# tkoolen/Parametron.jl

Hardware: AMD Instinct MI355X
Metric: QP re-evaluations/sec (Q,q,C,d rebuild) at n=4096 (higher is better)
Workload: dtype f64; 1 GPU; C2 dense least-squares QP: n=4096 vars, A 4096x4096, m=512 equality rows, fp64; canonical Q,q,const + C,d MOI triplets; n=4096, r=4096, m=512, objective_mode=canonical, instances_per_gpu=1, parallelism=single GPU, replay=tape

## Files before the change

include/parametron_hip.h:

```cpp
#ifndef PARAMETRON_HIP_H
#define PARAMETRON_HIP_H

#include <stddef.h>
#include <stdint.h>

#ifdef __cplusplus
extern "C" {
#endif

#define PMT_OK 0
#define PMT_DIMENSION_MISMATCH 1
#define PMT_INVALID_ARGUMENT 2
#define PMT_HIP_ERROR 3
#define PMT_STATE_ERROR 4
#define PMT_OUT_OF_MEMORY 5

typedef struct { double coeff; int64_t var; } pmt_linear_term;
typedef struct { double coeff; int64_t row; int64_t col; } pmt_quadratic_term;
typedef struct { int64_t output_index; double coeff; int64_t var; } pmt_vector_affine_term;

const char *pmt_last_error(void);
int pmt_version(void);
int pmt_device_count(void);

// ... 127 lines not shown
int pmt_pack_scalar_affine_f64(const pmt_linear_term *terms, int64_t n, const int64_t *varmap,
                               pmt_linear_term *out_terms, void *stream);
int pmt_pack_scalar_quadratic_f64(const pmt_quadratic_term *quad, int64_t nq, const int64_t *varmap,
                                  pmt_quadratic_term *out_quad, void *stream);
int pmt_pack_vector_affine_f64(const pmt_linear_term *terms, const int64_t *row_ptr, int64_t rows, int64_t row_len,
                               const int64_t *varmap, int64_t row_offset,
                               pmt_vector_affine_term *out_terms, void *stream);

int pmt_canonical_order_affine(int64_t n, const int64_t *host_vars, int64_t *host_perm, int64_t *host_seg_ptr, int64_t *host_out_vars,
                               int64_t *nseg);
int pmt_canonical_order_quadratic(int64_t n, const int64_t *host_rows, const int64_t *host_cols, int64_t *host_perm, int64_t *host_seg_ptr,
                                  int64_t *host_out_rows, int64_t *host_out_cols, int64_t *nseg);
int pmt_segment_sum_f64(const void *in_terms, int64_t in_stride_bytes, const int64_t *perm, const int64_t *seg_ptr, int64_t nseg,
                        void *out_terms, int64_t out_stride_bytes, void *stream);
int pmt_canonical_order_device(const void *terms, int64_t n, int term_bytes, int64_t *perm, int64_t *seg_ptr, int64_t *nseg_host, void *stream);
int pmt_canonical_init_terms(const void *terms, int term_bytes, const int64_t *perm, const int64_t *seg_ptr, int64_t nseg, void *out_terms, void *stream);

size_t pmt_prune_zero_workspace_bytes(int64_t n, int term_bytes);
int pmt_prune_zero_f64(const void *terms, int64_t n, int term_bytes, double atol, void *out_terms, int64_t *out_count,
                       void *workspace, size_t workspace_bytes, void *stream);

enum { PMT_SET_EQUAL = 0, PMT_SET_GREATER = 1, PMT_SET_LESS = 2 };
int pmt_csc_order(int64_t nnz_in, const int64_t *host_rows, const int64_t *host_cols, int64_t nrows, int64_t ncols, int upper,
                  int64_t *host_perm, int64_t *host_seg_ptr, int64_t *host_col_ptr, int64_t *host_row_idx, int64_t *nnz_out);
int pmt_csc_values_f64(const void *src_coeff, int64_t src_stride_bytes, int64_t nnz_in, const int64_t *perm, const int64_t *seg_ptr,
                       int64_t nnz_out, double alpha, const int64_t *dst_index, double *dst_values, void *stream);
int pmt_qp_bounds_f64(const double *consts, int64_t rows, int set_kind, double set_value, double infty, double *l, double *u,
                      void *stream);
int pmt_csc_values_gather_f64(const double *const *term_ptr, int64_t nnz_in, const int64_t *seg_ptr, int64_t nnz_out, double alpha,
                              const int64_t *dst_index, double *dst_values, void *stream);
int pmt_copy_2d_f64(const double *src, int64_t src_pitch, double *dst, int64_t dst_pitch, const int64_t *dst_offset, int64_t rows,
                    int64_t cols, void *stream);
int pmt_qp_bounds_rows_f64(const double *const *const_ptr, const int *set_kind, const double *set_value, int64_t rows, double infty,
                           double *l, double *u, void *stream);

int pmt_sparse_rowmajor_order(int64_t m, int64_t n, const int64_t *host_colptr, const int64_t *host_rowval,
                              int64_t *host_perm, int64_t *host_rows, int64_t *host_cols, int64_t *host_row_ptr);
int pmt_sparse_pack_vector_f64(const double *nzval, const int64_t *perm, const int64_t *term_row, const int64_t *term_var,
                               int64_t nnz, const int64_t *varmap, int64_t row_offset,
                               pmt_vector_affine_term *out_terms, void *stream);
int pmt_sparse_assemble_f64(const double *nzval, const int64_t *perm, const int64_t *term_var, int64_t nnz,
                            pmt_linear_term *out_terms, void *stream);
int pmt_sparse_slab_ptr(int64_t rows, int64_t cols, int nslab, const int64_t *host_row_ptr, const int64_t *host_term_col,
                        int64_t *host_slab_ptr);
int pmt_sparse_pack_vector_slabs_f64(const double *nzval, const int64_t *perm, const int64_t *term_var, const int64_t *slab_ptr,
                                     int64_t rows, int nslab, const int64_t *varmap, int64_t row_offset,
                                     pmt_vector_affine_term *out_terms, void *stream);
int pmt_sparse_assemble_slabs_f64(const double *nzval, const int64_t *perm, const int64_t *term_var, const int64_t *slab_ptr,
                                  int64_t rows, int nslab, pmt_linear_term *out_terms, void *stream);
int pmt_sparse_pack_vector_slabs_u32_f64(const double *nzval, const uint32_t *perm, const uint32_t *term_var, const int64_t *slab_ptr,
                                         int64_t rows, int nslab, const int64_t *varmap, int64_t row_offset,
                                         pmt_vector_affine_term *out_terms, void *stream);
int pmt_sparse_assemble_slabs_u32_f64(const double *nzval, const uint32_t *perm, const uint32_t *term_var, const int64_t *slab_ptr,
                                      int64_t rows, int nslab, pmt_linear_term *out_terms, void *stream);

int pmt_sparse_blocks_width(int64_t m, int64_t n, const int64_t *host_colptr, const int64_t *host_rowval, int *out_cw);
int pmt_sparse_blocks_build(int64_t m, int64_t n, const int64_t *host_colptr, const int64_t *host_rowval, const int64_t *host_perm,
                            const int64_t *host_term_col, const int64_t *host_row_ptr, int cw, uint64_t *host_desc, uint32_t *host_idx,
                            int64_t *host_band_ptr);
int pmt_sparse_pack_vector_blocks_f64(const double *nzval, const uint64_t *desc, const uint32_t *idx, const int64_t *band_ptr,
                                      const int64_t *col_var, int64_t rows, int64_t cols, int64_t nnz, int cw, const int64_t *varmap,
                                      int64_t row_offset, const double *d, int sign, pmt_vector_affine_term *out_terms,
                                      double *out_consts, void *stream);
int pmt_sparse_assemble_blocks_f64(const double *nzval, const uint64_t *desc, const uint32_t *idx, const int64_t *band_ptr,
                                   const int64_t *col_var, int64_t rows, int64_t cols, int64_t nnz, int cw, const double *d, int sign,
                                   pmt_linear_term *out_terms, double *out_consts, void *stream);
int pmt_consts_f64(const double *d, int64_t n, int sign, double *out, void *stream);

int pmt_sparse_gram_count(int64_t m, int64_t n, const int64_t *host_colptr, const int64_t *host_rowval, int64_t *nq, int64_t *nprod);
int pmt_sparse_gram_order(int64_t m, int64_t n, const int64_t *host_colptr, const int64_t *host_rowval, int64_t nq, int64_t nprod,
                          uint32_t *host_pair_j, uint32_t *host_pair_k, int64_t *host_seg_ptr, void *host_prod, uint32_t *host_lin_col,
                          int64_t *nlin);
int pmt_sparse_gram_runs(const int64_t *host_seg_ptr, int64_t nq, int64_t cap, int64_t *host_runs, int64_t *nruns, int64_t *host_long_seg,
                         int64_t *nlong);
int pmt_sparse_gram_f64(const double *nzval, const void *prod, const int64_t *seg_ptr, const uint32_t *pair_j, const uint32_t *pair_k,
                        int64_t nq, const int64_t *runs, int64_t nruns, const int64_t *long_seg, int64_t nlong,
                        const int64_t *lin_seg, const uint32_t *rowidx0, const uint32_t *lin_col, int64_t nlin, const int64_t *lin_runs,
                        int64_t nlin_runs, const int64_t *lin_long, int64_t nlin_long, int64_t rows, const int64_t *xvar, const double *d,
                        int sign, int moi, const int64_t *varmap, pmt_quadratic_term *out_quad, pmt_linear_term *out_lin, double *out_const,
                        void *stream);

int64_t pmt_batch_lsq_slab_doubles(int64_t n, int64_t m);
int pmt_batch_lsq_coeffs_f64(const double *A, const double *b, const double *C, const double *d, int64_t B, int64_t n, int64_t r,
                             int64_t m, int sign_b, int sign_d, double *out, int64_t out_stride, void *stream);
int pmt_batch_expand_f64(const double *slab, int64_t n, int64_t m, const int64_t *xvar, const int64_t *varmap,
                         pmt_quadratic_term *out_quad, pmt_linear_term *out_lin, double *out_const,
                         pmt_vector_affine_term *out_vat, double *out_vconsts, void *stream);

int pmt_fill_uniform_f64(double *dst, int64_t n, uint64_t seed, double scale, void *stream);
int pmt_fill_uniform_matrix_f64(double *dst, int64_t rows, int64_t cols, int64_t lda, uint64_t seed, double scale, void *stream);
int pmt_fill_uniform_dyn_f64(double *dst, int64_t rows, int64_t cols, int64_t lda, const uint64_t *seed_word, double scale, void *stream);
int pmt_fill_uniform_offset_f64(double *dst, int64_t n, uint64_t seed, uint64_t index_offset, double scale, void *stream);

int pmt_profile_enable(int on);
int pmt_profile_filter(const char *substring);
int64_t pmt_profile_report(char *host_buf, size_t cap);
int pmt_profile_kernel_stamps(void *device_words, int64_t workgroups);
int pmt_device_clock_khz(int device, int *khz);

int pmt_comm_unique_id(void *out_id_128_bytes);
int pmt_comm_init_rank(int nranks, int rank, const void *unique_id_128_bytes, int device, void **out_comm);
int64_t pmt_comm_rccl_calls(void *comm);
int pmt_comm_destroy(void *comm);
int pmt_batch_shard(int64_t total, int nranks, int rank, int64_t *per_rank, int64_t *first);
int64_t pmt_batch_num_chunks(int64_t per_rank, int64_t chunk);
int pmt_batch_chunk_range(int64_t per_rank, int64_t chunk, int64_t c, int64_t *lo, int64_t *hi);
int64_t pmt_batch_gathered_offset(int rank, int64_t per_rank, int64_t local_instance, int64_t stride);
int pmt_batch_allgather_f64(void *comm, const double *local, double *gathered, int64_t per_rank, int64_t stride, int64_t chunk, void *stream);
int pmt_batch_step_f64(void *comm, const double *A, const double *b, const double *C, const double *d, int64_t per_rank, int64_t n, int64_t r,
                       int64_t m, int sign_b, int sign_d, double *local, double *gathered, int64_t stride, int64_t chunk, void *stream);

typedef struct pmt_plan pmt_plan;

int pmt_plan_create(int device, void *stream , pmt_plan **out);
int pmt_plan_destroy(pmt_plan *plan);
void *pmt_plan_stream(pmt_plan *plan);
int pmt_plan_alloc(pmt_plan *plan, size_t bytes, void **out_device_ptr);
size_t pmt_plan_bytes_allocated(const pmt_plan *plan);
int pmt_host_alloc(size_t bytes, void **out_host_ptr);
int pmt_host_free(void *host_ptr);
int pmt_plan_upload(pmt_plan *plan, void *device_dst, const void *host_src, size_t bytes);
int pmt_plan_fetch(pmt_plan *plan, void *host_dst, const void *device_src, size_t bytes);
int pmt_plan_zero(pmt_plan *plan, void *device_dst, size_t bytes);
int pmt_plan_upload_2d(pmt_plan *plan, void *device_dst, size_t dst_pitch, const void *host_src, size_t src_pitch, size_t width_bytes,
                       size_t height);
int pmt_plan_fetch_2d(pmt_plan *plan, void *host_dst, size_t dst_pitch, const void *device_src, size_t src_pitch, size_t width_bytes,
                      size_t height);
int pmt_plan_synchronize(pmt_plan *plan);
int pmt_plan_check(pmt_plan *plan);
int pmt_plan_record_fetch(pmt_plan *plan, void *host_dst, const void *device_src, size_t bytes);
int pmt_plan_record_fetch_2d(pmt_plan *plan, void *host_dst, size_t dst_pitch, const void *device_src, size_t src_pitch, size_t width_bytes,
                             size_t height);
int pmt_host_copy_2d(void *host_dst, size_t dst_pitch, const void *host_src, size_t src_pitch, size_t width_bytes, size_t height, int threads);
int pmt_plan_fetch_synchronize(pmt_plan *plan);

int pmt_plan_stage_upload(pmt_plan *plan, void *device_staging, const void *host_src, size_t bytes);
int pmt_plan_stage_upload_2d(pmt_plan *plan, void *device_staging, size_t dst_pitch, const void *host_src, size_t src_pitch, size_t width_bytes,
                             size_t height);
int pmt_plan_wait_staged(pmt_plan *plan);
int pmt_plan_commit_staged(pmt_plan *plan, void *device_dst, const void *device_staging, size_t bytes);
int pmt_plan_staging_consumed(pmt_plan *plan);
int pmt_plan_commit_lane(pmt_plan *plan, int lane);
int pmt_plan_staged_synchronize(pmt_plan *plan);
int pmt_plan_stage_slot(pmt_plan *plan, int slot);

int pmt_plan_begin_record(pmt_plan *plan);
int pmt_plan_end_record(pmt_plan *plan);
int pmt_plan_set_lane(pmt_plan *plan, int lane);
int pmt_plan_lane_stream(pmt_plan *plan, int lane, void **out_stream);
void *pmt_plan_recording_stream(pmt_plan *plan);
int64_t pmt_plan_tape_length(const pmt_plan *plan);
int pmt_plan_set_fusion(pmt_plan *plan, int on);
int pmt_plan_fused(const pmt_plan *plan, int *groups, int *nodes, int64_t *exec_length);
int pmt_plan_fused_phases(const pmt_plan *plan);
int pmt_plan_fused_workgroups(const pmt_plan *plan);
typedef struct pmt_model pmt_model;
int pmt_model_create(pmt_plan *plan, pmt_model **out);
int pmt_model_destroy(pmt_model *model);
int pmt_model_add_mailbox(pmt_model *model, const double *host, int64_t rows, int64_t cols, int64_t row_stride, int64_t col_stride,
                          double *mailbox, int64_t ld, int *out_slot);
int pmt_model_add_seed(pmt_model *model, uint64_t *seed_word, uint64_t base, uint64_t stride, int *out_slot);
int pmt_model_set_host(pmt_model *model, int slot, const double *host);
int pmt_model_add_constant(pmt_model *model, const double *src, double *dst);
int pmt_model_add_fetch(pmt_model *model, void *host_dst, const void *device_src, size_t bytes);
int pmt_model_num_slots(const pmt_model *model);
int pmt_model_update(pmt_model *model, const unsigned char *dirty, int nslots, int synchronize);
int pmt_model_wait(pmt_model *model);
int pmt_plan_update(pmt_plan *plan);
int pmt_plan_instantiate_graph(pmt_plan *plan);

#ifdef __cplusplus
}
#endif
#endif
```

parametron.jl_amd/_lib.py:

```python
import ctypes as C
import os

import numpy as np

HERE = os.path.dirname(os.path.abspath(__file__))
LIB_PATH = os.environ.get("PMT_LIB_PATH") or os.path.join(HERE, "lib", "libparametron_hip.so")

LT = np.dtype([("coeff", "<f8"), ("var", "<i8")])
QT = np.dtype([("coeff", "<f8"), ("row", "<i8"), ("col", "<i8")])
VAT = np.dtype([("out", "<i8"), ("coeff", "<f8"), ("var", "<i8")])

PMT_OK, PMT_DIMENSION_MISMATCH, PMT_INVALID_ARGUMENT, PMT_HIP_ERROR, PMT_STATE_ERROR, PMT_OUT_OF_MEMORY = range(6)
PMT_LSQ_BLOCK, PMT_LSQ_DIAG, PMT_LSQ_LINEAR, PMT_LSQ_CONSTANT = 1, 2, 3, 4
PMT_LSQ_MAX_TERMS, PMT_LSQ_MAX_BLOCKS, PMT_LSQ_MAX_RUNS = 32, 8, 64
PMT_QUAD_MAX_GROUPS = 8
STACK_COLUMN = np.dtype([("src", "<u8"), ("sign", "<i8")])


class LsqTerm(C.Structure):
    _fields_ = [("kind", C.c_int32), ("sign", C.c_int32), ("scale", C.c_double), ("weight", C.c_void_p), ("values", C.c_void_p),
                ("lin", C.c_void_p), ("constant", C.c_void_p), ("vec", C.c_void_p)]


def lsq_terms(terms):
# ... 57 lines not shown

class ArgumentError(ValueError):
    """Julia's ArgumentError (src/lazyexpression.jl:175,185; src/model.jl:226,243,246)."""


class ErrorException(RuntimeError):
    """Julia's ErrorException — error(...) (src/model.jl:50,61,69,139)."""


class HipError(RuntimeError):
    pass


_vp, _i64, _f64, _ci, _u64, _sz = C.c_void_p, C.c_int64, C.c_double, C.c_int, C.c_uint64, C.c_size_t

SIGNATURES = {
    "pmt_last_error": (C.c_char_p, []),
    "pmt_version": (_ci, []),
    "pmt_device_count": (_ci, []),
    "pmt_affine_assemble_f64": (_ci, [_vp, _i64, _i64, _i64, _vp, _vp, _ci, _vp, _vp, _vp]),
    "pmt_affine_pack_vector_f64": (_ci, [_vp, _i64, _i64, _i64, _vp, _vp, _ci, _vp, _i64, _vp, _vp, _vp]),
    "pmt_affine_pack_vector_background_f64": (_ci, [_vp, _i64, _i64, _i64, _vp, _vp, _ci, _vp, _i64, _vp, _vp, _vp]),
    "pmt_vars_addsub_f64": (_ci, [_vp, _i64, _vp, _ci, _vp, _i64, _vp, _vp, _vp, _vp]),
    "pmt_affvec_combine_f64": (_ci, [_i64, _vp, _vp, _i64, _vp, _vp, _vp, _i64, _vp, _ci, _vp, _vp, _i64, _vp, _vp]),
    "pmt_affvec_scale_f64": (_ci, [_i64, _i64, _vp, _vp, _vp, _f64, _vp, _vp, _vp]),
    "pmt_scale_vars_f64": (_ci, [_vp, _i64, _vp, _f64, _vp, _vp]),
    "pmt_scale_numbers_f64": (_ci, [_vp, _i64, _vp, _f64, _vp, _vp]),
    "pmt_transpose_f64": (_ci, [_vp, _i64, _i64, _i64, _vp, _i64, _vp]),
    "pmt_quad_combine_f64": (_ci, [_vp, _i64, _vp, _i64, _ci, _vp, _vp]),
    "pmt_quad_scale_f64": (_ci, [_vp, _i64, _vp, _f64, _vp, _vp]),
    "pmt_copy_bytes": (_ci, [_vp, _vp, _sz, _vp]),
    "pmt_matvecmul_affs_f64": (_ci, [_vp, _i64, _i64, _i64, _vp, _i64, _vp, _vp, _vp, _vp]),
    "pmt_vecdot_numbers_vars_f64": (_ci, [_vp, _vp, _i64, _vp, _vp, _vp]),
    "pmt_vecdot_numbers_affs_f64": (_ci, [_vp, _i64, _vp, _i64, _vp, _vp, _vp, _vp]),
    "pmt_quad_expand_f64": (_ci, [_i64, _vp, _i64, _vp, _vp, _i64, _vp, _ci, _vp, _vp, _vp, _vp, _vp]),
    "pmt_quad_gram_workspace_bytes": (_sz, [_i64, _i64]),
    "pmt_quad_gram_constant_order": (_ci, [_i64, _i64, C.POINTER(_ci), C.POINTER(_ci), C.POINTER(_ci)]),
    "pmt_quad_gram_f64": (_ci, [_vp, _i64, _i64, _i64, _vp, _vp, _ci, _ci, _vp, _vp, _vp, _vp, _vp, _vp]),
    "pmt_quad_gram_csc_f64": (_ci, [_vp, _i64, _i64, _i64, _vp, _vp, _ci, _vp, _f64, _vp, _vp, _vp, _vp, _vp, _vp]),
    "pmt_quad_gram_csc_deliver_f64": (_ci, [_vp, _i64, _i64, _i64, _vp, _vp, _ci, _vp, _f64, _vp, _vp, _ci, _vp, _vp, _vp, _vp]),
    "pmt_quad_gram_deliver_f64": (_ci, [_vp, _i64, _i64, _i64, _vp, _vp, _ci, _ci, _vp, _vp, _vp, _ci, _vp, _vp, _vp, _vp]),
    "pmt_quad_gram_sum_f64": (_ci, [_i64, _vp, _ci, _vp, _vp, _vp, _vp]),
    "pmt_quad_gram_sum_sub_f64": (_ci, [_i64, _vp, _ci, _vp, _vp, _vp, _vp, _vp, _vp]),
    "pmt_affine_stack_columns_f64": (_ci, [_vp, _i64, _i64, _vp, _i64, _vp]),
    "pmt_quad_form_f64": (_ci, [_vp, _i64, _i64, _vp, _ci, _vp, _f64, _vp, _vp, _vp, _vp, _vp]),
    "pmt_quad_groups_gather_f64": (_ci, [_vp, _vp, _vp, _i64, _i64, _vp, _vp, _i64, _vp, _vp, _vp]),
    "pmt_quad_groups_constant_f64": (_ci, [_vp, _ci, _vp, _vp]),
    "pmt_fetch_synchronize": (_ci, [_vp]),
    "pmt_set_host_delivery": (_ci, [_ci]),
    "pmt_get_host_delivery": (_ci, [_ci, C.POINTER(_ci), C.POINTER(_ci)]),
    "pmt_set_fault_injection": (_ci, [_ci]),
    "pmt_bilinear_f64": (_ci, [_vp, _i64, _i64, _i64, _vp, _vp, _ci, _vp, _vp, _vp]),
    "pmt_fill_uniform_matrix_f64": (_ci, [_vp, _i64, _i64, _i64, _u64, _f64, _vp]),
    "pmt_plan_upload_2d": (_ci, [_vp, _vp, _sz, _vp, _sz, _sz, _sz]),
    "pmt_plan_fetch_2d": (_ci, [_vp, _vp, _sz, _vp, _sz, _sz, _sz]),
    "pmt_vecdot_terms_f64": (_ci, [_i64, _vp, _vp, _vp, _vp, _ci, _vp, _vp, _vp]),
    "pmt_vecdot_affs_vars_f64": (_ci, [_i64, _vp, _i64, _vp, _vp, _ci, _vp, _vp, _vp, _vp]),
    "pmt_pack_scalar_affine_f64": (_ci, [_vp, _i64, _vp, _vp, _vp]),
    "pmt_pack_scalar_quadratic_f64": (_ci, [_vp, _i64, _vp, _vp, _vp]),
    "pmt_pack_vector_affine_f64": (_ci, [_vp, _vp, _i64, _i64, _vp, _i64, _vp, _vp]),
    "pmt_canonical_order_affine": (_ci, [_i64, _vp, _vp, _vp, _vp, C.POINTER(_i64)]),
    "pmt_canonical_order_quadratic": (_ci, [_i64, _vp, _vp, _vp, _vp, _vp, _vp, C.POINTER(_i64)]),
    "pmt_canonical_order_device": (_ci, [_vp, _i64, _ci, _vp, _vp, C.POINTER(_i64), _vp]),
    "pmt_canonical_init_terms": (_ci, [_vp, _ci, _vp, _vp, _i64, _vp, _vp]),
    "pmt_segment_sum_f64": (_ci, [_vp, _i64, _vp, _vp, _i64, _vp, _i64, _vp]),
    "pmt_prune_zero_workspace_bytes": (_sz, [_i64, _ci]),
    "pmt_prune_zero_f64": (_ci, [_vp, _i64, _ci, _f64, _vp, _vp, _vp, _sz, _vp]),
    "pmt_csc_order": (_ci, [_i64, _vp, _vp, _i64, _i64, _ci, _vp, _vp, _vp, _vp, C.POINTER(_i64)]),
    "pmt_csc_values_f64": (_ci, [_vp, _i64, _i64, _vp, _vp, _i64, _f64, _vp, _vp, _vp]),
    "pmt_qp_bounds_f64": (_ci, [_vp, _i64, _ci, _f64, _f64, _vp, _vp, _vp]),
    "pmt_csc_values_gather_f64": (_ci, [_vp, _i64, _vp, _i64, _f64, _vp, _vp, _vp]),
    "pmt_copy_2d_f64": (_ci, [_vp, _i64, _vp, _i64, _vp, _i64, _i64, _vp]),
    "pmt_qp_bounds_rows_f64": (_ci, [_vp, _vp, _vp, _i64, _f64, _vp, _vp, _vp]),
    "pmt_sparse_rowmajor_order": (_ci, [_i64, _i64, _vp, _vp, _vp, _vp, _vp, _vp]),
    "pmt_sparse_assemble_f64": (_ci, [_vp, _vp, _vp, _i64, _vp, _vp]),
    "pmt_sparse_pack_vector_f64": (_ci, [_vp, _vp, _vp, _vp, _i64, _vp, _i64, _vp, _vp]),
    "pmt_sparse_slab_ptr": (_ci, [_i64, _i64, _ci, _vp, _vp, _vp]),
    "pmt_sparse_pack_vector_slabs_f64": (_ci, [_vp, _vp, _vp, _vp, _i64, _ci, _vp, _i64, _vp, _vp]),
    "pmt_sparse_assemble_slabs_f64": (_ci, [_vp, _vp, _vp, _vp, _i64, _ci, _vp, _vp]),
    "pmt_sparse_pack_vector_slabs_u32_f64": (_ci, [_vp, _vp, _vp, _vp, _i64, _ci, _vp, _i64, _vp, _vp]),
    "pmt_sparse_assemble_slabs_u32_f64": (_ci, [_vp, _vp, _vp, _vp, _i64, _ci, _vp, _vp]),
    "pmt_sparse_blocks_width": (_ci, [_i64, _i64, _vp, _vp, _vp]),
    "pmt_sparse_blocks_build": (_ci, [_i64, _i64, _vp, _vp, _vp, _vp, _vp, _ci, _vp, _vp, _vp]),
    "pmt_sparse_pack_vector_blocks_f64": (_ci, [_vp, _vp, _vp, _vp, _vp, _i64, _i64, _i64, _ci, _vp, _i64, _vp, _ci, _vp, _vp, _vp]),
    "pmt_sparse_assemble_blocks_f64": (_ci, [_vp, _vp, _vp, _vp, _vp, _i64, _i64, _i64, _ci, _vp, _ci, _vp, _vp, _vp]),
    "pmt_sparse_gram_count": (_ci, [_i64, _i64, _vp, _vp, C.POINTER(_i64), C.POINTER(_i64)]),
    "pmt_sparse_gram_order": (_ci, [_i64, _i64, _vp, _vp, _i64, _i64, _vp, _vp, _vp, _vp, _vp, C.POINTER(_i64)]),
    "pmt_sparse_gram_runs": (_ci, [_vp, _i64, _i64, _vp, C.POINTER(_i64), _vp, C.POINTER(_i64)]),
    "pmt_sparse_gram_f64": (_ci, [_vp, _vp, _vp, _vp, _vp, _i64, _vp, _i64, _vp, _i64, _vp, _vp, _vp, _i64, _vp, _i64, _vp, _i64, _i64, _vp, _vp, _ci,
                                  _ci, _vp, _vp, _vp, _vp, _vp]),
    "pmt_batch_lsq_slab_doubles": (_i64, [_i64, _i64]),
    "pmt_batch_lsq_coeffs_f64": (_ci, [_vp, _vp, _vp, _vp, _i64, _i64, _i64, _i64, _ci, _ci, _vp, _i64, _vp]),
    "pmt_batch_expand_f64": (_ci, [_vp, _i64, _i64, _vp, _vp, _vp, _vp, _vp, _vp, _vp, _vp]),
    "pmt_comm_unique_id": (_ci, [_vp]),
    "pmt_comm_init_rank": (_ci, [_ci, _ci, _vp, _ci, C.POINTER(_vp)]),
    "pmt_comm_destroy": (_ci, [_vp]),
    "pmt_comm_rccl_calls": (_i64, [_vp]),
    "pmt_batch_num_chunks": (_i64, [_i64, _i64]),
    "pmt_batch_chunk_range": (_ci, [_i64, _i64, _i64, C.POINTER(_i64), C.POINTER(_i64)]),
    "pmt_batch_gathered_offset": (_i64, [_ci, _i64, _i64, _i64]),
    "pmt_batch_shard": (_ci, [_i64, _ci, _ci, C.POINTER(_i64), C.POINTER(_i64)]),
    "pmt_batch_allgather_f64": (_ci, [_vp, _vp, _vp, _i64, _i64, _i64, _vp]),
    "pmt_batch_step_f64": (_ci, [_vp, _vp, _vp, _vp, _vp, _i64, _i64, _i64, _i64, _ci, _ci, _vp, _vp, _i64, _i64, _vp]),
    "pmt_consts_f64": (_ci, [_vp, _i64, _ci, _vp, _vp]),
    "pmt_fill_uniform_f64": (_ci, [_vp, _i64, _u64, _f64, _vp]),
    "pmt_fill_uniform_offset_f64": (_ci, [_vp, _i64, _u64, _u64, _f64, _vp]),
    "pmt_profile_enable": (_ci, [_ci]),
    "pmt_profile_filter": (_ci, [C.c_char_p]),
    "pmt_profile_kernel_stamps": (_ci, [_vp, _i64]),
    "pmt_device_clock_khz": (_ci, [_ci, C.POINTER(_ci)]),
    "pmt_profile_report": (_i64, [C.c_char_p, _sz]),
    "pmt_plan_create": (_ci, [_ci, _vp, C.POINTER(_vp)]),
    "pmt_plan_destroy": (_ci, [_vp]),
    "pmt_plan_stream": (_vp, [_vp]),
    "pmt_plan_alloc": (_ci, [_vp, _sz, C.POINTER(_vp)]),
    "pmt_plan_bytes_allocated": (_sz, [_vp]),
    "pmt_host_alloc": (_ci, [_sz, C.POINTER(_vp)]),
    "pmt_host_free": (_ci, [_vp]),
    "pmt_plan_upload": (_ci, [_vp, _vp, _vp, _sz]),
    "pmt_plan_fetch": (_ci, [_vp, _vp, _vp, _sz]),
    "pmt_plan_zero": (_ci, [_vp, _vp, _sz]),
    "pmt_plan_synchronize": (_ci, [_vp]),
    "pmt_plan_check": (_ci, [_vp]),
    "pmt_model_create": (_ci, [_vp, C.POINTER(_vp)]),
    "pmt_model_destroy": (_ci, [_vp]),
    "pmt_model_add_mailbox": (_ci, [_vp, _vp, _i64, _i64, _i64, _i64, _vp, _i64, C.POINTER(_ci)]),
    "pmt_model_add_seed": (_ci, [_vp, C.POINTER(C.c_uint64), C.c_uint64, C.c_uint64, C.POINTER(_ci)]),
    "pmt_model_set_host": (_ci, [_vp, _ci, _vp]),
    "pmt_model_add_constant": (_ci, [_vp, _vp, _vp]),
    "pmt_model_add_fetch": (_ci, [_vp, _vp, _vp, C.c_size_t]),
    "pmt_model_num_slots": (_ci, [_vp]),
    "pmt_model_update": (_ci, [_vp, _vp, _ci, _ci]),
    "pmt_model_wait": (_ci, [_vp]),
    "pmt_plan_record_fetch": (_ci, [_vp, _vp, _vp, _sz]),
    "pmt_plan_record_fetch_2d": (_ci, [_vp, _vp, _sz, _vp, _sz, _sz, _sz]),
    "pmt_host_copy_2d": (_ci, [_vp, _sz, _vp, _sz, _sz, _sz, _ci]),
    "pmt_plan_fetch_synchronize": (_ci, [_vp]),
    "pmt_plan_stage_upload": (_ci, [_vp, _vp, _vp, _sz]),
    "pmt_plan_stage_upload_2d": (_ci, [_vp, _vp, _sz, _vp, _sz, _sz, _sz]),
    "pmt_plan_wait_staged": (_ci, [_vp]),
    "pmt_plan_commit_staged": (_ci, [_vp, _vp, _vp, _sz]),
    "pmt_plan_staging_consumed": (_ci, [_vp]),
    "pmt_plan_staged_synchronize": (_ci, [_vp]),
    "pmt_plan_stage_slot": (_ci, [_vp, _ci]),
    "pmt_plan_begin_record": (_ci, [_vp]),
    "pmt_plan_end_record": (_ci, [_vp]),
    "pmt_plan_commit_lane": (_ci, [_vp, _ci]),
    "pmt_plan_set_lane": (_ci, [_vp, _ci]),
    "pmt_plan_lane_stream": (_ci, [_vp, _ci, C.POINTER(_vp)]),
    "pmt_plan_recording_stream": (_vp, [_vp]),
    "pmt_plan_tape_length": (_i64, [_vp]),
    "pmt_plan_set_fusion": (_ci, [_vp, _ci]),
    "pmt_plan_fused": (_ci, [_vp, C.POINTER(_ci), C.POINTER(_ci), C.POINTER(_i64)]),
    "pmt_plan_fused_phases": (_ci, [_vp]),
    "pmt_plan_fused_workgroups": (_ci, [_vp]),
    "pmt_fill_uniform_dyn_f64": (_ci, [_vp, _i64, _i64, _i64, C.POINTER(_u64), _f64, _vp]),
    "pmt_plan_update": (_ci, [_vp]),
    "pmt_plan_instantiate_graph": (_ci, [_vp]),
}

_lib = None


def load():
    global _lib
    if _lib is None:
        if not os.path.exists(LIB_PATH):
            raise ErrorException(
                "libparametron_hip.so is not built (%s); run `python -c 'import __graft_entry__ as g; g.build()'`" % LIB_PATH)
        if os.environ.get("PMT_NO_TORCH_PRELOAD") != "1":
            try:
                import torch
            except Exception:
                pass
        L = C.CDLL(LIB_PATH)
        for name, (res, args) in SIGNATURES.items():
            fn = getattr(L, name)
            fn.restype = res
            fn.argtypes = args
        _lib = L
    return _lib


def require_gpu():
    n = load().pmt_device_count()
    if n <= 0:
        raise ErrorException("no MI355X / HIP device visible: the Parametron hot path has no CPU fallback")
    return n


def check(rc):
    if rc == PMT_OK:
        return
    msg = load().pmt_last_error().decode("utf-8", "replace")
    if rc == PMT_DIMENSION_MISMATCH:
        raise DimensionMismatch(msg)
    if rc == PMT_INVALID_ARGUMENT:
        raise ArgumentError(msg)
    if rc == PMT_STATE_ERROR:
        raise ErrorException(msg)
    if rc == PMT_OUT_OF_MEMORY:
        raise MemoryError(msg)
    raise HipError(msg)


def call(name, *args):
    check(getattr(load(), name)(*args))
```

parametron.jl_amd/csrc/affine.hip:

```cpp
#include "common.h"

namespace pmt {

constexpr int64_t NTL_MIN_BYTES = 8 << 20;

constexpr int TILE = 64;
constexpr int PITCH = TILE + 1;

typedef unsigned long long u64;
typedef u64 u64x2 __attribute__((ext_vector_type(2)));
typedef double f64x2 __attribute__((ext_vector_type(2)));

__device__ __forceinline__ u64 f2u(double x) { return (u64)__double_as_longlong(x); }

template <bool NT>
__device__ __forceinline__ void store16(u64x2 *p, u64x2 v) {
    if (NT) __builtin_nontemporal_store(v, p); else *p = v;
}
template <bool NT>
__device__ __forceinline__ void store8(u64 *p, u64 v) {
    if (NT) __builtin_nontemporal_store(v, p); else *p = v;
}

template <int MODE, bool NT, int TR, bool NTL = false>
__global__ __launch_bounds__(256) void affine_tile_kernel(
    const double *__restrict__ A, int64_t lda, int64_t rows, int64_t cols,
    const int64_t *__restrict__ xvar, const double *__restrict__ b, int sign,
    const int64_t *__restrict__ varmap, int64_t row_offset,
    u64 *__restrict__ out, double *__restrict__ out_consts, int vec_in, int vec_out, u64 *stamps, unsigned stamp_cap) {
    __shared__ double tile[TR * PITCH];
    __shared__ u64 vmx[TILE];

    const int t = threadIdx.x;
    const unsigned wg = blockIdx.y * gridDim.x + blockIdx.x;
    if (stamps && t == 0 && wg < stamp_cap) stamps[2 * wg] = (u64)wall_clock64();
    const int lane = t & 63;
    const int wave = t >> 6;
    const int64_t c0 = (int64_t)blockIdx.x * TILE;
    const int64_t r0 = (int64_t)blockIdx.y * TR;
    const int nr = (int)min((int64_t)TR, rows - r0);
    const int nc = (int)min((int64_t)TILE, cols - c0);
    const bool full = (nr == TR) && (nc == TILE);

    if (full && vec_in) {
        constexpr int TPC = TR / 2;
        constexpr int CPI = 256 / TPC;
        const int cg = t / TPC;
        const int lr = (t % TPC) * 2;
        const double *base = A + (c0 + cg) * lda + r0 + lr;
#pragma unroll
        for (int it = 0; it < TILE / CPI; ++it) {
            const f64x2 *src = reinterpret_cast<const f64x2 *>(base + (int64_t)it * CPI * lda);
            f64x2 v = NTL ? __builtin_nontemporal_load(src) : *src;
            const int c = it * CPI + cg;
            tile[lr * PITCH + c] = v.x;
            tile[(lr + 1) * PITCH + c] = v.y;
        }
    } else {
        const int r = t & 63;
        for (int c = t >> 6; c < nc; c += 4)
            if (r < nr) tile[r * PITCH + c] = A[(c0 + c) * lda + r0 + r];
    }
    if (t < nc) {
        const int64_t v = xvar[c0 + t];
        vmx[t] = (u64)(MODE == 1 ? map_var(varmap, v) : v);
    }
    if (blockIdx.x == 0 && t < nr && out_consts)
        out_consts[r0 + t] = signed_const(b ? b[r0 + t] : 0.0, b ? sign : 0);
    __syncthreads();

    if (MODE == 0) {
        if (lane < nc) {
            const u64 var = vmx[lane];
            for (int r = wave; r < nr; r += 4) {
                u64x2 v;
                v.x = f2u(tile[r * PITCH + lane]);
                v.y = var;
                store16<NT>(reinterpret_cast<u64x2 *>(out + ((r0 + r) * cols + c0 + lane) * 2), v);
            }
        }
    } else {
        if (full && vec_out) {
            for (int rp = wave * 2; rp < TR; rp += 8) {
#pragma unroll
                for (int s = 0; s < 3; ++s) {
                    int r, chunk;
                    if (s == 0) { r = rp; chunk = lane; }
                    else if (s == 1) { r = rp + (lane >> 5); chunk = 64 + (lane & 31); }
                    else { r = rp + 1; chunk = lane; }
                    const int q0 = chunk * 2;
                    const u64 rowidx = (u64)(row_offset + r0 + r + 1);
                    u64 w[2];
#pragma unroll
                    for (int h = 0; h < 2; ++h) {
                        const int q = q0 + h;
                        const int term = q / 3;
                        const int f = q - term * 3;
                        w[h] = (f == 0) ? rowidx : (f == 1 ? f2u(tile[r * PITCH + term]) : vmx[term]);
                    }
                    u64x2 v; v.x = w[0]; v.y = w[1];
                    store16<NT>(reinterpret_cast<u64x2 *>(out + ((r0 + r) * cols + c0) * 3 + q0), v);
                }
            }
        } else {
            if (lane < nc) {
                const u64 var = vmx[lane];
                for (int r = wave; r < nr; r += 4) {
                    u64 *p = out + ((r0 + r) * cols + c0 + lane) * 3;
                    store8<NT>(p, (u64)(row_offset + r0 + r + 1));
                    store8<NT>(p + 1, f2u(tile[r * PITCH + lane]));
                    store8<NT>(p + 2, var);
                }
            }
        }
    }
    if (stamps) {
        __syncthreads();
        if (t == 0 && wg < stamp_cap) {
            __builtin_amdgcn_s_waitcnt(0);
            stamps[2 * wg + 1] = (u64)wall_clock64();
        }
    }
}

__global__ void vars_addsub_kernel(const int64_t *__restrict__ xvar, int64_t n, const double *__restrict__ v, int sign,
                                   const int64_t *__restrict__ varmap, int64_t row_offset,
                                   LT *__restrict__ out_lt, VAT *__restrict__ out_vat, double *__restrict__ out_consts) {
    const int64_t i = (int64_t)blockIdx.x * blockDim.x + threadIdx.x;
    if (i >= n) return;
    const int64_t var = xvar[i];
    if (out_lt) { LT t; t.coeff = 1.0; t.var = var; out_lt[i] = t; }
    if (out_vat) { VAT t; t.output_index = row_offset + i + 1; t.coeff = 1.0; t.var = map_var(varmap, var); out_vat[i] = t; }
    if (out_consts) out_consts[i] = signed_const(v ? v[i] : 0.0, v ? sign : 0);
}

__global__ void consts_kernel(const double *__restrict__ d, int64_t n, int sign, double *__restrict__ out) {
    const int64_t i = (int64_t)blockIdx.x * blockDim.x + threadIdx.x;
    if (i < n) out[i] = signed_const(d[i], sign);
}

__global__ __launch_bounds__(256) void affine_pack_background_kernel(const double *__restrict__ A, int64_t lda, int rows, int cols,
                                                                     const int64_t *__restrict__ xvar, const int64_t *__restrict__ varmap,
                                                                     int64_t row_offset, unsigned long long *__restrict__ out) {
    const int wave = blockIdx.x * 4 + (threadIdx.x >> 6), lane = threadIdx.x & 63;
    const int chunk = wave / rows, row = wave - chunk * rows;
    const int c0 = chunk * 256 + lane;
    const double *a = A + row;
    unsigned long long *o = out + (int64_t)row * cols * 3;
    const unsigned long long rowword = (unsigned long long)(row_offset + row + 1);
#pragma unroll 1
    for (int c = c0; c < min(cols, chunk * 256 + 256); c += 64) {
        const double v = a[(int64_t)c * lda];
        const int64_t var = map_var(varmap, xvar[c]);
        unsigned long long *p = o + (int64_t)c * 3;
        p[0] = rowword;
        p[1] = (unsigned long long)__double_as_longlong(v);
        p[2] = (unsigned long long)var;
    }
}

__global__ void pack_scalar_affine_kernel(const LT *__restrict__ in, int64_t n, const int64_t *__restrict__ varmap, LT *__restrict__ out) {
    const int64_t i = (int64_t)blockIdx.x * blockDim.x + threadIdx.x;
    if (i >= n) return;
    LT t = in[i];
    t.var = map_var(varmap, t.var);
    out[i] = t;
}
__global__ __launch_bounds__(256) void pack_scalar_quadratic_kernel(const QT *__restrict__ in, int64_t n, const int64_t *__restrict__ varmap,
                                                                    QT *__restrict__ out, int aligned) {
    typedef unsigned long long u64;
    typedef u64 u64x2 __attribute__((ext_vector_type(2)));
    __shared__ u64 words[256 * 3];
    const int64_t base = (int64_t)blockIdx.x * 256;
    const int cnt = (int)min((int64_t)256, n - base);
    const int tid = threadIdx.x;
    if (aligned && cnt == 256) {
        const u64x2 *src = reinterpret_cast<const u64x2 *>(in + base);
        u64x2 *sw = reinterpret_cast<u64x2 *>(words);
        sw[tid] = src[tid];
        if (tid < 128) sw[256 + tid] = src[256 + tid];
        __syncthreads();
        const double c = __longlong_as_double((long long)words[3 * tid]);
        const int64_t r = (int64_t)words[3 * tid + 1], cl = (int64_t)words[3 * tid + 2];
        const double cm = (r == cl) ? 2 * c : c;
        words[3 * tid] = (u64)__double_as_longlong(cm);
        words[3 * tid + 1] = (u64)map_var(varmap, r);
        words[3 * tid + 2] = (u64)map_var(varmap, cl);
        __syncthreads();
        u64x2 *dst = reinterpret_cast<u64x2 *>(out + base);
        dst[tid] = sw[tid];
        if (tid < 128) dst[256 + tid] = sw[256 + tid];
        return;
    }
    if (tid < cnt) {
        QT t = in[base + tid];
        QT o;
        o.coeff = (t.row == t.col) ? 2 * t.coeff : t.coeff;
        o.row = map_var(varmap, t.row);
        o.col = map_var(varmap, t.col);
        out[base + tid] = o;
    }
}
__global__ __launch_bounds__(256) void pack_vector_affine_kernel(const LT *__restrict__ in, const int64_t *__restrict__ row_ptr, int64_t rows,
                                                                 int64_t row_len, const int64_t *__restrict__ varmap, int64_t row_offset,
                                                                 VAT *__restrict__ out) {
    typedef unsigned long long u64;
    __shared__ u64 s_c[4][64], s_v[4][64];
    const int wave = threadIdx.x >> 6, lane = threadIdx.x & 63;
    const int64_t row = (int64_t)blockIdx.x * 4 + wave;
    if (row >= rows) return;
    const int64_t beg = row_ptr ? row_ptr[row] : row * row_len;
    const int64_t end = row_ptr ? row_ptr[row + 1] : beg + row_len;
    const u64 rowword = (u64)(row_offset + row + 1);
    for (int64_t ts = beg; ts < end; ts += 64) {
        const int cnt = (int)min((int64_t)64, end - ts);
        if (lane < cnt) {
            const LT t = in[ts + lane];
            s_c[wave][lane] = (u64)__double_as_longlong(t.coeff);
            s_v[wave][lane] = (u64)map_var(varmap, t.var);
        }
        __builtin_amdgcn_wave_barrier();
        wave_write_words<3>(reinterpret_cast<u64 *>(out) + ts * 3, cnt, lane, [&](int q) -> u64 {
            const int t = q / 3, f = q - 3 * t;
            return f == 0 ? rowword : (f == 1 ? s_c[wave][t] : s_v[wave][t]);
        });
        __builtin_amdgcn_wave_barrier();
    }
}

static int validate_affine(const double *A, int64_t lda, int64_t rows, int64_t cols, const int64_t *xvar, const double *b,
                           int sign, const void *out_terms) {
    PMT_REQUIRE(rows >= 0 && cols >= 0, PMT_DIMENSION_MISMATCH, "affine: negative dimension");
    PMT_REQUIRE(lda >= rows, PMT_DIMENSION_MISMATCH, "affine: lda < rows");
    PMT_REQUIRE(sign >= -1 && sign <= 1, PMT_INVALID_ARGUMENT, "affine: sign must be -1, 0 or +1");
    if (rows > 0 && cols > 0) {
        PMT_REQUIRE(A && xvar && out_terms, PMT_INVALID_ARGUMENT, "affine: null pointer");
    }
    PMT_REQUIRE(sign == 0 || b || rows == 0, PMT_INVALID_ARGUMENT, "affine: sign != 0 needs b");
    return PMT_OK;
}

static bool env_nt() {
#ifdef PMT_TUNING
    static int v = -1;
    if (v < 0) { const char *e = getenv("PMT_NONTEMPORAL"); v = (e && e[0] == '0') ? 0 : 1; }
    return v != 0;
#else
    return true;
#endif
}

static u64 *g_stamps = nullptr;
static unsigned g_stamp_cap = 0;

template <int MODE>
static int launch_affine(const double *A, int64_t lda, int64_t rows, int64_t cols, const int64_t *xvar, const double *b, int sign,
                         const int64_t *varmap, int64_t row_offset, void *out_terms, double *out_consts, hipStream_t s) {
    if (rows == 0 || cols == 0) return PMT_OK;
    const int vec_in = ((reinterpret_cast<uintptr_t>(A) & 15) == 0 && (lda & 1) == 0) ? 1 : 0;
    const int vec_out = ((reinterpret_cast<uintptr_t>(out_terms) & 15) == 0 && (cols & 1) == 0) ? 1 : 0;
    const char *name = MODE == 0 ? "affine_tile_kernel<LT>" : "affine_tile_kernel<VAT>";
    u64 *out = reinterpret_cast<u64 *>(out_terms);
    const bool small = cdiv(cols, TILE) * cdiv(rows, TILE) < 1024 && rows > 32;
    const bool ntl = MODE == 1 && rows * cols * (int64_t)sizeof(double) >= NTL_MIN_BYTES;
    u64 *stamps = MODE == 1 ? g_stamps : nullptr;
#define AFFINE_LAUNCH(NTV, TRV, NTLV)                                                                                                    \
    PMT_LAUNCH_NAMED(name, (affine_tile_kernel<MODE, NTV, TRV, NTLV>), dim3((unsigned)cdiv(cols, TILE), (unsigned)cdiv(rows, TRV)), dim3(256), 0, s, A, \
                     lda, rows, cols, xvar, b, sign, varmap, row_offset, out, out_consts, vec_in, vec_out, stamps, g_stamp_cap)
    if constexpr (MODE == 1) {
        if (ntl) {
            if (small) AFFINE_LAUNCH(true, 32, true); else AFFINE_LAUNCH(true, 64, true);
            return check_launch("affine_tile_kernel");
        }
    }
    if (env_nt()) { if (small) AFFINE_LAUNCH(true, 32, false); else AFFINE_LAUNCH(true, 64, false); }
    else { if (small) AFFINE_LAUNCH(false, 32, false); else AFFINE_LAUNCH(false, 64, false); }
#undef AFFINE_LAUNCH
    return check_launch("affine_tile_kernel");
}

}

using namespace pmt;

extern "C" int pmt_profile_kernel_stamps(void *device_words, int64_t workgroups) {
    PMT_REQUIRE(workgroups >= 0 && workgroups < ((int64_t)1 << 31), PMT_INVALID_ARGUMENT, "profile_kernel_stamps: bad capacity");
    g_stamps = workgroups > 0 ? reinterpret_cast<u64 *>(device_words) : nullptr;
    g_stamp_cap = g_stamps ? (unsigned)workgroups : 0;
    return PMT_OK;
}

extern "C" int pmt_device_clock_khz(int device, int *khz) {
    PMT_REQUIRE(khz, PMT_INVALID_ARGUMENT, "device_clock_khz: null pointer");
    PMT_HIP_CHECK(hipDeviceGetAttribute(khz, hipDeviceAttributeWallClockRate, device));
    return PMT_OK;
}

extern "C" int pmt_affine_assemble_f64(const double *A, int64_t lda, int64_t rows, int64_t cols, const int64_t *xvar, const double *b,
                                       int sign, pmt_linear_term *out_terms, double *out_consts, void *stream) {
    int rc = validate_affine(A, lda, rows, cols, xvar, b, sign, out_terms);
    if (rc) return rc;
    if (cols == 0 && rows > 0 && out_consts)
        return b && sign ? pmt_consts_f64(b, rows, sign, out_consts, stream)
                         : dispatch(stream, [=](hipStream_t s) { PMT_HIP_CHECK(hipMemsetAsync(out_consts, 0, rows * sizeof(double), s)); return PMT_OK; });
    SmallNode nd;
    nd.op = SOP_AFFINE_LT; nd.sign = sign; nd.d[0] = lda; nd.d[1] = rows; nd.d[2] = cols; nd.d[3] = 0;
    nd.in[0] = A; nd.in[1] = xvar; nd.in[2] = b; nd.out[0] = out_terms; nd.out[1] = out_consts; nd.work = rows * cols + rows;
    return dispatch(stream, [=](hipStream_t s) {
        return launch_affine<0>(A, lda, rows, cols, xvar, b, sign, nullptr, 0, out_terms, out_consts, s);
    }, nd);
}

extern "C" int pmt_affine_pack_vector_f64(const double *A, int64_t lda, int64_t rows, int64_t cols, const int64_t *xvar, const double *b,
                                          int sign, const int64_t *varmap, int64_t row_offset, pmt_vector_affine_term *out_terms,
                                          double *out_consts, void *stream) {
    int rc = validate_affine(A, lda, rows, cols, xvar, b, sign, out_terms);
    if (rc) return rc;
    if (cols == 0 && rows > 0 && out_consts)
        return b && sign ? pmt_consts_f64(b, rows, sign, out_consts, stream)
                         : dispatch(stream, [=](hipStream_t s) { PMT_HIP_CHECK(hipMemsetAsync(out_consts, 0, rows * sizeof(double), s)); return PMT_OK; });
    SmallNode nd;
    nd.op = SOP_AFFINE_VAT; nd.sign = sign; nd.d[0] = lda; nd.d[1] = rows; nd.d[2] = cols; nd.d[3] = row_offset;
    nd.in[0] = A; nd.in[1] = xvar; nd.in[2] = b; nd.in[3] = varmap; nd.out[0] = out_terms; nd.out[1] = out_consts; nd.work = rows * cols + rows;
    return dispatch(stream, [=](hipStream_t s) {
        return launch_affine<1>(A, lda, rows, cols, xvar, b, sign, varmap, row_offset, out_terms, out_consts, s);
    }, nd);
}

extern "C" int pmt_affine_pack_vector_background_f64(const double *A, int64_t lda, int64_t rows, int64_t cols, const int64_t *xvar, const double *b,
                                                     int sign, const int64_t *varmap, int64_t row_offset, pmt_vector_affine_term *out_terms,
                                                     double *out_consts, void *stream) {
    int rc = validate_affine(A, lda, rows, cols, xvar, b, sign, out_terms);
    if (rc) return rc;
    PMT_REQUIRE(rows < (1 << 30) && cols < (1 << 30) && cdiv(cols, 256) * rows < ((int64_t)1 << 31), PMT_DIMENSION_MISMATCH,
                "affine_pack_vector_background: block too large");
    if (rows > 0 && out_consts) {
        rc = b && sign ? pmt_consts_f64(b, rows, sign, out_consts, stream)
                       : dispatch(stream, [=](hipStream_t s) { PMT_HIP_CHECK(hipMemsetAsync(out_consts, 0, rows * sizeof(double), s)); return PMT_OK; });
        if (rc) return rc;
    }
    if (rows == 0 || cols == 0) return PMT_OK;
    return dispatch(stream, [=](hipStream_t s) {
        const int64_t waves = cdiv(cols, 256) * rows;
        PMT_LAUNCH(affine_pack_background_kernel, dim3((unsigned)cdiv(waves, 4)), dim3(256), 0, s, A, lda, (int)rows, (int)cols, xvar, varmap, row_offset,
                   reinterpret_cast<unsigned long long *>(out_terms));
        return check_launch("affine_pack_background_kernel");
    });
}

extern "C" int pmt_vars_addsub_f64(const int64_t *xvar, int64_t n, const double *v, int sign, const int64_t *varmap, int64_t row_offset,
                                   pmt_linear_term *out_terms_lt, pmt_vector_affine_term *out_terms_vat, double *out_consts, void *stream) {
    PMT_REQUIRE(n >= 0, PMT_DIMENSION_MISMATCH, "vars_addsub: negative length");
    PMT_REQUIRE(sign >= -1 && sign <= 1, PMT_INVALID_ARGUMENT, "vars_addsub: sign must be -1, 0 or +1");
    if (n == 0) return PMT_OK;
    PMT_REQUIRE(xvar, PMT_INVALID_ARGUMENT, "vars_addsub: null xvar");
    PMT_REQUIRE(sign == 0 || v, PMT_INVALID_ARGUMENT, "vars_addsub: sign != 0 needs v");
    SmallNode nd;
    nd.op = SOP_VARS_ADDSUB; nd.sign = sign; nd.d[0] = n; nd.d[1] = row_offset; nd.in[0] = xvar; nd.in[1] = v; nd.in[2] = varmap;
    nd.out[0] = out_terms_lt; nd.out[1] = out_terms_vat; nd.out[2] = out_consts; nd.work = n;
    return dispatch(stream, [=](hipStream_t s) {
        PMT_LAUNCH(vars_addsub_kernel, dim3((unsigned)cdiv(n, 256)), dim3(256), 0, s, xvar, n, v, sign, varmap, row_offset,
                           out_terms_lt, out_terms_vat, out_consts);
        return check_launch("vars_addsub_kernel");
    }, nd);
}

extern "C" int pmt_consts_f64(const double *d, int64_t n, int sign, double *out, void *stream) {
    PMT_REQUIRE(n >= 0, PMT_DIMENSION_MISMATCH, "consts: negative length");
    if (n == 0) return PMT_OK;
    PMT_REQUIRE(d && out, PMT_INVALID_ARGUMENT, "consts: null pointer");
    SmallNode nd;
    nd.op = SOP_CONSTS; nd.sign = sign; nd.d[0] = n; nd.in[0] = d; nd.out[0] = out; nd.work = n;
    return dispatch(stream, [=](hipStream_t s) {
        PMT_LAUNCH(consts_kernel, dim3((unsigned)cdiv(n, 256)), dim3(256), 0, s, d, n, sign, out);
        return check_launch("consts_kernel");
    }, nd);
}

extern "C" int pmt_pack_scalar_affine_f64(const pmt_linear_term *terms, int64_t n, const int64_t *varmap, pmt_linear_term *out_terms,
                                          void *stream) {
    PMT_REQUIRE(n >= 0, PMT_DIMENSION_MISMATCH, "pack_scalar_affine: negative length");
    if (n == 0) return PMT_OK;
    PMT_REQUIRE(terms && out_terms, PMT_INVALID_ARGUMENT, "pack_scalar_affine: null pointer");
    SmallNode nd;
    nd.op = SOP_PACK_SA; nd.d[0] = n; nd.in[0] = terms; nd.in[1] = varmap; nd.out[0] = out_terms; nd.work = n;
    return dispatch(stream, [=](hipStream_t s) {
        PMT_LAUNCH(pack_scalar_affine_kernel, dim3((unsigned)cdiv(n, 256)), dim3(256), 0, s, terms, n, varmap, out_terms);
        return check_launch("pack_scalar_affine_kernel");
    }, nd);
}

extern "C" int pmt_pack_scalar_quadratic_f64(const pmt_quadratic_term *quad, int64_t nq, const int64_t *varmap,
                                             pmt_quadratic_term *out_quad, void *stream) {
    PMT_REQUIRE(nq >= 0, PMT_DIMENSION_MISMATCH, "pack_scalar_quadratic: negative length");
    if (nq == 0) return PMT_OK;
    PMT_REQUIRE(quad && out_quad, PMT_INVALID_ARGUMENT, "pack_scalar_quadratic: null pointer");
    SmallNode nd;
    nd.op = SOP_PACK_SQ; nd.d[0] = nq; nd.in[0] = quad; nd.in[1] = varmap; nd.out[0] = out_quad; nd.work = nq;
    return dispatch(stream, [=](hipStream_t s) {
        const int aligned = (((reinterpret_cast<uintptr_t>(quad) | reinterpret_cast<uintptr_t>(out_quad)) & 15) == 0) ? 1 : 0;
        PMT_LAUNCH(pack_scalar_quadratic_kernel, dim3((unsigned)cdiv(nq, 256)), dim3(256), 0, s, quad, nq, varmap, out_quad, aligned);
        return check_launch("pack_scalar_quadratic_kernel");
    }, nd);
}

extern "C" int pmt_pack_vector_affine_f64(const pmt_linear_term *terms, const int64_t *row_ptr, int64_t rows, int64_t row_len,
                                          const int64_t *varmap, int64_t row_offset, pmt_vector_affine_term *out_terms, void *stream) {
    PMT_REQUIRE(rows >= 0 && row_len >= 0, PMT_DIMENSION_MISMATCH, "pack_vector_affine: negative dimension");
    if (rows == 0) return PMT_OK;
    PMT_REQUIRE((terms && out_terms) || (!row_ptr && row_len == 0), PMT_INVALID_ARGUMENT, "pack_vector_affine: null pointer");
    SmallNode nd;
    nd.op = SOP_PACK_VA; nd.d[0] = rows; nd.d[1] = row_len; nd.d[2] = row_offset; nd.in[0] = terms; nd.in[1] = row_ptr; nd.in[2] = varmap;
    nd.out[0] = out_terms;
    nd.work = row_ptr ? SMALL_NODE_WORK_MAX + 1 : rows * row_len;
    return dispatch(stream, [=](hipStream_t s) {
        PMT_LAUNCH(pack_vector_affine_kernel, dim3((unsigned)cdiv(rows, 4)), dim3(256), 0, s, terms, row_ptr, rows, row_len, varmap,
                           row_offset, out_terms);
        return check_launch("pack_vector_affine_kernel");
    }, nd);
}
```

parametron.jl_amd/csrc/gram.hip:

```cpp
#include <algorithm>
#include <memory>
#include <vector>

#include "streams.h"

#ifndef PMT_GRAM_ABL_NO_LINEAR
#define PMT_GRAM_ABL_NO_LINEAR 0
#endif

namespace pmt {

constexpr size_t PAIR_FLAG_BYTES = 4096;
constexpr int DELIVER_ORDER_W = 1;

__global__ __launch_bounds__(256) void gram_linear_kernel(const double *__restrict__ A, int64_t lda, int64_t rows, int64_t cols,
                                                          const int64_t *__restrict__ xvar, const double *__restrict__ b, int sign,
                                                          int moi, const int64_t *__restrict__ varmap, LT *__restrict__ out_lin) {
    const int64_t col = (int64_t)blockIdx.x * 4 + (threadIdx.x >> 6);
    if (col >= cols) return;
    const int lane = threadIdx.x & 63;
    const double *a = A + col * lda;
    double acc = 0.0;
    if (b && sign)
        for (int64_t i = lane; i < rows; i += 64) acc += signed_const(b[i], sign) * a[i];
// ... 115 lines not shown
    double *host = nullptr;
    double *host_dev = nullptr;
    const double *src = nullptr;
    std::shared_ptr<DeliverSignals> sig;
    int order_w = 0, nstages = 0;
    int64_t seq_begin[MAXGROUPS], seq_count[MAXGROUPS];
    int group_of[MAXGROUPS];
    int ngroups = 0;
    int64_t gbeg[MAXGROUPS], gend[MAXGROUPS];
};

static DeliverPlan deliver_plan(int64_t rows, int64_t cols, bool staged, int nstages_hint, bool quad) {
    DeliverPlan d;
#ifdef PMT_TUNING
    static const int order_w = [] { const char *e = getenv("PMT_DELIVER_ORDER_W"); return e ? atoi(e) : DELIVER_ORDER_W; }();
#else
    constexpr int order_w = DELIVER_ORDER_W;
#endif
    d.order_w = quad ? 0 : -order_w;
    const int nt = (int)cdiv(cols, ST);
    const int64_t T = (int64_t)nt * (nt + 1) / 2;
    const int64_t nchunk = std::max<int64_t>(1, cdiv(rows, 256));
    const int64_t G = std::min<int64_t>(T * nchunk, 256);
    int64_t per = nchunk >= 2 ? std::max<int64_t>(1, G / 2) : G;
    if (nstages_hint > 0) per = std::max<int64_t>(1, cdiv(T, std::min(nstages_hint, MAXGROUPS)));
    if (cdiv(T, per) > MAXGROUPS) per = cdiv(T, MAXGROUPS);
    if (!staged) per = T;
    std::vector<int64_t> seq_end_of_band((size_t)nt), bandbeg((size_t)nt), bandend((size_t)nt);
    int64_t seq_end = 0;
    if (quad) {
        for (int j0 = 0; j0 < nt; j0 += 4) {
            const int h = std::min(4, nt - j0), W = nt - j0;
            seq_end += (int64_t)h * (h + 1) / 2 + (int64_t)(W - h) * h;
            for (int jb = j0; jb < j0 + h; ++jb) seq_end_of_band[(size_t)jb] = seq_end;
        }
        for (int jb = 0; jb < nt; ++jb) {
            const int64_t J0 = (int64_t)jb * ST, J = std::min<int64_t>(cols, (int64_t)(jb + 1) * ST);
            bandbeg[(size_t)jb] = 3 * (J0 * cols - J0 * (J0 - 1) / 2);
            bandend[(size_t)jb] = 3 * (J * cols - J * (J - 1) / 2);
        }
    } else {
        std::vector<int64_t> start_of_super((size_t)nt);
        int64_t pos = 0;
        for (int c0 = 0; c0 < nt; c0 += order_w) {
            const int h = std::min(order_w, nt - c0);
            for (int kb = c0; kb < c0 + h; ++kb) start_of_super[(size_t)kb] = pos;
            pos += (int64_t)c0 * h + (int64_t)h * (h + 1) / 2;
        }
        for (int kb = 0; kb < nt; ++kb) {
            seq_end_of_band[(size_t)kb] = T - start_of_super[(size_t)kb];
            const int64_t c0 = (int64_t)kb * ST, cend = std::min<int64_t>(cols, (int64_t)(kb + 1) * ST);
            bandbeg[(size_t)kb] = c0 * (c0 + 1) / 2;
            bandend[(size_t)kb] = cend * (cend + 1) / 2;
        }
    }
    auto band_at = [&](int i) { return quad ? i : nt - 1 - i; };
    int done_bands = 0;
    for (int64_t t0 = 0; t0 < T; t0 += per) {
        const int st = d.nstages++;
        d.seq_begin[st] = t0;
        d.seq_count[st] = std::min<int64_t>(per, T - t0);
        int nb = done_bands;
        while (nb < nt && seq_end_of_band[(size_t)band_at(nb)] <= t0 + d.seq_count[st]) ++nb;
        d.group_of[st] = -1;
        if (nb > done_bands) {
            d.group_of[st] = d.ngroups;
            const int first = band_at(done_bands), last = band_at(nb - 1);
            d.gbeg[d.ngroups] = bandbeg[(size_t)std::min(first, last)];
            d.gend[d.ngroups] = bandend[(size_t)std::max(first, last)];
            ++d.ngroups;
            done_bands = nb;
        }
    }
    return d;
}

struct GramArgs {
    const double *A; int64_t lda, rows, cols; const int64_t *xvar; const double *b; int sign, moi; const int64_t *varmap;
    pmt_quadratic_term *out_quad; double *out_csc; double alpha; pmt_linear_term *out_lin; double *out_const; void *workspace;
};

static int deliver_arm(const DeliverPlan &d, SideStream *side, hipStream_t s) {
    PMT_REQUIRE(side && side->counters, PMT_STATE_ERROR, "quad_gram_csc_deliver: no auxiliary streams for this stream");
    DeliverSignals *sig = d.sig.get();
    const int mode = dma::delivery_mode();
    if (sig->pending) { if (int rc = dma::wait(sig->eng, sig->done, 10.0)) return rc; sig->pending = false; }
    if (!side->in_replay) { if (int rc = wait_dma_pending(side)) return rc; }
    if (mode != 2 && !sig->tried) {
        sig->tried = true;
        dma::Engine *eng = dma::get(side->device);
        bool ok = eng && dma::signal_create(eng, 0, &sig->done) == PMT_OK;
        for (int i = 0; ok && i < d.ngroups; ++i) { ok = dma::signal_create(eng, 1, &sig->dep[i]) == PMT_OK; if (ok) sig->n = i + 1; }
        if (ok) sig->eng = eng;
    }
    sig->engine = mode != 2 && sig->eng != nullptr;
    PMT_REQUIRE(mode != 1 || sig->engine, PMT_STATE_ERROR, "host delivery: the copy engine was demanded (pmt_set_host_delivery(1)) but is not available");
    if (side->fetch_pending) { PMT_HIP_CHECK(hipStreamWaitEvent(s, side->fetch_done, 0)); side->fetch_pending = false; }
    if (!sig->engine) return ensure_fetch_stream(side);
    for (int i = 0; i < d.ngroups; ++i) dma::signal_set(sig->eng, sig->dep[i], 1);
    dma::signal_set(sig->eng, sig->done, d.ngroups);
    return PMT_OK;
}

static int release_group(const DeliverPlan &d, SideStream *side, int grp, hipStream_t s) {
    const dma::Signal flag{0, reinterpret_cast<int64_t *>(static_cast<char *>(side->counters) + FLAGS_OFFSET) + grp};
    return dma::launch_signal_store(d.sig->engine ? d.sig->dep[grp] : flag, s);
}

static int deliver_submit(const DeliverPlan &d, SideStream *side) {
    if (!d.sig->engine) {
        char *cb = static_cast<char *>(side->counters);
        if (int rc = launch_courier(d.src, d.host_dev, reinterpret_cast<long long *>(cb + FLAGS_OFFSET), reinterpret_cast<unsigned *>(cb + DONE_OFFSET),
                                    side->err_dev, d.ngroups, d.gbeg, d.gend, side->fetch)) return rc;
        PMT_HIP_CHECK(hipEventRecord(side->fetch_done, side->fetch));
        side->fetch_pending = true;
        return PMT_OK;
    }
    auto submit = [p = d]() -> int {
        for (int i = 0; i < p.ngroups; ++i)
            if (int rc = dma::copy_to_host(p.sig->eng, p.host + p.gbeg[i], p.src + p.gbeg[i], sizeof(double) * (size_t)(p.gend[i] - p.gbeg[i]),
                                           &p.sig->dep[i], p.sig->done, 1)) return rc;
        return PMT_OK;
    };
    d.sig->pending = true;
    side->dma_pending.emplace_back(d.sig->eng, d.sig->done);
    side->keepalive.push_back(d.sig);
    if (!side->in_replay) return submit();
    side->deferred.push_back(submit);
    return PMT_OK;
}

static int fork_side(SideStream *side, hipStream_t s) {
    PMT_HIP_CHECK(hipEventRecord(side->fork, s));
    PMT_HIP_CHECK(hipStreamWaitEvent(side->stream, side->fork, 0));
    return PMT_OK;
}
static bool forks_in_replay(const SideStream *side) { return side && side->in_replay && side->side_work; }

static int fused_node(const GramArgs &g, SideStream *side, hipStream_t s) {
    int rc = launch_gram_tall(g.A, g.lda, g.rows, g.cols, g.xvar, g.b, g.sign, g.moi, g.varmap, g.out_quad, g.out_csc, g.alpha, g.out_lin,
                              g.out_const, g.workspace, s);
    if (!rc && forks_in_replay(side)) rc = fork_side(side, s);
    const int64_t nt = cdiv(g.cols, ST);
    if (!rc && nt > 1)
        rc = launch_gram_sk(g.A, g.lda, g.rows, g.cols, g.xvar, g.varmap, g.moi, g.out_quad, g.out_csc, g.alpha, g.workspace, 0, 0, nt * (nt - 1) / 2,
                            nullptr, 0, nullptr, s, 1);
    return rc;
}

static int mid_node(const GramArgs &g, SideStream *side, hipStream_t s) {
    PMT_REQUIRE(side && side->counters && (size_t)gram_mid_counters(g.cols) * sizeof(unsigned) <= MID_COUNTER_BYTES, PMT_STATE_ERROR,
                "quad_gram: no auxiliary state for this stream");
    int rc = launch_gram_mid(g.A, g.lda, g.rows, g.cols, g.xvar, g.b, g.sign, g.moi, g.varmap, g.out_quad, g.out_csc, g.alpha, g.out_lin,
                             g.out_const, g.workspace, reinterpret_cast<unsigned *>(static_cast<char *>(side->counters) + MID_OFFSET), s);
    return !rc && forks_in_replay(side) ? fork_side(side, s) : rc;
}

static int stream_k_node(const GramArgs &g, bool staged, const DeliverPlan &d, SideStream *side, hipStream_t s) {
    hipStream_t s2 = side ? side->stream : s;
    if (side) { if (int rc = fork_side(side, s)) return rc; }
    if (side && side->in_replay) side->side_work = true;
    const int64_t rows = g.rows, cols = g.cols;
    int rc = PMT_OK;
    double *scratch = g.workspace ? reinterpret_cast<double *>(static_cast<char *>(g.workspace) + gram_sk_workspace_bytes(rows, cols)) : nullptr;
    const int nsplit = (scratch && g.b && g.sign) ? linear_splits(rows, cols) : 1;
    if (PMT_GRAM_ABL_NO_LINEAR) {
    } else if (cols > 0 && nsplit > 1) {
        const int64_t chunk = 64 * cdiv(cdiv(rows, nsplit), 64);
        PMT_LAUNCH(gram_linear_split_kernel, dim3((unsigned)cdiv(cols, 4), (unsigned)nsplit), dim3(256), 0, s2, g.A, g.lda, rows, cols, g.b, g.sign, chunk, scratch);
        PMT_LAUNCH(gram_linear_finish_kernel, dim3((unsigned)cdiv(cols, 256)), dim3(256), 0, s2, scratch, nsplit, cols, g.xvar, g.moi, g.varmap, g.out_lin);
        rc = check_launch("gram_linear_split_kernel");
    } else if (cols > 0) {
        PMT_LAUNCH(gram_linear_kernel, dim3((unsigned)cdiv(cols, 4)), dim3(256), 0, s2, g.A, g.lda, rows, cols, g.xvar, g.b, g.sign, g.moi, g.varmap, g.out_lin);
        rc = check_launch("gram_linear_kernel");
    }
    double *chains = scratch ? scratch + (size_t)linear_splits(rows, cols) * (size_t)cols : nullptr;
    const int order = constant_order(staged ? GramForm::StreamKStaged : GramForm::StreamK, rows, cols).order;
    auto const_part = [=]() -> int {
        int rc2 = PMT_OK;
        if (order == 5) rc2 = launch_gram_mid_constant(g.b, g.sign, rows, g.out_const, s2);
        else if (g.b && g.sign && rows > 0) rc2 = launch_blocked_dot(g.b, g.sign, g.b, g.sign, rows, chains, g.out_const, s2, order);
        else if (hipMemsetAsync(g.out_const, 0, sizeof(double), s2) != hipSuccess) rc2 = fail(PMT_HIP_ERROR, "hipMemsetAsync(out_const)");
        if (side) { PMT_HIP_CHECK(hipEventRecord(side->join2, side->stream)); PMT_HIP_CHECK(hipStreamWaitEvent(s, side->join2, 0)); }
        return rc2;
    };
    const bool defer_const = side && side->in_replay;
    if (!rc && defer_const) side->deferred.push_back(const_part);
    if (side) PMT_HIP_CHECK(hipEventRecord(side->join, side->stream));
    if (!rc && cols > 0 && !staged) rc = launch_gram_sk(g.A, g.lda, rows, cols, g.xvar, g.varmap, g.moi, g.out_quad, g.out_csc, g.alpha, g.workspace, 0, 0, -1,
                                                        nullptr, 0, nullptr, s);
    else if (!rc && cols > 0) {
        unsigned *pair_flags = g.workspace ? reinterpret_cast<unsigned *>(static_cast<char *>(g.workspace) + gram_sk_workspace_bytes(rows, cols) - PAIR_FLAG_BYTES) : nullptr;
        if (pair_flags) PMT_HIP_CHECK(hipMemsetAsync(pair_flags, 0, PAIR_FLAG_BYTES, s));
        for (int st = 0; !rc && st < d.nstages; ++st) {
            rc = launch_gram_sk(g.A, g.lda, rows, cols, g.xvar, g.varmap, g.moi, g.out_quad, g.out_csc, g.alpha, g.workspace, d.order_w, d.seq_begin[st],
                                d.seq_count[st], pair_flags, (unsigned)(st + 1), side->err_dev, s);
            if (!rc && d.group_of[st] >= 0) rc = release_group(d, side, d.group_of[st], s);
        }
        if (!rc) rc = deliver_submit(d, side);
    }
    if (side) PMT_HIP_CHECK(hipStreamWaitEvent(s, side->join, 0));
    if (!rc && !defer_const) rc = const_part();
    return rc;
}

static int gram_node(const GramArgs &g, void *stream, double *host = nullptr, int ngroups = 0) {
    const int64_t rows = g.rows, cols = g.cols;
    PMT_REQUIRE(rows >= 0 && cols >= 0, PMT_DIMENSION_MISMATCH, "quad_gram: negative dimension");
    PMT_REQUIRE(g.lda >= rows, PMT_DIMENSION_MISMATCH, "quad_gram: lda < rows");
    PMT_REQUIRE(g.sign >= -1 && g.sign <= 1, PMT_INVALID_ARGUMENT, "quad_gram: sign must be -1, 0 or +1");
    PMT_REQUIRE(g.out_const, PMT_INVALID_ARGUMENT, "quad_gram: null out_const");
    PMT_REQUIRE(g.sign == 0 || g.b || rows == 0, PMT_INVALID_ARGUMENT, "quad_gram: sign != 0 needs b");
    if (cols > 0) PMT_REQUIRE(g.xvar && (g.out_quad || g.out_csc) && g.out_lin && (g.A || rows == 0), PMT_INVALID_ARGUMENT, "quad_gram: null pointer");
    PMT_REQUIRE(cols < (int64_t)ST * 32000, PMT_DIMENSION_MISMATCH, "quad_gram: too many columns");
    const GramForm form = gram_form(rows, cols, g.out_csc != nullptr, host != nullptr);
    PMT_REQUIRE(g.workspace || (form != GramForm::Fused && form != GramForm::Mid), PMT_INVALID_ARGUMENT, "quad_gram: workspace required");
    if (int rc = check_strictly_increasing(g.xvar, cols, stream)) return rc;
    if (form == GramForm::Tiny) {
        SmallNode nd;
        nd.op = SOP_GRAM; nd.sign = (g.b && g.sign) ? g.sign : 0; nd.moi = g.moi; nd.d[0] = g.lda; nd.d[1] = rows; nd.d[2] = cols;
        nd.in[0] = g.A; nd.in[1] = g.xvar; nd.in[2] = g.b; nd.in[3] = g.varmap; nd.out[0] = g.out_quad; nd.out[1] = g.out_lin; nd.out[2] = g.out_const;
        nd.work = rows * cols * (cols + 1) / 2 + 64 * rows;
        return dispatch(stream, [=](hipStream_t s) { return launch_small_one(nd, s); }, nd);
    }
    DeliverPlan dplan;
    if (host && cols > 0) {
        dplan = deliver_plan(rows, cols, form == GramForm::StreamKStaged, ngroups, !g.out_csc);
        dplan.host = host;
        dplan.src = g.out_csc ? g.out_csc : reinterpret_cast<const double *>(g.out_quad);
        dplan.host_dev = static_cast<double *>(host_device_pointer(host));
        PMT_REQUIRE(dplan.host_dev, PMT_INVALID_ARGUMENT, "quad_gram_csc_deliver: host_P_values must be page-locked host memory (pmt_host_alloc)");
        dplan.sig = std::make_shared<DeliverSignals>();
        mark_no_graph(stream);
    }
    return dispatch(stream, [=](hipStream_t s) -> int {
        SideStream *side = side_stream(s);
        const bool deliver = dplan.host != nullptr;
        if (deliver) { if (int rc = deliver_arm(dplan, side, s)) return rc; }
        if (form == GramForm::StreamK || form == GramForm::StreamKStaged) return stream_k_node(g, form == GramForm::StreamKStaged, dplan, side, s);
        int rc = form == GramForm::Fused ? fused_node(g, side, s) : mid_node(g, side, s);
        if (!rc && deliver) rc = release_group(dplan, side, 0, s);
        if (!rc && deliver) rc = deliver_submit(dplan, side);
        return rc;
    });
}

}

using namespace pmt;

extern "C" int pmt_quad_gram_constant_order(int64_t rows, int64_t cols, int *order, int *groups, int *stage_rows) {
    PMT_REQUIRE(rows >= 0 && cols >= 0 && order, PMT_INVALID_ARGUMENT, "quad_gram_constant_order: bad argument");
    const ConstantOrder o = constant_order(gram_form(rows, cols, true, false), rows, cols);
    *order = o.order; if (groups) *groups = o.groups; if (stage_rows) *stage_rows = o.stage_rows;
    return PMT_OK;
}

extern "C" size_t pmt_quad_gram_workspace_bytes(int64_t rows, int64_t cols) {
    size_t bytes = gram_sk_workspace_bytes(rows, cols) +
                   sizeof(double) * ((size_t)linear_splits(rows, cols) * (size_t)std::max<int64_t>(cols, 0) + blocked_dot_scratch_doubles());
    for (const bool deliver : {false, true}) {
        const GramForm form = gram_form(rows, cols, true, deliver);
        bytes = std::max(bytes, form == GramForm::Fused ? gram_tall_workspace_bytes(rows, cols) : form == GramForm::Mid ? gram_mid_workspace_bytes(rows, cols) : 0);
    }
    return bytes;
}

extern "C" int pmt_quad_gram_f64(const double *A, int64_t lda, int64_t rows, int64_t cols, const int64_t *xvar, const double *b, int sign,
                                 int moi, const int64_t *varmap, pmt_quadratic_term *out_quad, pmt_linear_term *out_lin, double *out_const,
                                 void *workspace, void *stream) {
    if (cols > 0) PMT_REQUIRE(out_quad, PMT_INVALID_ARGUMENT, "quad_gram: null out_quad");
    return gram_node({A, lda, rows, cols, xvar, b, sign, moi, varmap, out_quad, nullptr, 1.0, out_lin, out_const, workspace}, stream);
}

extern "C" int pmt_quad_gram_csc_f64(const double *A, int64_t lda, int64_t rows, int64_t cols, const int64_t *xvar, const double *b, int sign,
                                     const int64_t *varmap, double alpha, double *out_P_values, pmt_quadratic_term *out_quad,
                                     pmt_linear_term *out_lin, double *out_const, void *workspace, void *stream) {
    if (cols > 0) PMT_REQUIRE(out_P_values, PMT_INVALID_ARGUMENT, "quad_gram_csc: null out_P_values");
    return gram_node({A, lda, rows, cols, xvar, b, sign, 1, varmap, out_quad, out_P_values, alpha, out_lin, out_const, workspace}, stream);
}

extern "C" int pmt_quad_gram_deliver_f64(const double *A, int64_t lda, int64_t rows, int64_t cols, const int64_t *xvar, const double *b, int sign,
                                         int moi, const int64_t *varmap, pmt_quadratic_term *out_quad, pmt_quadratic_term *host_quad, int nstages,
                                         pmt_linear_term *out_lin, double *out_const, void *workspace, void *stream) {
    if (cols > 0) PMT_REQUIRE(out_quad && host_quad, PMT_INVALID_ARGUMENT, "quad_gram_deliver: null out_quad / host_quad");
    PMT_REQUIRE(nstages >= 0 && nstages <= MAXGROUPS, PMT_INVALID_ARGUMENT, "quad_gram_deliver: nstages must be 0 (default) .. 16");
    return gram_node({A, lda, rows, cols, xvar, b, sign, moi, varmap, out_quad, nullptr, 1.0, out_lin, out_const, workspace}, stream, reinterpret_cast<double *>(host_quad), nstages);
}

extern "C" int pmt_quad_gram_csc_deliver_f64(const double *A, int64_t lda, int64_t rows, int64_t cols, const int64_t *xvar, const double *b, int sign,
                                             const int64_t *varmap, double alpha, double *out_P_values, double *host_P_values, int ngroups,
                                             pmt_linear_term *out_lin, double *out_const, void *workspace, void *stream) {
    if (cols > 0) PMT_REQUIRE(out_P_values && host_P_values, PMT_INVALID_ARGUMENT, "quad_gram_csc_deliver: null P values pointer");
    PMT_REQUIRE(ngroups >= 0 && ngroups <= MAXGROUPS, PMT_INVALID_ARGUMENT, "quad_gram_csc_deliver: ngroups must be 0 (default) .. 16");
    return gram_node({A, lda, rows, cols, xvar, b, sign, 1, varmap, nullptr, out_P_values, alpha, out_lin, out_const, workspace}, stream, host_P_values, ngroups);
}
```

parametron.jl_amd/csrc/gram_common.h:

```cpp
#pragma once
#include "common.h"

namespace pmt {

typedef double f64x2 __attribute__((ext_vector_type(2)));
typedef unsigned long long u64;

constexpr int ST = 128;
constexpr int SKC = 256;
constexpr int MAXG = 512;
constexpr int SLOT = ST * ST;
constexpr int MAXGROUPS = 16;

struct SKArgs {
    const double *A; int64_t lda, rows, cols;
    const int64_t *xvar; const int64_t *varmap; int moi;
    QT *out_quad;
    double *out_csc;
    double alpha;
    int ntiles, nchunk, G;
    int skc;
    int tfull;
    int64_t U;
    int vec_in;
// ... 4 lines not shown
    unsigned *pair_flags; unsigned epoch;
    unsigned flag_value;
    int *error;
    long long pair_timeout;
    int strict;
};

template <int TN>
struct Cfg {
    static_assert(TN == 2, "the geometry below is the shipped one only");
    static constexpr int NW = 8;
    static constexpr int NT = NW * 64;
    static constexpr int WCOLS = 16 * TN;
    static constexpr int NWC = ST / WCOLS;
    static constexpr int NACC = 4 * TN * 4;
    static constexpr int NLD = (ST * 8) / NT;
};

__device__ __forceinline__ void sk_tri_unrank(int t, int nt, int &jb, int &kb) {
    int j = (int)((2.0 * nt + 1.0 - sqrt((2.0 * nt + 1.0) * (2.0 * nt + 1.0) - 8.0 * (double)t)) * 0.5);
    if (j < 0) j = 0;
    if (j > nt - 1) j = nt - 1;
    while (j > 0 && (j * nt - j * (j - 1) / 2) > t) --j;
    while (j + 1 < nt && ((j + 1) * nt - (j + 1) * j / 2) <= t) ++j;
    jb = j;
    kb = j + (t - (j * nt - j * (j - 1) / 2));
}

__device__ __forceinline__ void sk_seq_unrank(int idx, int nt, int &jb, int &kb) {
    int base = 0;
    for (int R = 0; R * 4 < nt; ++R) {
        const int j0 = R * 4;
        const int h = min(4, nt - j0);
        const int W = nt - j0;
        const int tri = h * (h + 1) / 2;
        const int count = tri + (W - h) * h;
        if (idx < base + count) {
            int p = idx - base;
            if (p < tri) {
                int c = 0;
                while (p >= c + 1) { p -= c + 1; ++c; }
                kb = j0 + c; jb = j0 + p;
            } else {
                p -= tri;
                kb = j0 + h + p / h; jb = j0 + p % h;
            }
            return;
        }
        base += count;
    }
    jb = kb = nt - 1;
}

__device__ __forceinline__ void sk_colseq_unrank(int idx, int nt, int w, int &jb, int &kb) {
    int base = 0;
    for (int c0 = 0; c0 < nt; c0 += w) {
        const int h = min(w, nt - c0);
        const int rect = c0 * h;
        const int count = rect + h * (h + 1) / 2;
        if (idx < base + count) {
            int p = idx - base;
            if (p < rect) {
                jb = p / h; kb = c0 + p % h;
            } else {
                p -= rect;
                int r = 0;
                while (p >= h - r) { p -= h - r; ++r; }
                jb = c0 + r; kb = c0 + r + p;
            }
            return;
        }
        base += count;
    }
    jb = kb = nt - 1;
}

__device__ __forceinline__ void sk_tile_unrank(const SKArgs &g, int idx, int &jb, int &kb) {
    if (g.order_w > 0) sk_colseq_unrank(idx, g.ntiles, g.order_w, jb, kb);
    else sk_seq_unrank(idx, g.ntiles, jb, kb);
}

__device__ __forceinline__ void sk_tile_unrank_strict(const SKArgs &g, int idx, int &jb, int &kb) {
    sk_seq_unrank(idx, g.ntiles - 1, jb, kb);
    kb += 1;
}

__device__ __forceinline__ int sk_phase_a_index(const SKArgs &g, int bid, int t) {
    if ((g.G & 7) == 0) return (t * 8 + (bid & 7)) * (g.G >> 3) + (bid >> 3);
    return bid * g.tfull + t;
}

__device__ __forceinline__ int64_t sk_unit_begin(const SKArgs &g, int b) { return (int64_t)b * g.U / g.G; }

__device__ __forceinline__ int sk_unit_owner(const SKArgs &g, int64_t u) {
    int b = (int)((u * g.G) / g.U);
    if (b >= g.G) b = g.G - 1;
    while (b + 1 < g.G && sk_unit_begin(g, b + 1) <= u) ++b;
    while (b > 0 && sk_unit_begin(g, b) > u) --b;
    return b;
}

__device__ __forceinline__ double *sk_partial_slot(const SKArgs &g, int b, int rtile) {
    const int64_t bu0 = sk_unit_begin(g, b);
    const int first_rtile = (int)(bu0 / g.nchunk);
    const int slot = 2 * b + (first_rtile == rtile ? 0 : 1);
    return g.ws + (int64_t)slot * SLOT;
}

template <int TN>
__device__ __forceinline__ void sk_acc_pos(int tid, int r, int &row, int &col) {
    const int lane = tid & 63, wave = tid >> 6;
    const int wr = wave / Cfg<TN>::NWC, wc = wave % Cfg<TN>::NWC;
    const int tm = r / (4 * TN), tn = (r / 4) % TN, s = r & 3;
    const int i = lane >> 4, b = (lane >> 2) & 3, j = lane & 3;
    row = wr * 64 + tm * 16 + 4 * b + i;
    col = wc * Cfg<TN>::WCOLS + tn * 16 + 4 * ((b + s) & 3) + j;
}

__device__ __forceinline__ void sk_store_term(const SKArgs &g, int jb, int kb, int row, int col, double v) {
    const int64_t n = g.cols;
    const int64_t j = (int64_t)jb * ST + row, k = (int64_t)kb * ST + col;
    if (k >= n || j >= n || j > k) return;
    double c = v;
    if (g.moi || j != k) c = 2 * c;
    if (g.out_csc) g.out_csc[k * (k + 1) / 2 + j] = g.alpha * c;
    if (!g.out_quad) return;
    const int64_t jv = g.xvar[j], kv = g.xvar[k];
    const int64_t pos = j * n - (j * (j - 1)) / 2 + (k - j);
    u64 *p = reinterpret_cast<u64 *>(g.out_quad) + pos * 3;
    p[0] = (u64)__double_as_longlong(c);
    p[1] = (u64)(g.moi ? map_var(g.varmap, jv) : jv);
    p[2] = (u64)(g.moi ? map_var(g.varmap, kv) : kv);
}


int launch_gram_sk(const double *A, int64_t lda, int64_t rows, int64_t cols, const int64_t *xvar, const int64_t *varmap, int moi,
                   pmt_quadratic_term *out_quad, double *out_csc, double alpha, void *workspace, int order_w, int64_t seq_begin, int64_t seq_count,
                   unsigned *pair_flags, unsigned epoch, int *error_word, hipStream_t s, int strict = 0);
size_t gram_sk_workspace_bytes(int64_t rows, int64_t cols);
bool gram_tiny(int64_t rows, int64_t cols);
bool gram_tall_applies(int64_t rows, int64_t cols);
bool gram_tall_diag_applies(int64_t rows, int64_t cols);
int gram_tall_groups(int64_t rows, int64_t cols);
int gram_tall_stage_rows(int64_t rows, int64_t cols);
int gram_tall_run_lanes(int64_t rows, int64_t cols);
size_t gram_tall_workspace_bytes(int64_t rows, int64_t cols);
int launch_gram_tall(const double *A, int64_t lda, int64_t rows, int64_t cols, const int64_t *xvar, const double *b, int sign, int moi,
                     const int64_t *varmap, pmt_quadratic_term *out_quad, double *out_csc, double alpha, pmt_linear_term *out_lin,
                     double *out_const, void *workspace, hipStream_t s);
size_t gram_mid_workspace_bytes(int64_t rows, int64_t cols);
int gram_mid_counters(int64_t cols);
int launch_gram_mid(const double *A, int64_t lda, int64_t rows, int64_t cols, const int64_t *xvar, const double *b, int sign, int moi,
                    const int64_t *varmap, pmt_quadratic_term *out_quad, double *out_csc, double alpha, pmt_linear_term *out_lin,
                    double *out_const, void *workspace, unsigned *counters, hipStream_t s);
int launch_gram_mid_constant(const double *b, int sign, int64_t rows, double *out_const, hipStream_t s);
int check_strictly_increasing(const int64_t *xvar_dev, int64_t n, void *stream);
void mark_no_graph(void *stream);
int launch_blocked_dot(const double *a, int sign_a, const double *b, int sign_b, int64_t n, double *scratch, double *out, hipStream_t s, int chained);
size_t blocked_dot_scratch_doubles();
int launch_small_one(const SmallNode &nd, hipStream_t s);

}
```

parametron.jl_amd/csrc/gram_mid.hip:

```cpp
#include "gram_common.h"

#ifndef PMT_MID_WPS
#define PMT_MID_WPS 1
#endif
#ifndef PMT_MID_G
#define PMT_MID_G 256
#endif
#ifndef PMT_MID_MAXWG
#define PMT_MID_MAXWG 2304
#endif
#ifndef PMT_MID_D
#define PMT_MID_D 2
#endif
#ifndef PMT_MID_GROUP_US
#define PMT_MID_GROUP_US 1.15
#endif
#ifndef PMT_MID_TAIL_US
#define PMT_MID_TAIL_US 0.95
#endif
#ifndef PMT_MID_SB
#define PMT_MID_SB 8
#endif
#ifndef PMT_MID_FB
#define PMT_MID_FB 4
#endif
#ifndef PMT_MID_FORMAL
#if defined(__HIP_DEVICE_COMPILE__) && !defined(__gfx950__) && !defined(__gfx942__)
#define PMT_MID_FORMAL 1
#else
#define PMT_MID_FORMAL 0
#endif
#endif

#ifdef PMT_MID_TRACE
__device__ unsigned long long g_mid_trace[1024 * 8];
__device__ unsigned long long g_mid_walk[1024 * 8];
#define MID_TRACE_WORDS 8
__device__ __forceinline__ void mid_walk_note(unsigned long long *w, int k, unsigned long long t) {
    if (k == 0) { if (w[0]) w[4] += t - w[7]; else w[5] = t; w[0] += 1; }
    else if (k == 1) w[1] += t - w[7];
    else if (k == 3 || k == 5) { w[2] += t - w[7]; w[6] = t; }
    else if (k == 6) { w[3] += t - w[7]; w[6] = t; }
    else return;
    w[7] = t;
}
#define MID_STAMP(k) do { if (threadIdx.x == 0 && blockIdx.x < 1024) { const unsigned long long t_ = wall_clock64(); g_mid_trace[blockIdx.x * 8 + (k)] = t_; \
                          mid_walk_note(reinterpret_cast<unsigned long long *>(sh + MSH), (k), t_); } } while (0)
extern "C" int pmt_mid_trace_read(unsigned long long *host) {
    return hipMemcpyFromSymbol(host, HIP_SYMBOL(g_mid_trace), sizeof(unsigned long long) * 1024 * 8) == hipSuccess ? 0 : 1;
}
extern "C" int pmt_mid_walk_read(unsigned long long *host) {
    return hipMemcpyFromSymbol(host, HIP_SYMBOL(g_mid_walk), sizeof(unsigned long long) * 1024 * 8) == hipSuccess ? 0 : 1;
}
#else
#define MID_STAMP(k) do { } while (0)
#define MID_TRACE_WORDS 0
#endif

namespace pmt {

constexpr int MT = 64;
constexpr int MACC = 64;
constexpr int MPART = MACC * 64;
constexpr int MSTRIDE = MPART + MT + 8;
constexpr int MPITCH = MT + 1;
constexpr int MFG = 8;
constexpr int MCNT = 16;
constexpr int MQBUF = 4 * 2048;
constexpr int MFLAG = MQBUF + 4 * MT;
constexpr int MMAPS = MFLAG + 8;
constexpr int MSH = MMAPS + 2 * MT;

struct MidArgs {
    const double *A; int64_t lda, rows, cols;
    const double *b; int sign;
    const int64_t *xvar; const int64_t *varmap; int moi;
    QT *out_quad; double *out_csc; double alpha; LT *out_lin; double *out_const;
    int nb;
    int n_off, s_off, s_diag;
    int gpc_off, gpc_diag;
    int n_tail, s_tail, gpc_tail;
    double *ws;
    unsigned *counters;
    int xcd;
    int persist, total;
    unsigned *tickets;
};

struct MidPlan { int nb, n_off, s_off, s_diag, gpc_off, gpc_diag, n_tail, s_tail, gpc_tail, wgs; };

static double mid_fold_us(int count) { return 0.5 + 2.6 * (double)cdiv(count, PMT_MID_FB); }

static MidPlan mid_plan(int64_t rows, int64_t cols) {
    MidPlan p;
    p.nb = (int)cdiv(cols, MT);
    p.n_off = p.nb * (p.nb - 1) / 2;
    const int ngroups = (int)std::max<int64_t>(1, cdiv(rows, 8));
    const int maxs = std::max(1, ngroups / 4);
    auto sd = [&](int s) { return std::min(maxs, std::max(1, (5 * s + 7) / 8)); };
    int best = 1;
    double best_t = 1e300;
    for (int s = 1; s <= std::min(maxs, 64); ++s) {
        const int64_t wgs = (int64_t)p.n_off * s + (int64_t)p.nb * sd(s);
        if (s > 1 && wgs > PMT_MID_MAXWG) break;
        const double it_off = (double)cdiv(cdiv(ngroups, s), 4), it_diag = 0.69 * (double)cdiv(cdiv(ngroups, sd(s)), 4);
        const double fold = s <= 1 ? 0.0 : s <= MFG ? mid_fold_us(s) : mid_fold_us(MFG) + 1.5 + mid_fold_us((int)cdiv(s, MFG));
        const double t = (double)cdiv(wgs, PMT_MID_G) * (PMT_MID_GROUP_US * (p.n_off ? std::max(it_off, it_diag) : it_diag) + 5.0 + (s > 1 ? 1.0 : 0.0)) +
                         fold * (1.0 + (double)(p.n_off + p.nb) / PMT_MID_G);
        if (t < best_t) { best_t = t; best = s; }
    }
    int s = best;
#ifdef PMT_TUNING
    if (const char *e = getenv("PMT_MID_S")) { const int v = atoi(e); if (v > 0) s = std::min(v, maxs); }
#endif
    int sdiag = sd(s), ntail = 0, stail = 1;
    if (p.n_off + p.nb > PMT_MID_G) {
        auto wg_us = [&](int c, double w) { return PMT_MID_TAIL_US * w * (double)cdiv(cdiv(ngroups, c), 4) + 5.0 + (c > 1 ? 1.0 : 0.0); };
        const int rem = p.n_off % PMT_MID_G;
        int ct = 1;
        double tail_off = 0.0;
        if (rem) {
            tail_off = 1e300;
            for (int c = 1; c <= std::min(maxs, MFG); ++c) {
                const double t = (double)cdiv((int64_t)rem * c, PMT_MID_G) * wg_us(c, 1.0) + (c > 1 ? mid_fold_us(c) : 0.0);
                if (t < tail_off) { tail_off = t; ct = c; }
            }
        }
        const int last = rem ? (int)(((int64_t)rem * ct) % PMT_MID_G) : 0, free_cus = last ? PMT_MID_G - last : 0;
        const double t_last = rem ? wg_us(ct, 1.0) : wg_us(1, 1.0);
        int cd = 1;
        double tail_diag = 1e300;
        for (int c = 1; c <= std::min(maxs, MFG); ++c) {
            const double t_d = wg_us(c, 0.69);
            const int64_t inside = (int64_t)free_cus * (int64_t)(t_last / t_d);
            const int64_t left = std::max<int64_t>(0, (int64_t)p.nb * c - inside);
            const double t = (double)cdiv(left, PMT_MID_G) * t_d + (c > 1 ? mid_fold_us(c) : 0.0);
            if (t < tail_diag) { tail_diag = t; cd = c; }
        }
        const double t1 = (double)(p.n_off / PMT_MID_G) * wg_us(1, 1.0) + tail_off + tail_diag;
        if (s == 1 || t1 * (PMT_MID_GROUP_US / PMT_MID_TAIL_US) < best_t) { s = 1; sdiag = cd; ntail = ct > 1 ? rem : 0; stail = ct > 1 ? ct : 1; }
    }
#ifdef PMT_TUNING
    if (const char *e = getenv("PMT_MID_TAIL")) { if (atoi(e) == 0) { ntail = 0; stail = 1; } }
#endif
    p.gpc_off = (int)cdiv(ngroups, s);
    p.s_off = (int)cdiv(ngroups, p.gpc_off);
    p.gpc_diag = (int)cdiv(ngroups, sdiag);
    p.s_diag = (int)cdiv(ngroups, p.gpc_diag);
    p.n_tail = ntail;
    p.gpc_tail = (int)cdiv(ngroups, stail);
    p.s_tail = ntail ? (int)cdiv(ngroups, p.gpc_tail) : 1;
    if (p.s_tail <= 1) { p.n_tail = 0; p.s_tail = 1; p.gpc_tail = ngroups; }
    p.wgs = (p.n_off - p.n_tail) * p.s_off + p.n_tail * p.s_tail + p.nb * p.s_diag + 1;
    return p;
}

template <bool DIAG, bool FAST>
__device__ __forceinline__ void mid_load(const MidArgs &g, int64_t row0, int lane, int64_t cj0, int64_t ck0, const unsigned (&voff)[DIAG ? 4 : 8],
                                         f64x2 (&buf)[DIAG ? 4 : 8], f64x2 &cb) {
    constexpr int NG = DIAG ? 4 : 8;
    const int lm = lane & 15, lk = lane >> 4;
    if (FAST) {
        const char *base = reinterpret_cast<const char *>(g.A + row0);
#pragma unroll
        for (int t = 0; t < NG; ++t) buf[t] = *reinterpret_cast<const f64x2 *>(base + voff[t]);
        cb.x = 0.0; cb.y = 0.0;
        if (DIAG && g.b) cb = *reinterpret_cast<const f64x2 *>(g.b + row0 + 2 * lk);
        return;
    }
    const int64_t row = row0 + 2 * lk;
    const bool r0 = row < g.rows, r1 = row + 1 < g.rows;
#pragma unroll
    for (int t = 0; t < NG; ++t) {
        const int64_t col = (t < 4 ? cj0 : ck0) + 16 * (t & 3) + lm;
        const bool cv = col < g.cols;
        const bool v0 = cv && r0, v1 = cv && r1;
        const double *p0 = g.A + (v0 ? col * g.lda + row : 0), *p1 = g.A + (v1 ? col * g.lda + row + 1 : 0);
        const double x = *p0, y = *p1;
        buf[t].x = v0 ? x : 0.0;
        buf[t].y = v1 ? y : 0.0;
    }
    cb.x = 0.0; cb.y = 0.0;
    if (DIAG && g.b) {
        const double x = g.b[r0 ? row : 0], y = g.b[r1 ? row + 1 : 0];
        cb.x = r0 ? x : 0.0;
        cb.y = r1 ? y : 0.0;
    }
}

template <bool DIAG>
__device__ __forceinline__ void mid_compute(double *__restrict__ rot, const f64x2 (&buf)[DIAG ? 4 : 8], const f64x2 &cb, int sign, int lane,
                                            double (&acc)[MACC], double (&qacc)[4]) {
    constexpr int BO = DIAG ? 0 : 4;
    const int lm = lane & 15, lrow = lane & 48;
#pragma unroll
    for (int t = 0; t < 4; ++t) *reinterpret_cast<f64x2 *>(rot + (t * 64 + lane) * 2) = buf[BO + t];
    f64x2 bv[4][4];
#pragma unroll
    for (int c = 0; c < 4; ++c) {
        bv[c][0] = buf[BO + c];
#pragma unroll
        for (int r = 1; r < 4; ++r) {
            bv[c][r] = *reinterpret_cast<const f64x2 *>(rot + (c * 64 + lrow + ((lm + 4 * r) & 15)) * 2);
        }
    }
    __builtin_amdgcn_sched_barrier(0);
    constexpr int NC = 4;
#pragma unroll
    for (int c = 0; c < NC; ++c)
#pragma unroll
        for (int tm = 0; tm < (DIAG ? c + 1 : 4); ++tm) {
            const int a = (tm * 4 + c) * 4;
            acc[a] = __builtin_amdgcn_mfma_f64_4x4x4f64(buf[tm].x, bv[c][0].x, acc[a], 0, 0, 0);
        }
#pragma unroll
    for (int c = 0; c < NC; ++c)
#pragma unroll
        for (int tm = 0; tm < (DIAG ? c + 1 : 4); ++tm) {
            const int a = (tm * 4 + c) * 4;
            acc[a] = __builtin_amdgcn_mfma_f64_4x4x4f64(buf[tm].y, bv[c][0].y, acc[a], 0, 0, 0);
        }
    __builtin_amdgcn_sched_barrier(0);
#pragma unroll
    for (int c = 0; c < NC; ++c) {
#pragma unroll
        for (int r = 1; r < 4; ++r)
#pragma unroll
            for (int tm = 0; tm < (DIAG ? c + 1 : 4); ++tm) {
                const int a = (tm * 4 + c) * 4 + r;
                acc[a] = __builtin_amdgcn_mfma_f64_4x4x4f64(buf[tm].x, bv[c][r].x, acc[a], 0, 0, 0);
            }
#pragma unroll
        for (int r = 1; r < 4; ++r)
#pragma unroll
            for (int tm = 0; tm < (DIAG ? c + 1 : 4); ++tm) {
                const int a = (tm * 4 + c) * 4 + r;
                acc[a] = __builtin_amdgcn_mfma_f64_4x4x4f64(buf[tm].y, bv[c][r].y, acc[a], 0, 0, 0);
            }
    }
// ... 350 lines not shown
                    mid_load<DIAG, FAST>(g, row_of(s0 + d + D), lane, cj0, ck0, voff, buf[d], cb[d]);
                }
            }
        }
    }
    if (ragged) {
        mid_load<DIAG, false>(g, (int64_t)(ngroups - 1) * 8, lane, cj0, ck0, voff, buf[0], cb[0]);
        mid_compute<DIAG>(rot, buf[0], cb[0], g.sign, lane, acc, qacc);
    }

    MID_STAMP(1);
    wk.pre = pf;
    unsigned drawn = 0;
    if (!DIAG && wk.early && tid == 0) drawn = __hip_atomic_fetch_add(wk.ticket, 1u, __ATOMIC_RELAXED, __HIP_MEMORY_SCOPE_AGENT);
    unsigned *flag = reinterpret_cast<unsigned *>(sh + MFLAG);
    double *w = g.ws + (int64_t)(first_wg + chunk) * MSTRIDE;
    __syncthreads();
    if (wave == 0) mid_tail<DIAG, 0>(g, sh, lane, acc, qacc, nchunk, w);
    else if (wave == 1) mid_tail<DIAG, 1>(g, sh, lane, acc, qacc, nchunk, w);
    else if (wave == 2) mid_tail<DIAG, 2>(g, sh, lane, acc, qacc, nchunk, w);
    else mid_tail<DIAG, 3>(g, sh, lane, acc, qacc, nchunk, w);
    MID_STAMP(2);
    if (nchunk > 1) {
        const bool two = nchunk > MFG;
        const int gfirst = two ? (chunk / MFG) * MFG : 0;
        const int n1 = two ? min(MFG, nchunk - gfirst) : nchunk;
        unsigned *c1 = two ? counter + 1 + chunk / MFG : counter;
        __syncthreads();
        if (tid == 0) *flag = __hip_atomic_fetch_add(c1, 1u, __ATOMIC_RELAXED, __HIP_MEMORY_SCOPE_AGENT);
        __syncthreads();
        MID_STAMP(3);
        if (*flag != (unsigned)(n1 - 1)) { mid_forget(buf); return; }
#if PMT_MID_FORMAL
        __builtin_amdgcn_fence(__ATOMIC_ACQUIRE, "agent");
#endif
        if (tid == 0) __hip_atomic_store(c1, 0u, __ATOMIC_RELAXED, __HIP_MEMORY_SCOPE_AGENT);
        double sum[16], qs;
        double *p = g.ws + (int64_t)(first_wg + gfirst) * MSTRIDE;
        mid_fold<DIAG>(p, n1, MSTRIDE, tid, sum, qs);
        if (two) {
#pragma unroll
            for (int u = 0; u < 16; ++u) if (mid_used(DIAG, (tid >> 6) + 4 * u)) mid_put(p + tid + 256 * u, sum[u]);
            if (DIAG && tid < MT) mid_put(p + MPART + tid, qs);
#if PMT_MID_FORMAL
            __builtin_amdgcn_fence(__ATOMIC_RELEASE, "agent");
#else
            __builtin_amdgcn_s_waitcnt(0);
#endif
            __syncthreads();
            if (tid == 0) *flag = __hip_atomic_fetch_add(counter, 1u, __ATOMIC_RELAXED, __HIP_MEMORY_SCOPE_AGENT);
            __syncthreads();
            const int ng = (nchunk + MFG - 1) / MFG;
            if (*flag != (unsigned)(ng - 1)) { mid_forget(buf); return; }
#if PMT_MID_FORMAL
            __builtin_amdgcn_fence(__ATOMIC_ACQUIRE, "agent");
#endif
            if (tid == 0) __hip_atomic_store(counter, 0u, __ATOMIC_RELAXED, __HIP_MEMORY_SCOPE_AGENT);
            mid_fold<DIAG>(g.ws + (int64_t)first_wg * MSTRIDE, ng, (int64_t)MFG * MSTRIDE, tid, sum, qs);
        }
        __syncthreads();
        MID_STAMP(4);
#pragma unroll
        for (int u = 0; u < 16; ++u) {
            const int a = (tid >> 6) + 4 * u;
            if (!mid_used(DIAG, a)) continue;
            int row, col;
            mid_pos(lane, a, row, col);
            sh[row * MPITCH + col] = sum[u];
        }
        if (DIAG && tid < MT) sh[MT * MPITCH + tid] = qs;
        mid_forget(buf);
    }
    if (!DIAG && wk.early && tid == 0) *wk.slot = wk.id0 + 8 * (int)drawn;
    __syncthreads();
    if (!DIAG && wk.early) wk.drawn = *wk.slot;
    MID_STAMP(5);
    mid_epilogue(g, sh, tid, jb, kb);
#ifdef PMT_MID_TRACE
    __builtin_amdgcn_s_waitcnt(0);
    MID_STAMP(6);
#endif
}

__device__ __forceinline__ int mid_xcd_rank(int id, int base, int n) {
    const int x = id & 7, end = base + n;
    int start = 0;
    for (int y = 0; y < x; ++y) {
        const int fy = base + ((y - base) & 7);
        start += fy < end ? ((end - 1 - fy) >> 3) + 1 : 0;
    }
    return start + ((id - (base + ((x - base) & 7))) >> 3);
}

__device__ __forceinline__ void mid_tile_of(int t, int nb, int &jb, int &kb) {
    constexpr int SB = PMT_MID_SB;
    const int nsb = (nb + SB - 1) / SB;
    for (int K = 0; K < nsb; ++K) {
        const int wK = min(SB, nb - SB * K);
        for (int J = 0; J <= K; ++J) {
            const int cnt = J < K ? SB * wK : wK * (wK - 1) / 2;
            if (t >= cnt) { t -= cnt; continue; }
            if (J < K) { jb = SB * J + t / wK; kb = SB * K + t % wK; return; }
            int kk = 1;
            while (t >= kk) { t -= kk; ++kk; }
            jb = SB * K + t; kb = SB * K + kk;
            return;
        }
    }
    jb = 0; kb = 1;
}

struct MidItem { int kind, jb, kb, chunk, nch, gpc, first, rank; };
__device__ __forceinline__ MidItem mid_decode(const MidArgs &g, int id) {
    MidItem it = {2, 0, 0, 0, 1, 0, 0, 0};
    const int nbody = g.n_off - g.n_tail, wbody = nbody * g.s_off, noff = wbody + g.n_tail * g.s_tail;
    if (id < noff) {
        const bool tail = id >= wbody;
        const int base = tail ? wbody : 0, ntile = tail ? g.n_tail : nbody, nch = tail ? g.s_tail : g.s_off;
        const int k = g.xcd ? mid_xcd_rank(id, base, ntile * nch) : ((id - base) % nch) * ntile + (id - base) / nch;
        const int chunk = k / ntile;
        const int rank = (tail ? nbody : 0) + (k - chunk * ntile);
        int t = rank, jb, kb;
        if (g.xcd) mid_tile_of(t, g.nb, jb, kb);
        else {
            kb = 1;
            while (t >= kb) { t -= kb; ++kb; }
            jb = t;
        }
        it.kind = 0; it.jb = jb; it.kb = kb; it.chunk = chunk; it.nch = nch; it.gpc = tail ? g.gpc_tail : g.gpc_off;
        it.first = tail ? wbody + (rank - nbody) * g.s_tail : rank * g.s_off;
        it.rank = rank;
        return it;
    }
    if (id < noff + g.nb * g.s_diag) {
        const int k = g.xcd ? mid_xcd_rank(id, noff, g.nb * g.s_diag) : ((id - noff) % g.s_diag) * g.nb + (id - noff) / g.s_diag;
        const int chunk = k / g.nb, jb = k - chunk * g.nb;
        it.kind = 1; it.jb = jb; it.kb = jb; it.chunk = chunk; it.nch = g.s_diag; it.gpc = g.gpc_diag; it.first = noff + jb * g.s_diag; it.rank = g.n_off + jb;
    }
    return it;
}

template <bool FAST>
__device__ __forceinline__ void mid_item(const MidArgs &g, double *sh, int tid, const MidItem &it, MidWalk &wk, f64x2 (&pbuf)[PMT_MID_D][8]) {
    if (it.kind == 0) {
        mid_body<false, FAST>(g, sh, tid, it.jb, it.kb, it.chunk, it.nch, it.gpc, it.first, g.counters + it.rank * MCNT, wk, pbuf);
        return;
    }
    wk.pre = false;
    if (it.kind == 1) mid_body<true, FAST>(g, sh, tid, it.jb, it.kb, it.chunk, it.nch, it.gpc, it.first, g.counters + it.rank * MCNT, wk, pbuf);
    else mid_constant(g, sh, tid);
    mid_forget(pbuf);
}

template <bool FAST>
__global__ __launch_bounds__(256, PMT_MID_WPS) void gram_mid_kernel(MidArgs g) {
    __shared__ double sh[MSH + MID_TRACE_WORDS];
    __shared__ int next_id, ahead_id;
    const int tid = threadIdx.x;
    const int x = blockIdx.x & 7, per = gridDim.x >> 3;
#ifdef PMT_MID_TRACE
    if (tid == 0) for (int i = 0; i < MID_TRACE_WORDS; ++i) reinterpret_cast<unsigned long long *>(sh + MSH)[i] = 0;
#endif
    f64x2 pbuf[PMT_MID_D][8];
    MidWalk wk = {};
    wk.ticket = g.tickets + x; wk.id0 = x + 8 * per; wk.slot = &ahead_id;
    const int wbody = (g.n_off - g.n_tail) * g.s_off;
    const bool look = FAST && g.persist && g.s_off == 1;
    int id = blockIdx.x, hand = -1;
    if (look) {
        if (tid == 0) next_id = wk.id0 + 8 * (int)__hip_atomic_fetch_add(wk.ticket, 1u, __ATOMIC_RELAXED, __HIP_MEMORY_SCOPE_AGENT);
        __syncthreads();
        hand = next_id;
    }
    MidItem cur = mid_decode(g, id);
    for (;;) {
        wk.early = hand >= 0 && hand < wbody;
        wk.next_full = false;
        if (wk.early) {
            const MidItem nx = mid_decode(g, hand);
            wk.next_full = (int64_t)(nx.kb + 1) * MT <= g.cols;
            wk.njb = nx.jb; wk.nkb = nx.kb; wk.nrank = nx.rank;
        }
        mid_item<FAST>(g, sh, tid, cur, wk, pbuf);
        if (!g.persist) return;
        __syncthreads();
        if (wk.early) {
            id = hand; hand = wk.drawn;
            cur.jb = wk.njb; cur.kb = wk.nkb; cur.first = cur.rank = wk.nrank;
            continue;
        }
        if (hand >= 0) { id = hand; hand = -1; }
        else {
            if (tid == 0) next_id = wk.id0 + 8 * (int)__hip_atomic_fetch_add(wk.ticket, 1u, __ATOMIC_RELAXED, __HIP_MEMORY_SCOPE_AGENT);
            __syncthreads();
            id = next_id;
        }
        if (id >= g.total) break;
        cur = mid_decode(g, id);
    }
#ifdef PMT_MID_TRACE
    if (tid == 0 && blockIdx.x < 1024) {
        for (int i = 0; i < 7; ++i) g_mid_walk[blockIdx.x * 8 + i] = reinterpret_cast<unsigned long long *>(sh + MSH)[i];
        g_mid_walk[blockIdx.x * 8 + 7] = wall_clock64();
    }
#endif
    if (tid == 0) {
        const unsigned gone = __hip_atomic_fetch_add(g.tickets + 8, 1u, __ATOMIC_RELAXED, __HIP_MEMORY_SCOPE_AGENT);
        if (gone == gridDim.x - 1) {
#pragma unroll
            for (int i = 0; i < 9; ++i) __hip_atomic_store(g.tickets + i, 0u, __ATOMIC_RELAXED, __HIP_MEMORY_SCOPE_AGENT);
        }
    }
}

__global__ __launch_bounds__(256) void gram_mid_constant_kernel(MidArgs g) {
    __shared__ double sh[8];
    mid_constant(g, sh, threadIdx.x);
}
int launch_gram_mid_constant(const double *b, int sign, int64_t rows, double *out_const, hipStream_t s) {
    MidArgs g = {};
    g.rows = rows; g.b = (b && sign) ? b : nullptr; g.sign = g.b ? sign : 0; g.out_const = out_const;
    PMT_LAUNCH_NAMED("gram_mid_constant_kernel", gram_mid_constant_kernel, dim3(1), dim3(256), 0, s, g);
    return check_launch("gram_mid_constant_kernel");
}

size_t gram_mid_workspace_bytes(int64_t rows, int64_t cols) {
    if (cols <= 0) return 0;
    const MidPlan p = mid_plan(rows, cols);
    return sizeof(double) * (size_t)p.wgs * MSTRIDE;
}
int gram_mid_counters(int64_t cols) { const int nb = (int)cdiv(cols, MT); return MCNT * (nb * (nb + 1) / 2) + 16; }

int launch_gram_mid(const double *A, int64_t lda, int64_t rows, int64_t cols, const int64_t *xvar, const double *b, int sign, int moi,
                    const int64_t *varmap, pmt_quadratic_term *out_quad, double *out_csc, double alpha, pmt_linear_term *out_lin,
                    double *out_const, void *workspace, unsigned *counters, hipStream_t s) {
    if (!workspace || !counters) return fail(PMT_INVALID_ARGUMENT, "quad_gram: workspace required");
    const MidPlan p = mid_plan(rows, cols);
    MidArgs g;
    g.A = A; g.lda = lda; g.rows = rows; g.cols = cols; g.b = (b && sign) ? b : nullptr; g.sign = g.b ? sign : 0;
    g.xvar = xvar; g.varmap = varmap; g.moi = moi; g.out_quad = reinterpret_cast<QT *>(out_quad); g.out_csc = out_csc; g.alpha = alpha;
    g.out_lin = reinterpret_cast<LT *>(out_lin); g.out_const = out_const;
    g.nb = p.nb; g.n_off = p.n_off; g.s_off = p.s_off; g.s_diag = p.s_diag; g.gpc_off = p.gpc_off; g.gpc_diag = p.gpc_diag;
    g.n_tail = p.n_tail; g.s_tail = p.s_tail; g.gpc_tail = p.gpc_tail;
    g.ws = reinterpret_cast<double *>(workspace); g.counters = counters;
    g.xcd = rows * cols * 8 > ((int64_t)4 << 20);
    const bool fast = (reinterpret_cast<uintptr_t>(A) & 15) == 0 && (lda & 1) == 0 && (reinterpret_cast<uintptr_t>(g.b) & 15) == 0 &&
                      (uint64_t)lda * (uint64_t)cols * 8 < (1ull << 32);
    g.total = p.wgs;
    g.persist = p.wgs >= 2 * PMT_MID_G;
    g.tickets = counters + gram_mid_counters(cols) - 16;
    const unsigned grid = g.persist ? (unsigned)PMT_MID_G : (unsigned)p.wgs;
    if (fast) PMT_LAUNCH_NAMED("gram_mid_kernel", (gram_mid_kernel<true>), dim3(grid), dim3(256), 0, s, g);
    else PMT_LAUNCH_NAMED("gram_mid_kernel", (gram_mid_kernel<false>), dim3(grid), dim3(256), 0, s, g);
    return check_launch("gram_mid_kernel");
}

}
```

parametron.jl_amd/csrc/plan.hip:

```cpp
#include <algorithm>
#include <atomic>
#include <cstring>
#include <mutex>
#include <unordered_map>
#include <vector>

#include <memory>

#include "streams.h"

namespace pmt {

static thread_local std::string g_last_error;
void set_error(const std::string &msg) { g_last_error = msg; }
int fail(int code, const std::string &msg) { g_last_error = msg; return code; }

}

struct pmt_plan {
    int device = 0;
    hipStream_t stream = nullptr;
    bool owns_stream = false;
    bool recording = false;
    std::vector<void *> allocations;
    size_t bytes = 0;
    std::vector<pmt::Launch> tape;
    std::vector<pmt::Launch> exec;
    std::vector<char> exec_lanes;
    std::vector<int> node_of;
    std::vector<pmt::SmallNode> nodes;
    bool fusion = true;
    int fused_groups = 0, fused_nodes = 0, fused_phases = 0, fused_workgroups = 0;
    int *barrier_error = nullptr;
    std::vector<std::pair<void *, size_t>> fused_tables;
    hipEvent_t multi_done = nullptr;
    bool multi_pending = false;
    bool single_workgroup_runs = false;
    std::vector<char> lanes;
    char record_lane = 0;
    hipEvent_t lane_fork = nullptr, lane_join = nullptr;
    hipGraph_t graph = nullptr;
    hipGraphExec_t graph_exec = nullptr;
    char recording_tag = 0;
    hipStream_t copy_stream = nullptr;
    hipEvent_t staged[2] = {nullptr, nullptr};
    hipEvent_t consumed[2] = {nullptr, nullptr};
    bool consumed_recorded[2] = {false, false};
    hipEvent_t consumed_side[2] = {nullptr, nullptr};
    bool consumed_side_recorded[2] = {false, false};
    bool side_commits = false;
    int commit_lane = 0;
    int slot = 0;
    hipEvent_t alloc_done = nullptr;
    bool alloc_pending = false;
    std::vector<hipEvent_t> fetch_events;
    bool no_graph = false;
};

namespace pmt { int small_plan_occupancy(); }

namespace {
struct MultiRegistry { std::mutex mu; std::vector<pmt_plan *> plans; };
MultiRegistry &multi_registry(int device) {
    static std::mutex mu;
    static std::unordered_map<int, std::unique_ptr<MultiRegistry>> regs;
    std::lock_guard<std::mutex> lock(mu);
    auto &r = regs[device];
    if (!r) r.reset(new MultiRegistry);
    return *r;
}
void multi_unregister(pmt_plan *plan) {
    MultiRegistry &r = multi_registry(plan->device);
    std::lock_guard<std::mutex> lock(r.mu);
    r.plans.erase(std::remove(r.plans.begin(), r.plans.end(), plan), r.plans.end());
}
int multi_workgroup_limit(pmt_plan *plan) {
    int cus = 0, per_cu = 0;
    hipDeviceProp_t prop;
    if (hipGetDeviceProperties(&prop, plan->device) == hipSuccess) cus = prop.multiProcessorCount; else (void)hipGetLastError();
    uint32_t mask[16] = {0};
    if (hipExtStreamGetCUMask(plan->stream, 16, mask) == hipSuccess) {
        int bits = 0;
        for (uint32_t m : mask) bits += __builtin_popcount(m);
        if (bits > 0 && (cus == 0 || bits < cus)) cus = bits;
    } else (void)hipGetLastError();
    per_cu = pmt::small_plan_occupancy();
    return std::max(1, cus * std::max(1, per_cu) / 2);
}
bool multi_may_launch(MultiRegistry &r, pmt_plan *plan) {
    for (pmt_plan *other : r.plans) {
        if (other == plan || !other->multi_pending) continue;
        const hipError_t e = hipEventQuery(other->multi_done);
        if (e == hipSuccess) { other->multi_pending = false; continue; }
        (void)hipGetLastError();
        return false;
    }
    return true;
}
int check_barrier_error(pmt_plan *plan) {
    if (plan->barrier_error && __atomic_exchange_n(plan->barrier_error, 0, __ATOMIC_ACQ_REL))
        return pmt::fail(PMT_HIP_ERROR, "small plan: a workgroup waited 2 s at the grid barrier of a fused run (its workgroups were not all running); "
                                        "the outputs of this re-evaluation are invalid");
    return PMT_OK;
}
}


namespace pmt {

static std::mutex g_mu;
static std::unordered_map<void *, pmt_plan *> g_recording;

static pmt_plan *recording_plan(void *stream) {
    if (!stream) return nullptr;
    std::lock_guard<std::mutex> lock(g_mu);
    auto it = g_recording.find(stream);
    return it != g_recording.end() ? it->second : nullptr;
}

int check_strictly_increasing(const int64_t *xvar_dev, int64_t n, void *stream) {
    if (n < 2 || !xvar_dev) return PMT_OK;
    pmt_plan *plan = recording_plan(stream);
    hipStream_t s;
    if (plan) {
        s = plan->stream;
    } else {
#ifdef PMT_DEBUG_CHECKS
        s = reinterpret_cast<hipStream_t>(stream);
#else
        return PMT_OK;
#endif
    }
    std::vector<int64_t> h((size_t)n);
    PMT_HIP_CHECK(hipStreamSynchronize(s));
    PMT_HIP_CHECK(hipMemcpy(h.data(), xvar_dev, (size_t)n * sizeof(int64_t), hipMemcpyDeviceToHost));
    for (int64_t i = 0; i + 1 < n; ++i)
        if (h[(size_t)i] >= h[(size_t)i + 1])
            return fail(PMT_INVALID_ARGUMENT, "quad_gram: xvar must be strictly increasing (xvar[" + std::to_string(i) + "] = " +
                        std::to_string(h[(size_t)i]) + " >= xvar[" + std::to_string(i + 1) + "] = " + std::to_string(h[(size_t)i + 1]) +
                        "); use the literal objective or canonicalize on the device for other variable orders");
    return PMT_OK;
}

bool is_recording_handle(void *stream) { return recording_plan(stream) != nullptr; }

void mark_no_graph(void *stream) {
    if (pmt_plan *plan = recording_plan(stream)) plan->no_graph = true;
}

int dispatch(void *stream, Launch launch) {
    if (stream) {
        pmt_plan *plan = nullptr;
        {
            std::lock_guard<std::mutex> lock(g_mu);
            auto it = g_recording.find(stream);
            if (it != g_recording.end()) plan = it->second;
        }
        if (plan) {
            if (!plan->recording) return fail(PMT_STATE_ERROR, "plan is not recording (call pmt_plan_begin_record first)");
            plan->tape.push_back(std::move(launch));
            plan->lanes.push_back(plan->record_lane);
            plan->node_of.push_back(-1);
            return PMT_OK;
        }
    }
    return launch(reinterpret_cast<hipStream_t>(stream));
}

int dispatch(void *stream, Launch launch, const SmallNode &node) {
    pmt_plan *plan = recording_plan(stream);
    if (plan && plan->recording) {
        plan->nodes.push_back(node);
        const int idx = (int)plan->nodes.size() - 1;
        if (int rc = dispatch(stream, std::move(launch))) { plan->nodes.pop_back(); return rc; }
        plan->node_of.back() = idx;
        if (node.seed_host) plan->no_graph = true;
        return PMT_OK;
    }
    return dispatch(stream, std::move(launch));
}

}

namespace pmt {

struct ProfRecord { const char *name; hipEvent_t e0, e1; };
static std::atomic<bool> g_prof_on{false};
static std::string g_prof_filter;
static std::vector<ProfRecord> g_prof_records;
static std::vector<hipEvent_t> g_prof_pool;

static hipEvent_t prof_event() {
    if (!g_prof_pool.empty()) { hipEvent_t e = g_prof_pool.back(); g_prof_pool.pop_back(); return e; }
    hipEvent_t e = nullptr;
    if (hipEventCreate(&e) != hipSuccess) { (void)hipGetLastError(); return nullptr; }
    return e;
}

ProfScope::ProfScope(const char *name, hipStream_t s) : name_(name), s_(s) {
    if (!g_prof_on.load(std::memory_order_relaxed)) return;
    hipStreamCaptureStatus st = hipStreamCaptureStatusNone;
    if (hipStreamIsCapturing(s, &st) != hipSuccess) { (void)hipGetLastError(); return; }
    if (st != hipStreamCaptureStatusNone) return;
    {
        std::lock_guard<std::mutex> lock(g_mu);
        if (!g_prof_filter.empty() && !strstr(name, g_prof_filter.c_str())) return;
        e0_ = prof_event(); e1_ = prof_event();
    }
    if (e0_ && e1_) (void)hipEventRecord(e0_, s);
}
ProfScope::~ProfScope() {
    if (!e0_ || !e1_) return;
    (void)hipEventRecord(e1_, s_);
    std::lock_guard<std::mutex> lock(g_mu);
    g_prof_records.push_back({name_, e0_, e1_});
}

}

using namespace pmt;

extern "C" int pmt_profile_filter(const char *substring) {
    std::lock_guard<std::mutex> lock(g_mu);
    g_prof_filter = substring ? substring : "";
    return PMT_OK;
}

extern "C" int pmt_profile_enable(int on) {
    std::lock_guard<std::mutex> lock(g_mu);
    for (auto &r : g_prof_records) { g_prof_pool.push_back(r.e0); g_prof_pool.push_back(r.e1); }
    g_prof_records.clear();
    g_prof_on.store(on != 0);
    return PMT_OK;
}

extern "C" int64_t pmt_profile_report(char *buf, size_t cap) {
    std::vector<ProfRecord> recs;
    {
        std::lock_guard<std::mutex> lock(g_mu);
        recs = g_prof_records;
    }
    struct Agg { int64_t n = 0; double tot = 0, mn = 1e300, mx = 0; };
    std::vector<std::pair<std::string, Agg>> aggs;
    for (auto &r : recs) {
        if (hipEventSynchronize(r.e1) != hipSuccess) { (void)hipGetLastError(); continue; }
        float ms = 0;
        if (hipEventElapsedTime(&ms, r.e0, r.e1) != hipSuccess) { (void)hipGetLastError(); continue; }
        Agg *a = nullptr;
        for (auto &p : aggs) if (p.first == r.name) { a = &p.second; break; }
        if (!a) { aggs.emplace_back(r.name, Agg()); a = &aggs.back().second; }
        a->n++; a->tot += ms; a->mn = std::min(a->mn, (double)ms); a->mx = std::max(a->mx, (double)ms);
    }
    std::string out;
    char line[512];
    for (auto &p : aggs) {
        snprintf(line, sizeof line, "%s\t%lld\t%.6f\t%.6f\t%.6f\n", p.first.c_str(), (long long)p.second.n, p.second.tot, p.second.mn, p.second.mx);
        out += line;
    }
    if (buf && cap) {
        size_t k = std::min(cap - 1, out.size());
        memcpy(buf, out.data(), k);
        buf[k] = 0;
    }
    return (int64_t)out.size();
}

extern "C" const char *pmt_last_error(void) { return g_last_error.c_str(); }
extern "C" int pmt_version(void) { return 100; }
extern "C" int pmt_device_count(void) {
    int n = 0;
    if (hipGetDeviceCount(&n) != hipSuccess) { (void)hipGetLastError(); return 0; }
    return n;
}

extern "C" int pmt_plan_create(int device, void *stream, pmt_plan **out) {
    PMT_REQUIRE(out, PMT_INVALID_ARGUMENT, "plan_create: null out");
    PMT_HIP_CHECK(hipSetDevice(device));
    pmt_plan *p = new pmt_plan();
    p->device = device;
    if (stream) {
        p->stream = reinterpret_cast<hipStream_t>(stream);
    } else {
        hipError_t e = hipStreamCreateWithFlags(&p->stream, hipStreamNonBlocking);
        if (e != hipSuccess) { delete p; return fail(PMT_HIP_ERROR, std::string("hipStreamCreate: ") + hipGetErrorString(e)); }
        p->owns_stream = true;
    }
    {
        std::lock_guard<std::mutex> lock(g_mu);
        g_recording[&p->recording_tag] = p;
    }
    pmt::retain_side_stream(p->stream);
    *out = p;
    return PMT_OK;
}


extern "C" int pmt_plan_destroy(pmt_plan *plan) {
    if (!plan) return PMT_OK;
    {
        std::lock_guard<std::mutex> lock(g_mu);
        g_recording.erase(&plan->recording_tag);
    }
    (void)hipSetDevice(plan->device);
    (void)hipStreamSynchronize(plan->stream);
    (void)pmt::fetch_synchronize(plan->stream);
    pmt::release_side_stream(plan->stream);
    if (plan->copy_stream) { (void)hipStreamSynchronize(plan->copy_stream); (void)hipStreamDestroy(plan->copy_stream); }
    for (int i = 0; i < 2; ++i) {
        if (plan->staged[i]) (void)hipEventDestroy(plan->staged[i]);
        if (plan->consumed[i]) (void)hipEventDestroy(plan->consumed[i]);
    }
    if (plan->alloc_done) (void)hipEventDestroy(plan->alloc_done);
    for (hipEvent_t e : plan->fetch_events) (void)hipEventDestroy(e);
    for (int i = 0; i < 2; ++i) if (plan->consumed_side[i]) (void)hipEventDestroy(plan->consumed_side[i]);
    if (plan->lane_fork) (void)hipEventDestroy(plan->lane_fork);
    if (plan->lane_join) (void)hipEventDestroy(plan->lane_join);
    if (plan->graph_exec) (void)hipGraphExecDestroy(plan->graph_exec);
    if (plan->graph) (void)hipGraphDestroy(plan->graph);
    for (void *p : plan->allocations) (void)hipFree(p);
    for (auto &t : plan->fused_tables) (void)hipFree(t.first);
    multi_unregister(plan);
    if (plan->multi_done) (void)hipEventDestroy(plan->multi_done);
    if (plan->barrier_error) (void)hipHostFree(plan->barrier_error);
    if (plan->owns_stream) (void)hipStreamDestroy(plan->stream);
    delete plan;
    return PMT_OK;
}

extern "C" void *pmt_plan_stream(pmt_plan *plan) { return plan ? plan->stream : nullptr; }
extern "C" void *pmt_plan_recording_stream(pmt_plan *plan) { return plan ? &plan->recording_tag : nullptr; }
extern "C" size_t pmt_plan_bytes_allocated(const pmt_plan *plan) { return plan ? plan->bytes : 0; }
extern "C" int64_t pmt_plan_tape_length(const pmt_plan *plan) { return plan ? (int64_t)plan->tape.size() : 0; }

extern "C" int pmt_plan_alloc(pmt_plan *plan, size_t bytes, void **out_device_ptr) {
    PMT_REQUIRE(plan && out_device_ptr, PMT_INVALID_ARGUMENT, "plan_alloc: null argument");
    PMT_HIP_CHECK(hipSetDevice(plan->device));
    void *p = nullptr;
    size_t sz = bytes ? bytes : 16;
    hipError_t e = hipMalloc(&p, sz);
    if (e != hipSuccess) { (void)hipGetLastError(); return fail(PMT_OUT_OF_MEMORY, std::string("hipMalloc: ") + hipGetErrorString(e)); }
    PMT_HIP_CHECK(hipMemsetAsync(p, 0, sz, plan->stream));
    if (!plan->alloc_done) PMT_HIP_CHECK(hipEventCreateWithFlags(&plan->alloc_done, hipEventDisableTiming));
    PMT_HIP_CHECK(hipEventRecord(plan->alloc_done, plan->stream));
    plan->alloc_pending = true;
    plan->allocations.push_back(p);
    plan->bytes += sz;
    *out_device_ptr = p;
    return PMT_OK;
}

extern "C" int pmt_host_alloc(size_t bytes, void **out_host_ptr) {
    PMT_REQUIRE(out_host_ptr, PMT_INVALID_ARGUMENT, "host_alloc: null argument");
    void *p = nullptr;
    hipError_t e = hipHostMalloc(&p, bytes ? bytes : 16, hipHostMallocDefault);
    if (e != hipSuccess) { (void)hipGetLastError(); return fail(PMT_OUT_OF_MEMORY, std::string("hipHostMalloc: ") + hipGetErrorString(e)); }
    memset(p, 0, bytes ? bytes : 16);
    *out_host_ptr = p;
    return PMT_OK;
}

extern "C" int pmt_host_free(void *host_ptr) {
    if (!host_ptr) return PMT_OK;
    PMT_HIP_CHECK(hipHostFree(host_ptr));
    return PMT_OK;
}

extern "C" int pmt_plan_upload(pmt_plan *plan, void *device_dst, const void *host_src, size_t bytes) {
    PMT_REQUIRE(plan, PMT_INVALID_ARGUMENT, "plan_upload: null plan");
    PMT_HIP_CHECK(hipSetDevice(plan->device));
    if (bytes == 0) return PMT_OK;
    PMT_REQUIRE(device_dst && host_src, PMT_INVALID_ARGUMENT, "plan_upload: null pointer");
    PMT_HIP_CHECK(hipMemcpyAsync(device_dst, host_src, bytes, hipMemcpyHostToDevice, plan->stream));
    return PMT_OK;
}

extern "C" int pmt_plan_zero(pmt_plan *plan, void *device_dst, size_t bytes) {
    PMT_REQUIRE(plan, PMT_INVALID_ARGUMENT, "plan_zero: null plan");
    PMT_HIP_CHECK(hipSetDevice(plan->device));
    if (bytes == 0) return PMT_OK;
    PMT_REQUIRE(device_dst, PMT_INVALID_ARGUMENT, "plan_zero: null pointer");
    PMT_HIP_CHECK(hipMemsetAsync(device_dst, 0, bytes, plan->stream));
    return PMT_OK;
}

extern "C" int pmt_plan_fetch(pmt_plan *plan, void *host_dst, const void *device_src, size_t bytes) {
    PMT_REQUIRE(plan, PMT_INVALID_ARGUMENT, "plan_fetch: null plan");
    PMT_HIP_CHECK(hipSetDevice(plan->device));
    if (bytes == 0) return PMT_OK;
    PMT_REQUIRE(host_dst && device_src, PMT_INVALID_ARGUMENT, "plan_fetch: null pointer");
    PMT_HIP_CHECK(hipMemcpyAsync(host_dst, device_src, bytes, hipMemcpyDeviceToHost, plan->stream));
    return PMT_OK;
}

extern "C" int pmt_plan_upload_2d(pmt_plan *plan, void *device_dst, size_t dst_pitch, const void *host_src, size_t src_pitch, size_t width_bytes,
                                  size_t height) {
    PMT_REQUIRE(plan, PMT_INVALID_ARGUMENT, "plan_upload_2d: null plan");
    PMT_HIP_CHECK(hipSetDevice(plan->device));
    if (width_bytes == 0 || height == 0) return PMT_OK;
    PMT_REQUIRE(device_dst && host_src && dst_pitch >= width_bytes && src_pitch >= width_bytes, PMT_INVALID_ARGUMENT, "plan_upload_2d: bad argument");
    PMT_HIP_CHECK(hipMemcpy2DAsync(device_dst, dst_pitch, host_src, src_pitch, width_bytes, height, hipMemcpyHostToDevice, plan->stream));
    return PMT_OK;
}

extern "C" int pmt_plan_fetch_2d(pmt_plan *plan, void *host_dst, size_t dst_pitch, const void *device_src, size_t src_pitch, size_t width_bytes,
                                 size_t height) {
    PMT_REQUIRE(plan, PMT_INVALID_ARGUMENT, "plan_fetch_2d: null plan");
    PMT_HIP_CHECK(hipSetDevice(plan->device));
    if (width_bytes == 0 || height == 0) return PMT_OK;
    PMT_REQUIRE(host_dst && device_src && dst_pitch >= width_bytes && src_pitch >= width_bytes, PMT_INVALID_ARGUMENT, "plan_fetch_2d: bad argument");
    PMT_HIP_CHECK(hipMemcpy2DAsync(host_dst, dst_pitch, device_src, src_pitch, width_bytes, height, hipMemcpyDeviceToHost, plan->stream));
    return PMT_OK;
}

static int ensure_copy_stream(pmt_plan *plan) {
    if (plan->copy_stream) return PMT_OK;
    PMT_HIP_CHECK(hipSetDevice(plan->device));
    PMT_HIP_CHECK(hipStreamCreateWithFlags(&plan->copy_stream, hipStreamNonBlocking));
    for (int i = 0; i < 2; ++i) {
        PMT_HIP_CHECK(hipEventCreateWithFlags(&plan->staged[i], hipEventDisableTiming));
        PMT_HIP_CHECK(hipEventCreateWithFlags(&plan->consumed[i], hipEventDisableTiming));
        PMT_HIP_CHECK(hipEventCreateWithFlags(&plan->consumed_side[i], hipEventDisableTiming));
    }
    return PMT_OK;
}

static int stage_prologue(pmt_plan *plan) {
    if (int rc = ensure_copy_stream(plan)) return rc;
    PMT_HIP_CHECK(hipSetDevice(plan->device));
    if (plan->alloc_pending) {
        PMT_HIP_CHECK(hipStreamWaitEvent(plan->copy_stream, plan->alloc_done, 0));
        plan->alloc_pending = false;
    }
    if (plan->consumed_recorded[plan->slot]) PMT_HIP_CHECK(hipStreamWaitEvent(plan->copy_stream, plan->consumed[plan->slot], 0));
    if (plan->consumed_side_recorded[plan->slot]) PMT_HIP_CHECK(hipStreamWaitEvent(plan->copy_stream, plan->consumed_side[plan->slot], 0));
    return PMT_OK;
}

extern "C" int pmt_plan_stage_upload(pmt_plan *plan, void *device_staging, const void *host_src, size_t bytes) {
    PMT_REQUIRE(plan, PMT_INVALID_ARGUMENT, "plan_stage_upload: null plan");
    if (bytes == 0) return PMT_OK;
    PMT_REQUIRE(device_staging && host_src, PMT_INVALID_ARGUMENT, "plan_stage_upload: null pointer");
    if (int rc = stage_prologue(plan)) return rc;
    PMT_HIP_CHECK(hipMemcpyAsync(device_staging, host_src, bytes, hipMemcpyHostToDevice, plan->copy_stream));
    PMT_HIP_CHECK(hipEventRecord(plan->staged[plan->slot], plan->copy_stream));
    return PMT_OK;
}

extern "C" int pmt_plan_stage_upload_2d(pmt_plan *plan, void *device_staging, size_t dst_pitch, const void *host_src, size_t src_pitch,
                                        size_t width_bytes, size_t height) {
    PMT_REQUIRE(plan, PMT_INVALID_ARGUMENT, "plan_stage_upload_2d: null plan");
    if (width_bytes == 0 || height == 0) return PMT_OK;
    PMT_REQUIRE(device_staging && host_src && dst_pitch >= width_bytes && src_pitch >= width_bytes, PMT_INVALID_ARGUMENT, "plan_stage_upload_2d: bad argument");
    if (int rc = stage_prologue(plan)) return rc;
    PMT_HIP_CHECK(hipMemcpy2DAsync(device_staging, dst_pitch, host_src, src_pitch, width_bytes, height, hipMemcpyHostToDevice, plan->copy_stream));
    PMT_HIP_CHECK(hipEventRecord(plan->staged[plan->slot], plan->copy_stream));
    return PMT_OK;
}

static hipStream_t commit_stream(pmt_plan *plan) {
    if (plan->commit_lane == 1)
        if (hipStream_t side = pmt::side_stream_of(plan->stream)) return side;
    return plan->stream;
}

extern "C" int pmt_plan_wait_staged(pmt_plan *plan) {
    PMT_REQUIRE(plan, PMT_INVALID_ARGUMENT, "plan_wait_staged: null plan");
    if (!plan->copy_stream) return PMT_OK;
    PMT_HIP_CHECK(hipSetDevice(plan->device));
    PMT_HIP_CHECK(hipStreamWaitEvent(commit_stream(plan), plan->staged[plan->slot], 0));
    return PMT_OK;
}

extern "C" int pmt_plan_commit_staged(pmt_plan *plan, void *device_dst, const void *device_staging, size_t bytes) {
    PMT_REQUIRE(plan, PMT_INVALID_ARGUMENT, "plan_commit_staged: null plan");
    if (bytes == 0) return PMT_OK;
    PMT_REQUIRE(device_dst && device_staging, PMT_INVALID_ARGUMENT, "plan_commit_staged: null pointer");
    if (int rc = pmt_plan_wait_staged(plan)) return rc;
    hipStream_t target = commit_stream(plan);
    PMT_HIP_CHECK(hipMemcpyAsync(device_dst, device_staging, bytes, hipMemcpyDeviceToDevice, target));
    if (target != plan->stream) plan->side_commits = true;
    return PMT_OK;
}

extern "C" int pmt_plan_commit_lane(pmt_plan *plan, int lane) {
    PMT_REQUIRE(plan, PMT_INVALID_ARGUMENT, "plan_commit_lane: null plan");
    PMT_REQUIRE(lane == 0 || lane == 1, PMT_INVALID_ARGUMENT, "plan_commit_lane: lane must be 0 or 1");
    plan->commit_lane = lane;
    return PMT_OK;
}

extern "C" int pmt_plan_staging_consumed(pmt_plan *plan) {
    PMT_REQUIRE(plan, PMT_INVALID_ARGUMENT, "plan_staging_consumed: null plan");
    if (int rc = ensure_copy_stream(plan)) return rc;
    PMT_HIP_CHECK(hipSetDevice(plan->device));
    PMT_HIP_CHECK(hipEventRecord(plan->consumed[plan->slot], plan->stream));
    plan->consumed_recorded[plan->slot] = true;
    if (plan->side_commits) {
        if (hipStream_t side = pmt::side_stream_of(plan->stream)) {
            PMT_HIP_CHECK(hipEventRecord(plan->consumed_side[plan->slot], side));
            plan->consumed_side_recorded[plan->slot] = true;
        }
        plan->side_commits = false;
    }
    return PMT_OK;
}

extern "C" int pmt_plan_stage_slot(pmt_plan *plan, int slot) {
    PMT_REQUIRE(plan, PMT_INVALID_ARGUMENT, "plan_stage_slot: null plan");
    PMT_REQUIRE(slot == 0 || slot == 1, PMT_INVALID_ARGUMENT, "plan_stage_slot: slot must be 0 or 1");
    plan->slot = slot;
    return PMT_OK;
}

extern "C" int pmt_plan_staged_synchronize(pmt_plan *plan) {
    PMT_REQUIRE(plan, PMT_INVALID_ARGUMENT, "plan_staged_synchronize: null plan");
    if (!plan->copy_stream) return PMT_OK;
    PMT_HIP_CHECK(hipSetDevice(plan->device));
    PMT_HIP_CHECK(hipStreamSynchronize(plan->copy_stream));
    return PMT_OK;
}

extern "C" int pmt_plan_synchronize(pmt_plan *plan) {
    PMT_REQUIRE(plan, PMT_INVALID_ARGUMENT, "plan_synchronize: null plan");
    PMT_HIP_CHECK(hipSetDevice(plan->device));
    PMT_HIP_CHECK(hipStreamSynchronize(plan->stream));
    return check_barrier_error(plan);
}

extern "C" int pmt_plan_check(pmt_plan *plan) {
    PMT_REQUIRE(plan, PMT_INVALID_ARGUMENT, "plan_check: null plan");
    return check_barrier_error(plan);
}

extern "C" int pmt_plan_begin_record(pmt_plan *plan) {
    PMT_REQUIRE(plan, PMT_INVALID_ARGUMENT, "plan_begin_record: null plan");
    PMT_REQUIRE(!plan->recording, PMT_STATE_ERROR, "plan is already recording");
    PMT_REQUIRE(!plan->graph_exec, PMT_STATE_ERROR, "plan graph already instantiated");
    plan->recording = true;
    return PMT_OK;
}

namespace pmt {
size_t small_table_bytes(int count);
void small_table_image(const SmallNode *nodes, int count, void *image);
int small_plan_workgroups(int64_t work);
int launch_small_plan(const void *device_table, int count, const uint64_t *const *seed_words, int ndyn, unsigned long long syncmask,
                      unsigned long long narrowmask, int workgroups, unsigned long long *barrier_word, unsigned long long barrier_base, int *barrier_error,
                      long long barrier_bound, hipStream_t s);
void small_plan_masks(const SmallNode *nodes, int count, unsigned long long *syncmask, unsigned long long *narrowmask);
int small_plan_phases(SmallNode *nodes, int count);
int small_max_nodes();
}

static int build_exec_into(pmt_plan *plan, std::vector<pmt::Launch> &exec, std::vector<char> &exec_lanes, std::vector<std::pair<void *, size_t>> &tables);
static int build_exec(pmt_plan *plan) {
    PMT_HIP_CHECK(hipSetDevice(plan->device));
    if (!plan->fused_tables.empty()) {
        PMT_HIP_CHECK(hipStreamSynchronize(plan->stream));
        for (auto &t : plan->fused_tables) { (void)hipFree(t.first); plan->bytes -= t.second; }
        plan->fused_tables.clear();
        plan->exec.clear(); plan->exec_lanes.clear();
    }
    std::vector<pmt::Launch> exec;
    std::vector<char> exec_lanes;
    std::vector<std::pair<void *, size_t>> tables;
    const int rc = build_exec_into(plan, exec, exec_lanes, tables);
    if (rc) {
        for (auto &t : tables) (void)hipFree(t.first);
        plan->exec = plan->tape; plan->exec_lanes = plan->lanes;
        plan->fused_groups = 0; plan->fused_nodes = 0; plan->fused_phases = 0; plan->fused_workgroups = 0;
        return rc;
    }
    plan->exec.swap(exec); plan->exec_lanes.swap(exec_lanes);
    for (auto &t : tables) plan->bytes += t.second;
    plan->fused_tables.swap(tables);
    if (plan->fused_workgroups > 1) {
        MultiRegistry &r = multi_registry(plan->device);
        std::lock_guard<std::mutex> lock(r.mu);
        if (std::find(r.plans.begin(), r.plans.end(), plan) == r.plans.end()) r.plans.push_back(plan);
        if (!plan->multi_done) PMT_HIP_CHECK(hipEventCreateWithFlags(&plan->multi_done, hipEventDisableTiming));
    } else multi_unregister(plan);
    return PMT_OK;
}

static int build_exec_into(pmt_plan *plan, std::vector<pmt::Launch> &out_exec, std::vector<char> &out_lanes, std::vector<std::pair<void *, size_t>> &tables) {
    plan->fused_groups = 0; plan->fused_nodes = 0; plan->fused_phases = 0; plan->fused_workgroups = 0;
    const int wg_limit = multi_workgroup_limit(plan);
    const size_t n = plan->tape.size();
    auto small = [&](size_t i) {
        return plan->fusion && plan->node_of[i] >= 0 && plan->lanes[i] == 0 && plan->nodes[(size_t)plan->node_of[i]].work <= pmt::SMALL_NODE_WORK_MAX;
    };
    for (size_t i = 0; i < n;) {
        size_t j = i;
        int64_t work = 0;
        int ndyn = 0;
        while (j < n && small(j)) {
            const pmt::SmallNode &nd = plan->nodes[(size_t)plan->node_of[j]];
            if (work + nd.work > pmt::SMALL_GROUP_WORK_MAX && j > i) break;
            if (nd.seed_host && ndyn == pmt::SMALL_MAX_DYN) break;
            if ((int)(j - i) == pmt::small_max_nodes()) break;
            work += nd.work;
            ndyn += nd.seed_host ? 1 : 0;
            ++j;
        }
        if (j - i < 2) {
            out_exec.push_back(plan->tape[i]);
            out_lanes.push_back(plan->lanes[i]);
            ++i;
            continue;
        }
        const int count = (int)(j - i);
        std::vector<pmt::SmallNode> group;
        std::vector<const uint64_t *> words;
        for (size_t k = i; k < j; ++k) {
            pmt::SmallNode nd = plan->nodes[(size_t)plan->node_of[k]];
            nd.dyn = -1;
            if (nd.seed_host) { nd.dyn = (int)words.size(); words.push_back(nd.seed_host); }
            group.push_back(nd);
        }
        plan->fused_phases += pmt::small_plan_phases(group.data(), count);
        std::vector<char> image(pmt::small_table_bytes(count));
        pmt::small_table_image(group.data(), count, image.data());
        const size_t table_bytes = (image.size() + 63) / 64 * 64;
        void *table = nullptr;
        hipError_t e = hipMalloc(&table, table_bytes + 64);
        if (e != hipSuccess) { (void)hipGetLastError(); return fail(PMT_OUT_OF_MEMORY, std::string("hipMalloc: ") + hipGetErrorString(e)); }
        tables.emplace_back(table, table_bytes + 64);
        PMT_HIP_CHECK(hipMemcpy(table, image.data(), image.size(), hipMemcpyHostToDevice));
        PMT_HIP_CHECK(hipMemset(static_cast<char *>(table) + table_bytes, 0, 64));
        unsigned long long syncmask = 0, narrowmask = 0;
        pmt::small_plan_masks(group.data(), count, &syncmask, &narrowmask);
        int64_t group_work = 0;
        for (const pmt::SmallNode &nd : group) group_work += nd.work;
        const int wgs = plan->single_workgroup_runs ? 1 : std::min(wg_limit, pmt::small_plan_workgroups(group_work));
        unsigned long long *bar = reinterpret_cast<unsigned long long *>(static_cast<char *>(table) + table_bytes);
        if (wgs > 1 && !plan->barrier_error) {
            PMT_HIP_CHECK(hipHostMalloc(reinterpret_cast<void **>(&plan->barrier_error), 64, hipHostMallocDefault));
            memset(plan->barrier_error, 0, 64);
        }
        int *barrier_error = plan->barrier_error;
        const unsigned long long per_launch = (unsigned long long)__builtin_popcountll(syncmask) * (unsigned long long)wgs;
        std::shared_ptr<unsigned long long> arrivals = std::make_shared<unsigned long long>(0);
        plan->fused_workgroups = std::max(plan->fused_workgroups, wgs);
        out_exec.push_back([=](hipStream_t s) {
            if (wgs == 1) return pmt::launch_small_plan(table, count, words.data(), (int)words.size(), syncmask, narrowmask, 1, bar, 0, barrier_error, 0, s);
            MultiRegistry &reg = multi_registry(plan->device);
            std::lock_guard<std::mutex> lock(reg.mu);
            const bool multi = multi_may_launch(reg, plan) && !(pmt::dma::fault_injection() & 4);
            unsigned long long base = *arrivals;
            long long bound = 200000000LL;
            if (multi && (pmt::dma::fault_injection() & 2)) { base += 1; bound = 2000000LL; }
            const int rc = pmt::launch_small_plan(table, count, words.data(), (int)words.size(), syncmask, narrowmask, multi ? wgs : 1, bar, base, barrier_error, bound, s);
            if (!rc && multi) {
                *arrivals += per_launch;
                if (reg.plans.size() > 1 && plan->multi_done && hipEventRecord(plan->multi_done, s) == hipSuccess) plan->multi_pending = true;
            }
            return rc;
        });
        out_lanes.push_back(0);
        plan->fused_groups += 1;
        plan->fused_nodes += count;
        i = j;
    }
    return PMT_OK;
}

extern "C" int pmt_plan_end_record(pmt_plan *plan) {
    PMT_REQUIRE(plan, PMT_INVALID_ARGUMENT, "plan_end_record: null plan");
    PMT_REQUIRE(plan->recording, PMT_STATE_ERROR, "plan is not recording");
    plan->recording = false;
    plan->record_lane = 0;
    return build_exec(plan);
}

extern "C" int pmt_plan_set_fusion(pmt_plan *plan, int on) {
    PMT_REQUIRE(plan, PMT_INVALID_ARGUMENT, "plan_set_fusion: null plan");
    PMT_REQUIRE(!plan->recording, PMT_STATE_ERROR, "plan_set_fusion: the plan is recording");
    PMT_REQUIRE(!plan->graph_exec, PMT_STATE_ERROR, "plan_set_fusion: the plan's graph is already instantiated");
    plan->fusion = on != 0;
    PMT_HIP_CHECK(hipSetDevice(plan->device));
    PMT_HIP_CHECK(hipStreamSynchronize(plan->stream));
    return build_exec(plan);
}

extern "C" int pmt_plan_fused_phases(const pmt_plan *plan) { return plan ? plan->fused_phases : 0; }
extern "C" int pmt_plan_fused_workgroups(const pmt_plan *plan) { return plan ? plan->fused_workgroups : 0; }

extern "C" int pmt_plan_fused(const pmt_plan *plan, int *groups, int *nodes, int64_t *exec_length) {
    PMT_REQUIRE(plan, PMT_INVALID_ARGUMENT, "plan_fused: null plan");
    if (groups) *groups = plan->fused_groups;
    if (nodes) *nodes = plan->fused_nodes;
    if (exec_length) *exec_length = (int64_t)plan->exec.size();
    return PMT_OK;
}


static int replay(pmt_plan *plan, hipStream_t s) {
    if (!plan->fetch_events.empty())
        if (int rc = pmt::fetch_fence(s)) return rc;
    bool any = false;
    for (char l : plan->exec_lanes) any |= (l != 0);
    pmt::replay_begin(s, any);
    struct End { hipStream_t s; int rc = PMT_OK; bool done = false; int finish() { if (!done) { done = true; rc = pmt::replay_end(s); } return rc; } ~End() { finish(); } } end{s};
    hipStream_t side = nullptr;
    if (any && (side = pmt::side_stream_of(s))) {
        if (!plan->lane_fork) {
            PMT_HIP_CHECK(hipEventCreateWithFlags(&plan->lane_fork, hipEventDisableTiming));
            PMT_HIP_CHECK(hipEventCreateWithFlags(&plan->lane_join, hipEventDisableTiming));
        }
        PMT_HIP_CHECK(hipEventRecord(plan->lane_fork, s));
    }
    bool forked = false;
    bool side_used = false;
    for (size_t i = 0; side && i < plan->exec.size(); ++i)
        if (plan->exec_lanes[i] == 3) {
            side_used = true;
            if (int rc = plan->exec[i](side)) return rc;
        }
    for (size_t i = 0; side && i < plan->exec.size(); ++i) {
        if (plan->exec_lanes[i] != 2) continue;
        if (!forked) { PMT_HIP_CHECK(hipStreamWaitEvent(side, plan->lane_fork, 0)); forked = true; }
        if (int rc = plan->exec[i](side)) return rc;
    }
    for (size_t i = 0; i < plan->exec.size(); ++i) {
        hipStream_t target = s;
        if (side && plan->exec_lanes[i] >= 2) continue;
        if (side && plan->exec_lanes[i]) {
            if (!forked) { PMT_HIP_CHECK(hipStreamWaitEvent(side, plan->lane_fork, 0)); forked = true; }
            target = side;
        }
        int rc = plan->exec[i](target);
        if (rc) return rc;
    }
    if (forked || side_used) {
        PMT_HIP_CHECK(hipEventRecord(plan->lane_join, side));
        PMT_HIP_CHECK(hipStreamWaitEvent(s, plan->lane_join, 0));
    }
    return end.finish();
}

extern "C" int pmt_plan_record_fetch(pmt_plan *plan, void *host_dst, const void *device_src, size_t bytes) {
    PMT_REQUIRE(plan, PMT_INVALID_ARGUMENT, "plan_record_fetch: null plan");
    PMT_REQUIRE(plan->recording, PMT_STATE_ERROR, "plan_record_fetch: the plan is not recording");
    if (bytes == 0) return PMT_OK;
    PMT_REQUIRE(host_dst && device_src, PMT_INVALID_ARGUMENT, "plan_record_fetch: null pointer");
    PMT_HIP_CHECK(hipSetDevice(plan->device));
    hipEvent_t ev = nullptr;
    PMT_HIP_CHECK(hipEventCreateWithFlags(&ev, hipEventDisableTiming));
    plan->fetch_events.push_back(ev);
    hipStream_t main = plan->stream;
    std::shared_ptr<pmt::FetchState> st = std::make_shared<pmt::FetchState>();
    plan->tape.push_back([=](hipStream_t target) { return pmt::fetch_async(main, target, ev, host_dst, device_src, bytes, st.get(), pmt::FetchRect{}); });
    plan->lanes.push_back(plan->record_lane);
    plan->node_of.push_back(-1);
    return PMT_OK;
}

extern "C" int pmt_plan_record_fetch_2d(pmt_plan *plan, void *host_dst, size_t dst_pitch, const void *device_src, size_t src_pitch, size_t width_bytes,
                                        size_t height) {
    PMT_REQUIRE(plan, PMT_INVALID_ARGUMENT, "plan_record_fetch_2d: null plan");
    PMT_REQUIRE(plan->recording, PMT_STATE_ERROR, "plan_record_fetch_2d: the plan is not recording");
    if (width_bytes == 0 || height == 0) return PMT_OK;
    PMT_REQUIRE(host_dst && device_src && dst_pitch >= width_bytes && src_pitch >= width_bytes, PMT_INVALID_ARGUMENT, "plan_record_fetch_2d: bad argument");
    if (dst_pitch == width_bytes && src_pitch == width_bytes) return pmt_plan_record_fetch(plan, host_dst, device_src, width_bytes * height);
    PMT_HIP_CHECK(hipSetDevice(plan->device));
    hipEvent_t ev = nullptr;
    PMT_HIP_CHECK(hipEventCreateWithFlags(&ev, hipEventDisableTiming));
    plan->fetch_events.push_back(ev);
    hipStream_t main = plan->stream;
    std::shared_ptr<pmt::FetchState> st = std::make_shared<pmt::FetchState>();
    pmt::FetchRect r;
    r.dst_pitch = dst_pitch; r.src_pitch = src_pitch; r.height = height;
    plan->tape.push_back([=](hipStream_t target) { return pmt::fetch_async(main, target, ev, host_dst, device_src, width_bytes, st.get(), r); });
    plan->lanes.push_back(plan->record_lane);
    plan->node_of.push_back(-1);
    return PMT_OK;
}

extern "C" int pmt_plan_fetch_synchronize(pmt_plan *plan) {
    PMT_REQUIRE(plan, PMT_INVALID_ARGUMENT, "plan_fetch_synchronize: null plan");
    PMT_HIP_CHECK(hipSetDevice(plan->device));
    if (int rc = pmt::fetch_synchronize(plan->stream)) return rc;
    return check_barrier_error(plan);
}

extern "C" int pmt_plan_set_lane(pmt_plan *plan, int lane) {
    PMT_REQUIRE(plan, PMT_INVALID_ARGUMENT, "plan_set_lane: null plan");
    PMT_REQUIRE(plan->recording, PMT_STATE_ERROR, "plan_set_lane: the plan is not recording");
    PMT_REQUIRE(lane >= 0 && lane <= 3, PMT_INVALID_ARGUMENT, "plan_set_lane: lane must be 0, 1, 2 or 3");
    plan->record_lane = (char)lane;
    return PMT_OK;
}

extern "C" int pmt_plan_lane_stream(pmt_plan *plan, int lane, void **out_stream) {
    PMT_REQUIRE(plan && out_stream, PMT_INVALID_ARGUMENT, "plan_lane_stream: null pointer");
    PMT_REQUIRE(lane >= 0 && lane <= 2, PMT_INVALID_ARGUMENT, "plan_lane_stream: lane must be 0, 1 or 2");
    PMT_HIP_CHECK(hipSetDevice(plan->device));
    hipStream_t s = lane == 0 ? plan->stream : pmt::side_stream_of(plan->stream);
    PMT_REQUIRE(s || lane == 0, PMT_STATE_ERROR, "plan_lane_stream: the plan's stream has no side stream");
    *out_stream = s;
    return PMT_OK;
}

extern "C" int pmt_plan_update(pmt_plan *plan) {
    PMT_REQUIRE(plan, PMT_INVALID_ARGUMENT, "plan_update: null plan");
    PMT_REQUIRE(!plan->recording, PMT_STATE_ERROR, "plan is still recording");
    PMT_HIP_CHECK(hipSetDevice(plan->device));
    if (plan->graph_exec) {
        PMT_HIP_CHECK(hipGraphLaunch(plan->graph_exec, plan->stream));
        return PMT_OK;
    }
    return replay(plan, plan->stream);
}

extern "C" int pmt_plan_instantiate_graph(pmt_plan *plan) {
    PMT_REQUIRE(plan, PMT_INVALID_ARGUMENT, "plan_instantiate_graph: null plan");
    PMT_REQUIRE(!plan->recording, PMT_STATE_ERROR, "plan is still recording");
    if (plan->graph_exec) return PMT_OK;
    PMT_REQUIRE(plan->fetch_events.empty() && !plan->no_graph, PMT_STATE_ERROR,
                "plan_instantiate_graph: a tape with recorded fetches or a host delivery is replayed as launches (its copies leave the capture)");
    PMT_HIP_CHECK(hipSetDevice(plan->device));
    if (plan->fused_workgroups > 1) {
        PMT_HIP_CHECK(hipStreamSynchronize(plan->stream));
        plan->single_workgroup_runs = true;
        if (int rc = build_exec(plan)) return rc;
    }
    PMT_HIP_CHECK(hipStreamBeginCapture(plan->stream, hipStreamCaptureModeThreadLocal));
    int rc = replay(plan, plan->stream);
    hipError_t e = hipStreamEndCapture(plan->stream, &plan->graph);
    if (rc) { if (plan->graph) { (void)hipGraphDestroy(plan->graph); plan->graph = nullptr; } return rc; }
    if (e != hipSuccess) return fail(PMT_HIP_ERROR, std::string("hipStreamEndCapture: ") + hipGetErrorString(e));
    PMT_HIP_CHECK(hipGraphInstantiate(&plan->graph_exec, plan->graph, nullptr, nullptr, 0));
    return PMT_OK;
}
```

parametron.jl_amd/csrc/streams.h:

```cpp
#pragma once
#include <memory>
#include <vector>

#include "dma.h"
#include "gram_common.h"

namespace pmt {

struct SideStream {
    hipStream_t stream = nullptr; hipEvent_t fork = nullptr, join = nullptr, join2 = nullptr; int device = -1;
    void *counters = nullptr;
    int *err_host = nullptr, *err_dev = nullptr;
    hipStream_t fetch = nullptr; hipEvent_t fetch_done = nullptr; bool fetch_pending = false;
    std::vector<std::pair<dma::Engine *, dma::Signal>> dma_pending;
    std::vector<std::shared_ptr<void>> keepalive;
    bool in_replay = false;
    bool side_work = false;
    std::vector<std::function<int()>> deferred;
};
constexpr int ERR_COURIER = 1, ERR_PAIR_FOLD = 2;
constexpr size_t PROGRESS_OFFSET = 0;
constexpr size_t FLAGS_OFFSET = PROGRESS_OFFSET + MAXGROUPS * sizeof(unsigned long long);
constexpr size_t DONE_OFFSET = FLAGS_OFFSET + MAXGROUPS * sizeof(long long);
constexpr size_t MID_OFFSET = DONE_OFFSET + 2 * sizeof(unsigned);
constexpr size_t MID_COUNTER_BYTES = 135168;
constexpr size_t COUNTER_BYTES = MID_OFFSET + MID_COUNTER_BYTES;

SideStream *side_stream(hipStream_t s);
int ensure_fetch_stream(SideStream *ss);
int wait_dma_pending(SideStream *ss);
inline hipStream_t side_stream_of(hipStream_t s) { SideStream *ss = side_stream(s); return ss ? ss->stream : nullptr; }
void retain_side_stream(hipStream_t s);
void release_side_stream(hipStream_t s);
int fetch_async(hipStream_t s, hipStream_t after, hipEvent_t order_event, void *host_dst, const void *device_src, size_t bytes, FetchState *st, FetchRect r);
int fetch_fence(hipStream_t s);
int fetch_synchronize(hipStream_t s);
void replay_begin(hipStream_t s, bool side_work);
int replay_end(hipStream_t s);
int gram_after_deferred(hipStream_t s, std::function<int()> f);

void *host_device_pointer(void *host);
int launch_courier(const double *src, double *dst_dev, long long *ready, unsigned *done, int *error, int ngroups, const int64_t *gbeg, const int64_t *gend, hipStream_t s);
int launch_to_host(const void *src, void *dst_dev, size_t bytes, hipStream_t s);
int launch_to_host_2d(const void *src, size_t src_pitch, void *dst_dev, size_t dst_pitch, size_t width_bytes, size_t height, hipStream_t s);

}
```

Baseline: 916.3 re-evaluations/s.

## Fold independent affine VAT nodes as riders into persistent Gram-mid kernel

Adds a rider mechanism. Independent affine (VAT triplet) tape nodes are attached to the persistent Gram-mid launch so their tiles run in the same kernel instead of as separate launches. At plan build, a host-side dependency check compares read and write address ranges to choose riders, and a device table describes each rider's tiles. The goal is to fill idle workgroups during the Gram computation and cut launch and serialization overhead for the C,d rebuild. The cost is extra complexity, blocking host syncs and memcpys at plan build time, and a risk of contention with the Gram kernel.

```diff
diff --git a/include/parametron_hip.h b/include/parametron_hip.h
--- a/include/parametron_hip.h
+++ b/include/parametron_hip.h
@@ -303,6 +303,14 @@
 int64_t pmt_plan_tape_length(const pmt_plan *plan);
 int pmt_plan_set_fusion(pmt_plan *plan, int on);
 int pmt_plan_fused(const pmt_plan *plan, int *groups, int *nodes, int64_t *exec_length);
+#define PMT_RIDER_RANGES 5
+typedef struct pmt_rider_entry {
+    int32_t kind, lane;
+    int64_t rows, cols;
+    uint64_t reads[PMT_RIDER_RANGES][2], writes[PMT_RIDER_RANGES][2];
+} pmt_rider_entry;
+int pmt_plan_riders(const pmt_plan *plan, int *riders, int64_t *tiles);
+int pmt_plan_rider_check(const pmt_rider_entry *tape, int64_t n, int64_t node, int *rides, int *riders, int64_t *tiles);
 int pmt_plan_fused_phases(const pmt_plan *plan);
 int pmt_plan_fused_workgroups(const pmt_plan *plan);
 typedef struct pmt_model pmt_model;
diff --git a/parametron.jl_amd/_lib.py b/parametron.jl_amd/_lib.py
--- a/parametron.jl_amd/_lib.py
+++ b/parametron.jl_amd/_lib.py
@@ -233,6 +233,8 @@
     "pmt_plan_tape_length": (_i64, [_vp]),
     "pmt_plan_set_fusion": (_ci, [_vp, _ci]),
     "pmt_plan_fused": (_ci, [_vp, C.POINTER(_ci), C.POINTER(_ci), C.POINTER(_i64)]),
+    "pmt_plan_riders": (_ci, [_vp, C.POINTER(_ci), C.POINTER(_i64)]),
+    "pmt_plan_rider_check": (_ci, [_vp, _i64, _i64, C.POINTER(_ci), C.POINTER(_ci), C.POINTER(_i64)]),
     "pmt_plan_fused_phases": (_ci, [_vp]),
     "pmt_plan_fused_workgroups": (_ci, [_vp]),
     "pmt_fill_uniform_dyn_f64": (_ci, [_vp, _i64, _i64, _i64, C.POINTER(_u64), _f64, _vp]),
diff --git a/parametron.jl_amd/csrc/affine.hip b/parametron.jl_amd/csrc/affine.hip
--- a/parametron.jl_amd/csrc/affine.hip
+++ b/parametron.jl_amd/csrc/affine.hip
@@ -1,26 +1,8 @@
-#include "common.h"
+#include "affine_tile.h"
 
 namespace pmt {
 
 constexpr int64_t NTL_MIN_BYTES = 8 << 20;
-
-constexpr int TILE = 64;
-constexpr int PITCH = TILE + 1;
-
-typedef unsigned long long u64;
-typedef u64 u64x2 __attribute__((ext_vector_type(2)));
-typedef double f64x2 __attribute__((ext_vector_type(2)));
-
-__device__ __forceinline__ u64 f2u(double x) { return (u64)__double_as_longlong(x); }
-
-template <bool NT>
-__device__ __forceinline__ void store16(u64x2 *p, u64x2 v) {
-    if (NT) __builtin_nontemporal_store(v, p); else *p = v;
-}
-template <bool NT>
-__device__ __forceinline__ void store8(u64 *p, u64 v) {
-    if (NT) __builtin_nontemporal_store(v, p); else *p = v;
-}
 
 template <int MODE, bool NT, int TR, bool NTL = false>
 __global__ __launch_bounds__(256) void affine_tile_kernel(
@@ -34,86 +16,8 @@
     const int t = threadIdx.x;
     const unsigned wg = blockIdx.y * gridDim.x + blockIdx.x;
     if (stamps && t == 0 && wg < stamp_cap) stamps[2 * wg] = (u64)wall_clock64();
-    const int lane = t & 63;
-    const int wave = t >> 6;
-    const int64_t c0 = (int64_t)blockIdx.x * TILE;
-    const int64_t r0 = (int64_t)blockIdx.y * TR;
-    const int nr = (int)min((int64_t)TR, rows - r0);
-    const int nc = (int)min((int64_t)TILE, cols - c0);
-    const bool full = (nr == TR) && (nc == TILE);
-
-    if (full && vec_in) {
-        constexpr int TPC = TR / 2;
-        constexpr int CPI = 256 / TPC;
-        const int cg = t / TPC;
-        const int lr = (t % TPC) * 2;
-        const double *base = A + (c0 + cg) * lda + r0 + lr;
-#pragma unroll
-        for (int it = 0; it < TILE / CPI; ++it) {
-            const f64x2 *src = reinterpret_cast<const f64x2 *>(base + (int64_t)it * CPI * lda);
-            f64x2 v = NTL ? __builtin_nontemporal_load(src) : *src;
-            const int c = it * CPI + cg;
-            tile[lr * PITCH + c] = v.x;
-            tile[(lr + 1) * PITCH + c] = v.y;
-        }
-    } else {
-        const int r = t & 63;
-        for (int c = t >> 6; c < nc; c += 4)
-            if (r < nr) tile[r * PITCH + c] = A[(c0 + c) * lda + r0 + r];
-    }
-    if (t < nc) {
-        const int64_t v = xvar[c0 + t];
-        vmx[t] = (u64)(MODE == 1 ? map_var(varmap, v) : v);
-    }
-    if (blockIdx.x == 0 && t < nr && out_consts)
-        out_consts[r0 + t] = signed_const(b ? b[r0 + t] : 0.0, b ? sign : 0);
-    __syncthreads();
-
-    if (MODE == 0) {
-        if (lane < nc) {
-            const u64 var = vmx[lane];
-            for (int r = wave; r < nr; r += 4) {
-                u64x2 v;
-                v.x = f2u(tile[r * PITCH + lane]);
-                v.y = var;
-                store16<NT>(reinterpret_cast<u64x2 *>(out + ((r0 + r) * cols + c0 + lane) * 2), v);
-            }
-        }
-    } else {
-        if (full && vec_out) {
-            for (int rp = wave * 2; rp < TR; rp += 8) {
-#pragma unroll
-                for (int s = 0; s < 3; ++s) {
-                    int r, chunk;
-                    if (s == 0) { r = rp; chunk = lane; }
-                    else if (s == 1) { r = rp + (lane >> 5); chunk = 64 + (lane & 31); }
-                    else { r = rp + 1; chunk = lane; }
-                    const int q0 = chunk * 2;
-                    const u64 rowidx = (u64)(row_offset + r0 + r + 1);
-                    u64 w[2];
-#pragma unroll
-                    for (int h = 0; h < 2; ++h) {
-                        const int q = q0 + h;
-                        const int term = q / 3;
-                        const int f = q - term * 3;
-                        w[h] = (f == 0) ? rowidx : (f == 1 ? f2u(tile[r * PITCH + term]) : vmx[term]);
-                    }
-                    u64x2 v; v.x = w[0]; v.y = w[1];
-                    store16<NT>(reinterpret_cast<u64x2 *>(out + ((r0 + r) * cols + c0) * 3 + q0), v);
-                }
-            }
-        } else {
-            if (lane < nc) {
-                const u64 var = vmx[lane];
-                for (int r = wave; r < nr; r += 4) {
-                    u64 *p = out + ((r0 + r) * cols + c0 + lane) * 3;
-                    store8<NT>(p, (u64)(row_offset + r0 + r + 1));
-                    store8<NT>(p + 1, f2u(tile[r * PITCH + lane]));
-                    store8<NT>(p + 2, var);
-                }
-            }
-        }
-    }
+    affine_tile_body<MODE, NT, TR, NTL>(A, lda, rows, cols, xvar, b, sign, varmap, row_offset, out, out_consts, vec_in, vec_out,
+                                        (int)blockIdx.x, (int)blockIdx.y, t, tile, vmx);
     if (stamps) {
         __syncthreads();
         if (t == 0 && wg < stamp_cap) {
@@ -253,6 +157,9 @@
 static u64 *g_stamps = nullptr;
 static unsigned g_stamp_cap = 0;
 
+static bool affine_small_tiles(int64_t rows, int64_t cols) { return cdiv(cols, TILE) * cdiv(rows, TILE) < 1024 && rows > 32; }
+static bool affine_cold(int64_t rows, int64_t cols) { return rows * cols * (int64_t)sizeof(double) >= NTL_MIN_BYTES; }
+
 template <int MODE>
 static int launch_affine(const double *A, int64_t lda, int64_t rows, int64_t cols, const int64_t *xvar, const double *b, int sign,
                          const int64_t *varmap, int64_t row_offset, void *out_terms, double *out_consts, hipStream_t s) {
@@ -261,8 +168,8 @@
     const int vec_out = ((reinterpret_cast<uintptr_t>(out_terms) & 15) == 0 && (cols & 1) == 0) ? 1 : 0;
     const char *name = MODE == 0 ? "affine_tile_kernel<LT>" : "affine_tile_kernel<VAT>";
     u64 *out = reinterpret_cast<u64 *>(out_terms);
-    const bool small = cdiv(cols, TILE) * cdiv(rows, TILE) < 1024 && rows > 32;
-    const bool ntl = MODE == 1 && rows * cols * (int64_t)sizeof(double) >= NTL_MIN_BYTES;
+    const bool small = affine_small_tiles(rows, cols);
+    const bool ntl = MODE == 1 && affine_cold(rows, cols);
     u64 *stamps = MODE == 1 ? g_stamps : nullptr;
 #define AFFINE_LAUNCH(NTV, TRV, NTLV)                                                                                                    \
     PMT_LAUNCH_NAMED(name, (affine_tile_kernel<MODE, NTV, TRV, NTLV>), dim3((unsigned)cdiv(cols, TILE), (unsigned)cdiv(rows, TRV)), dim3(256), 0, s, A, \
@@ -277,6 +184,28 @@
     else { if (small) AFFINE_LAUNCH(false, 32, false); else AFFINE_LAUNCH(false, 64, false); }
 #undef AFFINE_LAUNCH
     return check_launch("affine_tile_kernel");
+}
+
+int64_t affine_rider_tiles(int64_t rows, int64_t cols) {
+    if (rows <= 0 || cols <= 0) return 0;
+    return cdiv(cols, TILE) * cdiv(rows, affine_small_tiles(rows, cols) ? 32 : 64);
+}
+bool affine_rider(const SmallNode &nd, AffineRider *r) {
+    const int64_t lda = nd.d[0], rows = nd.d[1], cols = nd.d[2];
+    if (nd.op != SOP_AFFINE_VAT || rows <= 0 || cols <= 0) return false;
+    r->A = static_cast<const double *>(nd.in[0]); r->lda = lda; r->rows = rows; r->cols = cols;
+    r->xvar = static_cast<const int64_t *>(nd.in[1]); r->b = static_cast<const double *>(nd.in[2]);
+    r->varmap = static_cast<const int64_t *>(nd.in[3]); r->row_offset = nd.d[3];
+    r->out = static_cast<u64 *>(nd.out[0]); r->out_consts = static_cast<double *>(nd.out[1]);
+    r->sign = nd.sign;
+    r->vec_in = ((reinterpret_cast<uintptr_t>(r->A) & 15) == 0 && (lda & 1) == 0) ? 1 : 0;
+    r->vec_out = ((reinterpret_cast<uintptr_t>(r->out) & 15) == 0 && (cols & 1) == 0) ? 1 : 0;
+    r->tr = affine_small_tiles(rows, cols) ? 32 : 64;
+    r->ntl = affine_cold(rows, cols) ? 1 : 0;
+    r->nt = (r->ntl || env_nt()) ? 1 : 0;
+    r->tiles_x = (int)cdiv(cols, TILE);
+    r->first_tile = 0;
+    return true;
 }
 
 }
diff --git a/parametron.jl_amd/csrc/affine_tile.h b/parametron.jl_amd/csrc/affine_tile.h
--- /dev/null
+++ b/parametron.jl_amd/csrc/affine_tile.h
@@ -0,0 +1,124 @@
+#pragma once
+#include "common.h"
+
+namespace pmt {
+
+constexpr int TILE = 64;
+constexpr int PITCH = TILE + 1;
+
+typedef unsigned long long u64;
+typedef u64 u64x2 __attribute__((ext_vector_type(2)));
+typedef double f64x2 __attribute__((ext_vector_type(2)));
+
+__device__ __forceinline__ u64 f2u(double x) { return (u64)__double_as_longlong(x); }
+
+template <bool NT>
+__device__ __forceinline__ void store16(u64x2 *p, u64x2 v) {
+    if (NT) __builtin_nontemporal_store(v, p); else *p = v;
+}
+template <bool NT>
+__device__ __forceinline__ void store8(u64 *p, u64 v) {
+    if (NT) __builtin_nontemporal_store(v, p); else *p = v;
+}
+
+struct AffineRider {
+    const double *A; int64_t lda, rows, cols;
+    const int64_t *xvar; const double *b; const int64_t *varmap; int64_t row_offset;
+    u64 *out; double *out_consts;
+    int sign, vec_in, vec_out;
+    int tr, nt, ntl;
+    int tiles_x, first_tile;
+};
+
+template <int MODE, bool NT, int TR, bool NTL>
+__device__ __forceinline__ void affine_tile_body(const double *__restrict__ A, int64_t lda, int64_t rows, int64_t cols,
+                                                 const int64_t *__restrict__ xvar, const double *__restrict__ b, int sign,
+                                                 const int64_t *__restrict__ varmap, int64_t row_offset, u64 *__restrict__ out,
+                                                 double *__restrict__ out_consts, int vec_in, int vec_out, int bx, int by, int t,
+                                                 double *tile, u64 *vmx) {
+    const int lane = t & 63;
+    const int wave = t >> 6;
+    const int64_t c0 = (int64_t)bx * TILE;
+    const int64_t r0 = (int64_t)by * TR;
+    const int nr = (int)min((int64_t)TR, rows - r0);
+    const int nc = (int)min((int64_t)TILE, cols - c0);
+    const bool full = (nr == TR) && (nc == TILE);
+
+    if (full && vec_in) {
+        constexpr int TPC = TR / 2;
+        constexpr int CPI = 256 / TPC;
+        const int cg = t / TPC;
+        const int lr = (t % TPC) * 2;
+        const double *base = A + (c0 + cg) * lda + r0 + lr;
+#pragma unroll
+        for (int it = 0; it < TILE / CPI; ++it) {
+            const f64x2 *src = reinterpret_cast<const f64x2 *>(base + (int64_t)it * CPI * lda);
+            f64x2 v = NTL ? __builtin_nontemporal_load(src) : *src;
+            const int c = it * CPI + cg;
+            tile[lr * PITCH + c] = v.x;
+            tile[(lr + 1) * PITCH + c] = v.y;
+        }
+    } else {
+        const int r = t & 63;
+        for (int c = t >> 6; c < nc; c += 4)
+            if (r < nr) tile[r * PITCH + c] = A[(c0 + c) * lda + r0 + r];
+    }
+    if (t < nc) {
+        const int64_t v = xvar[c0 + t];
+        vmx[t] = (u64)(MODE == 1 ? map_var(varmap, v) : v);
+    }
+    if (bx == 0 && t < nr && out_consts)
+        out_consts[r0 + t] = signed_const(b ? b[r0 + t] : 0.0, b ? sign : 0);
+    __syncthreads();
+
+    if (MODE == 0) {
+        if (lane < nc) {
+            const u64 var = vmx[lane];
+            for (int r = wave; r < nr; r += 4) {
+                u64x2 v;
+                v.x = f2u(tile[r * PITCH + lane]);
+                v.y = var;
+                store16<NT>(reinterpret_cast<u64x2 *>(out + ((r0 + r) * cols + c0 + lane) * 2), v);
+            }
+        }
+    } else {
+        if (full && vec_out) {
+            for (int rp = wave * 2; rp < TR; rp += 8) {
+#pragma unroll
+                for (int s = 0; s < 3; ++s) {
+                    int r, chunk;
+                    if (s == 0) { r = rp; chunk = lane; }
+                    else if (s == 1) { r = rp + (lane >> 5); chunk = 64 + (lane & 31); }
+                    else { r = rp + 1; chunk = lane; }
+                    const int q0 = chunk * 2;
+                    const u64 rowidx = (u64)(row_offset + r0 + r + 1);
+                    u64 w[2];
+#pragma unroll
+                    for (int h = 0; h < 2; ++h) {
+                        const int q = q0 + h;
+                        const int term = q / 3;
+                        const int f = q - term * 3;
+                        w[h] = (f == 0) ? rowidx : (f == 1 ? f2u(tile[r * PITCH + term]) : vmx[term]);
+                    }
+                    u64x2 v; v.x = w[0]; v.y = w[1];
+                    store16<NT>(reinterpret_cast<u64x2 *>(out + ((r0 + r) * cols + c0) * 3 + q0), v);
+                }
+            }
+        } else {
+            if (lane < nc) {
+                const u64 var = vmx[lane];
+                for (int r = wave; r < nr; r += 4) {
+                    u64 *p = out + ((r0 + r) * cols + c0 + lane) * 3;
+                    store8<NT>(p, (u64)(row_offset + r0 + r + 1));
+                    store8<NT>(p + 1, f2u(tile[r * PITCH + lane]));
+                    store8<NT>(p + 2, var);
+                }
+            }
+        }
+    }
+}
+
+bool affine_rider(const SmallNode &nd, AffineRider *out);
+int64_t affine_rider_tiles(int64_t rows, int64_t cols);
+
+}
diff --git a/parametron.jl_amd/csrc/gram.hip b/parametron.jl_amd/csrc/gram.hip
--- a/parametron.jl_amd/csrc/gram.hip
+++ b/parametron.jl_amd/csrc/gram.hip
@@ -291,7 +291,8 @@
     PMT_REQUIRE(side && side->counters && (size_t)gram_mid_counters(g.cols) * sizeof(unsigned) <= MID_COUNTER_BYTES, PMT_STATE_ERROR,
                 "quad_gram: no auxiliary state for this stream");
     int rc = launch_gram_mid(g.A, g.lda, g.rows, g.cols, g.xvar, g.b, g.sign, g.moi, g.varmap, g.out_quad, g.out_csc, g.alpha, g.out_lin,
-                             g.out_const, g.workspace, reinterpret_cast<unsigned *>(static_cast<char *>(side->counters) + MID_OFFSET), s);
+                             g.out_const, g.workspace, reinterpret_cast<unsigned *>(static_cast<char *>(side->counters) + MID_OFFSET),
+                             side->mid_riders, side->mid_nriders, side->mid_rider_tiles, s);
     return !rc && forks_in_replay(side) ? fork_side(side, s) : rc;
 }
 
@@ -372,7 +373,7 @@
         dplan.sig = std::make_shared<DeliverSignals>();
         mark_no_graph(stream);
     }
-    return dispatch(stream, [=](hipStream_t s) -> int {
+    Launch node = [=](hipStream_t s) -> int {
         SideStream *side = side_stream(s);
         const bool deliver = dplan.host != nullptr;
         if (deliver) { if (int rc = deliver_arm(dplan, side, s)) return rc; }
@@ -381,7 +382,12 @@
         if (!rc && deliver) rc = release_group(dplan, side, 0, s);
         if (!rc && deliver) rc = deliver_submit(dplan, side);
         return rc;
-    });
+    };
+    if (form == GramForm::Mid && !host && cols > 0)
+        return dispatch_mid(stream, std::move(node), MidNote{g.A, g.lda, rows, cols, (g.b && g.sign) ? g.b : nullptr, g.xvar, g.moi ? g.varmap : nullptr,
+                                                              g.out_quad, g.out_csc, g.out_lin, g.out_const, g.workspace,
+                                                              pmt_quad_gram_workspace_bytes(rows, cols)});
+    return dispatch(stream, std::move(node));
 }
 
 }
diff --git a/parametron.jl_amd/csrc/gram_common.h b/parametron.jl_amd/csrc/gram_common.h
--- a/parametron.jl_amd/csrc/gram_common.h
+++ b/parametron.jl_amd/csrc/gram_common.h
@@ -180,7 +180,18 @@
 int gram_mid_counters(int64_t cols);
 int launch_gram_mid(const double *A, int64_t lda, int64_t rows, int64_t cols, const int64_t *xvar, const double *b, int sign, int moi,
                     const int64_t *varmap, pmt_quadratic_term *out_quad, double *out_csc, double alpha, pmt_linear_term *out_lin,
-                    double *out_const, void *workspace, unsigned *counters, hipStream_t s);
+                    double *out_const, void *workspace, unsigned *counters, const void *riders, int nriders, int rider_tiles, hipStream_t s);
+bool gram_mid_persistent(int64_t rows, int64_t cols);
+struct MidNote {
+    const double *A; int64_t lda, rows, cols; const double *b; const int64_t *xvar, *varmap;
+    const void *out_quad, *out_csc, *out_lin, *out_const, *workspace; size_t workspace_bytes;
+};
+int dispatch_mid(void *stream, Launch launch, const MidNote &note);
+#ifndef PMT_MID_RIDER_MB
+#define PMT_MID_RIDER_MB 256
+#endif
+constexpr int MID_MAX_RIDERS = 8;
+constexpr int64_t PMT_MID_RIDER_BYTES = (int64_t)PMT_MID_RIDER_MB << 20;
 int launch_gram_mid_constant(const double *b, int sign, int64_t rows, double *out_const, hipStream_t s);
 int check_strictly_increasing(const int64_t *xvar_dev, int64_t n, void *stream);
 void mark_no_graph(void *stream);
diff --git a/parametron.jl_amd/csrc/gram_mid.hip b/parametron.jl_amd/csrc/gram_mid.hip
--- a/parametron.jl_amd/csrc/gram_mid.hip
+++ b/parametron.jl_amd/csrc/gram_mid.hip
@@ -1,3 +1,4 @@
+#include "affine_tile.h"
 #include "gram_common.h"
 
 #ifndef PMT_MID_WPS
@@ -35,6 +36,7 @@
 #ifdef PMT_MID_TRACE
 __device__ unsigned long long g_mid_trace[1024 * 8];
 __device__ unsigned long long g_mid_walk[1024 * 8];
+__device__ unsigned long long g_mid_riders[1024 * 2];
 #define MID_TRACE_WORDS 8
 __device__ __forceinline__ void mid_walk_note(unsigned long long *w, int k, unsigned long long t) {
     if (k == 0) { if (w[0]) w[4] += t - w[7]; else w[5] = t; w[0] += 1; }
@@ -51,6 +53,9 @@
 }
 extern "C" int pmt_mid_walk_read(unsigned long long *host) {
     return hipMemcpyFromSymbol(host, HIP_SYMBOL(g_mid_walk), sizeof(unsigned long long) * 1024 * 8) == hipSuccess ? 0 : 1;
+}
+extern "C" int pmt_mid_riders_read(unsigned long long *host) {
+    return hipMemcpyFromSymbol(host, HIP_SYMBOL(g_mid_riders), sizeof(unsigned long long) * 1024 * 2) == hipSuccess ? 0 : 1;
 }
 #else
 #define MID_STAMP(k) do { } while (0)
@@ -85,6 +90,8 @@
     int xcd;
     int persist, total;
     unsigned *tickets;
+    const AffineRider *riders;
+    int nriders, rider_tiles;
 };
 
 struct MidPlan { int nb, n_off, s_off, s_diag, gpc_off, gpc_diag, n_tail, s_tail, gpc_tail, wgs; };
@@ -741,6 +748,24 @@
     mid_forget(pbuf);
 }
 
+__device__ __forceinline__ void mid_rider_tile(const AffineRider &r, int local, double *sh) {
+    int t;
+    asm volatile("v_mov_b32 %0, %1" : "=v"(t) : "v"((int)threadIdx.x));
+    const int by = local / r.tiles_x, bx = local - by * r.tiles_x;
+    double *tile = sh;
+    u64 *vmx = reinterpret_cast<u64 *>(sh + TILE * PITCH);
+#define MID_RIDE(NTV, TRV, NTLV)                                                                                                         \
+    affine_tile_body<1, NTV, TRV, NTLV>(r.A, r.lda, r.rows, r.cols, r.xvar, r.b, r.sign, r.varmap, r.row_offset, r.out, r.out_consts,   \
+                                        r.vec_in, r.vec_out, bx, by, t, tile, vmx)
+    if (r.ntl) { if (r.tr == 32) MID_RIDE(true, 32, true); else MID_RIDE(true, 64, true); }
+#ifdef PMT_TUNING
+    else if (!r.nt) { if (r.tr == 32) MID_RIDE(false, 32, false); else MID_RIDE(false, 64, false); }
+#endif
+    else { if (r.tr == 32) MID_RIDE(true, 32, false); else MID_RIDE(true, 64, false); }
+#undef MID_RIDE
+}
+static_assert(TILE * PITCH + TILE <= MQBUF, "a rider's tile and its variable-map row live in the front of the kernel's LDS");
+
 template <bool FAST>
 __global__ __launch_bounds__(256, PMT_MID_WPS) void gram_mid_kernel(MidArgs g) {
     __shared__ double sh[MSH + MID_TRACE_WORDS];
@@ -787,6 +812,25 @@
         if (id >= g.total) break;
         cur = mid_decode(g, id);
     }
+    if (g.rider_tiles > 0) {
+        int mine = 0;
+        for (;;) {
+            __syncthreads();
+            if (tid == 0) next_id = (int)__hip_atomic_fetch_add(g.tickets + 9, 1u, __ATOMIC_RELAXED, __HIP_MEMORY_SCOPE_AGENT);
+            __syncthreads();
+            const int rt = __builtin_amdgcn_readfirstlane(next_id);
+            if (rt >= g.rider_tiles) break;
+            int k = 0;
+            while (k + 1 < g.nriders && rt >= g.riders[k + 1].first_tile) ++k;
+            mid_rider_tile(g.riders[k], rt - g.riders[k].first_tile, sh);
+            ++mine;
+        }
+#ifdef PMT_MID_TRACE
+        __builtin_amdgcn_s_waitcnt(0);
+        if (tid == 0 && blockIdx.x < 1024) { g_mid_riders[blockIdx.x * 2] = (unsigned long long)mine; g_mid_riders[blockIdx.x * 2 + 1] = wall_clock64(); }
+#endif
+        (void)mine;
+    }
 #ifdef PMT_MID_TRACE
     if (tid == 0 && blockIdx.x < 1024) {
         for (int i = 0; i < 7; ++i) g_mid_walk[blockIdx.x * 8 + i] = reinterpret_cast<unsigned long long *>(sh + MSH)[i];
@@ -797,7 +841,7 @@
         const unsigned gone = __hip_atomic_fetch_add(g.tickets + 8, 1u, __ATOMIC_RELAXED, __HIP_MEMORY_SCOPE_AGENT);
         if (gone == gridDim.x - 1) {
 #pragma unroll
-            for (int i = 0; i < 9; ++i) __hip_atomic_store(g.tickets + i, 0u, __ATOMIC_RELAXED, __HIP_MEMORY_SCOPE_AGENT);
+            for (int i = 0; i < 10; ++i) __hip_atomic_store(g.tickets + i, 0u, __ATOMIC_RELAXED, __HIP_MEMORY_SCOPE_AGENT);
         }
     }
 }
@@ -818,11 +862,12 @@
     const MidPlan p = mid_plan(rows, cols);
     return sizeof(double) * (size_t)p.wgs * MSTRIDE;
 }
+bool gram_mid_persistent(int64_t rows, int64_t cols) { return cols > 0 && rows > 0 && mid_plan(rows, cols).wgs >= 2 * PMT_MID_G; }
 int gram_mid_counters(int64_t cols) { const int nb = (int)cdiv(cols, MT); return MCNT * (nb * (nb + 1) / 2) + 16; }
 
 int launch_gram_mid(const double *A, int64_t lda, int64_t rows, int64_t cols, const int64_t *xvar, const double *b, int sign, int moi,
                     const int64_t *varmap, pmt_quadratic_term *out_quad, double *out_csc, double alpha, pmt_linear_term *out_lin,
-                    double *out_const, void *workspace, unsigned *counters, hipStream_t s) {
+                    double *out_const, void *workspace, unsigned *counters, const void *riders, int nriders, int rider_tiles, hipStream_t s) {
     if (!workspace || !counters) return fail(PMT_INVALID_ARGUMENT, "quad_gram: workspace required");
     const MidPlan p = mid_plan(rows, cols);
     MidArgs g;
@@ -838,6 +883,8 @@
     g.total = p.wgs;
     g.persist = p.wgs >= 2 * PMT_MID_G;
     g.tickets = counters + gram_mid_counters(cols) - 16;
+    const bool ride = g.persist && riders && nriders > 0 && rider_tiles > 0;
+    g.riders = ride ? static_cast<const AffineRider *>(riders) : nullptr; g.nriders = ride ? nriders : 0; g.rider_tiles = ride ? rider_tiles : 0;
     const unsigned grid = g.persist ? (unsigned)PMT_MID_G : (unsigned)p.wgs;
     if (fast) PMT_LAUNCH_NAMED("gram_mid_kernel", (gram_mid_kernel<true>), dim3(grid), dim3(256), 0, s, g);
     else PMT_LAUNCH_NAMED("gram_mid_kernel", (gram_mid_kernel<false>), dim3(grid), dim3(256), 0, s, g);
diff --git a/parametron.jl_amd/csrc/plan.hip b/parametron.jl_amd/csrc/plan.hip
--- a/parametron.jl_amd/csrc/plan.hip
+++ b/parametron.jl_amd/csrc/plan.hip
@@ -7,6 +7,7 @@
 
 #include <memory>
 
+#include "affine_tile.h"
 #include "streams.h"
 
 namespace pmt {
@@ -29,6 +30,10 @@
     std::vector<char> exec_lanes;
     std::vector<int> node_of;
     std::vector<pmt::SmallNode> nodes;
+    std::unordered_map<size_t, pmt::MidNote> mid_notes;
+    int riders = 0; int64_t rider_tiles = 0;
+    bool lane1_riders = false;
+    bool side_external = false;
     bool fusion = true;
     int fused_groups = 0, fused_nodes = 0, fused_phases = 0, fused_workgroups = 0;
     int *barrier_error = nullptr;
@@ -167,6 +172,16 @@
     return launch(reinterpret_cast<hipStream_t>(stream));
 }
 
+int dispatch_mid(void *stream, Launch launch, const MidNote &note) {
+    pmt_plan *plan = recording_plan(stream);
+    if (plan && plan->recording) {
+        if (int rc = dispatch(stream, std::move(launch))) return rc;
+        plan->mid_notes[plan->tape.size() - 1] = note;
+        return PMT_OK;
+    }
+    return dispatch(stream, std::move(launch));
+}
+
 int dispatch(void *stream, Launch launch, const SmallNode &node) {
     pmt_plan *plan = recording_plan(stream);
     if (plan && plan->recording) {
@@ -412,6 +427,17 @@
     return PMT_OK;
 }
 
+static int build_exec(pmt_plan *plan);
+static int side_stream_goes_external(pmt_plan *plan) {
+    if (plan->side_external) return PMT_OK;
+    plan->side_external = true;
+    if (!plan->lane1_riders) return PMT_OK;
+    PMT_REQUIRE(!plan->graph_exec, PMT_STATE_ERROR, "plan: side-lane packs ride in the captured graph's Gram node; use the side stream before pmt_plan_instantiate_graph");
+    PMT_HIP_CHECK(hipSetDevice(plan->device));
+    PMT_HIP_CHECK(hipStreamSynchronize(plan->stream));
+    return build_exec(plan);
+}
+
 static int ensure_copy_stream(pmt_plan *plan) {
     if (plan->copy_stream) return PMT_OK;
     PMT_HIP_CHECK(hipSetDevice(plan->device));
@@ -486,7 +512,7 @@
     PMT_REQUIRE(plan, PMT_INVALID_ARGUMENT, "plan_commit_lane: null plan");
     PMT_REQUIRE(lane == 0 || lane == 1, PMT_INVALID_ARGUMENT, "plan_commit_lane: lane must be 0 or 1");
     plan->commit_lane = lane;
-    return PMT_OK;
+    return lane ? side_stream_goes_external(plan) : PMT_OK;
 }
 
 extern "C" int pmt_plan_staging_consumed(pmt_plan *plan) {
@@ -583,12 +609,135 @@
     return PMT_OK;
 }
 
+static bool ranges_meet(const uint64_t (*a)[2], const uint64_t (*b)[2]) {
+    for (int i = 0; i < PMT_RIDER_RANGES; ++i)
+        for (int j = 0; j < PMT_RIDER_RANGES; ++j)
+            if (a[i][0] < a[i][1] && b[j][0] < b[j][1] && a[i][0] < b[j][1] && b[j][0] < a[i][1]) return true;
+    return false;
+}
+static bool rider_independent(const pmt_rider_entry &a, const pmt_rider_entry &b) {
+    if (a.kind == 0 || b.kind == 0) return false;
+    return !ranges_meet(a.writes, b.writes) && !ranges_meet(a.writes, b.reads) && !ranges_meet(a.reads, b.writes);
+}
+
+extern "C" int pmt_plan_rider_check(const pmt_rider_entry *tape, int64_t n, int64_t node, int *rides, int *riders, int64_t *tiles) {
+    PMT_REQUIRE(tape && rides && n >= 0 && node >= 0 && node < n && tape[node].kind == 1, PMT_INVALID_ARGUMENT, "plan_rider_check: bad argument");
+    for (int64_t i = 0; i < n; ++i) rides[i] = 0;
+    int count = 0;
+    int64_t bytes = 0, ntiles = 0;
+    const pmt_rider_entry &nd = tape[node];
+    const bool persistent = pmt::gram_mid_persistent(nd.rows, nd.cols);
+    bool run = true;
+    for (int64_t i = 0; persistent && i < n; ++i) {
+        const pmt_rider_entry &e = tape[i];
+        if (i == node) continue;
+        const bool side = e.lane == 1;
+        if (!side) {
+            if (e.lane != 0 || i < node || !run) continue;
+            if (e.kind != 2) { run = false; continue; }
+        }
+        if (e.kind != 2 || e.rows <= 0 || e.cols <= 0 || count == pmt::MID_MAX_RIDERS) continue;
+        if (e.rows > pmt::PMT_MID_RIDER_BYTES / 32 / e.cols || bytes + 32 * e.rows * e.cols > pmt::PMT_MID_RIDER_BYTES) continue;
+        bool ok = rider_independent(e, nd);
+        for (int64_t k = 0; ok && k < n; ++k) {
+            if (k == i || k == node) continue;
+            const bool matters = rides[k] || (side ? tape[k].lane != 0 : (tape[k].lane == 0 && k > node && k < i));
+            if (matters && !rider_independent(e, tape[k])) ok = false;
+        }
+        if (!ok) continue;
+        rides[i] = 1;
+        count += 1;
+        bytes += 32 * e.rows * e.cols;
+        ntiles += pmt::affine_rider_tiles(e.rows, e.cols);
+    }
+    if (riders) *riders = count;
+    if (tiles) *tiles = ntiles;
+    return PMT_OK;
+}
+
+extern "C" int pmt_plan_riders(const pmt_plan *plan, int *riders, int64_t *tiles) {
+    PMT_REQUIRE(plan, PMT_INVALID_ARGUMENT, "plan_riders: null plan");
+    if (riders) *riders = plan->riders;
+    if (tiles) *tiles = plan->rider_tiles;
+    return PMT_OK;
+}
+
+static void set_range(uint64_t (&r)[2], const void *p, size_t bytes) {
+    r[0] = reinterpret_cast<uintptr_t>(p); r[1] = p ? r[0] + bytes : r[0];
+}
+static int64_t max_index(const int64_t *xvar_dev, int64_t n, bool increasing) {
+    if (n <= 0 || !xvar_dev) return 0;
+    std::vector<int64_t> h((size_t)(increasing ? 1 : n));
+    if (hipMemcpy(h.data(), increasing ? xvar_dev + n - 1 : xvar_dev, h.size() * sizeof(int64_t), hipMemcpyDeviceToHost) != hipSuccess) { (void)hipGetLastError(); return -1; }
+    return std::max<int64_t>(0, *std::max_element(h.begin(), h.end()));
+}
+
+static std::vector<int64_t> choose_riders(pmt_plan *plan) {
+    const size_t n = plan->tape.size();
+    std::vector<int64_t> host(n, -1);
+    if (!plan->fusion || plan->mid_notes.empty()) return host;
+    std::vector<pmt_rider_entry> entries(n);
+    bool packs = false;
+    for (size_t i = 0; i < n; ++i) {
+        pmt_rider_entry &e = entries[i];
+        memset(&e, 0, sizeof e);
+        e.lane = plan->lanes[i];
+        if (plan->node_of[i] < 0 || (e.lane == 1 && plan->side_external)) continue;
+        const pmt::SmallNode &nd = plan->nodes[(size_t)plan->node_of[i]];
+        if (nd.op != pmt::SOP_AFFINE_VAT || nd.d[1] <= 0 || nd.d[2] <= 0) continue;
+        e.kind = 2; e.rows = nd.d[1]; e.cols = nd.d[2];
+        packs = true;
+    }
+    if (!packs) return host;
+    if (hipStreamSynchronize(plan->stream) != hipSuccess) { (void)hipGetLastError(); return host; }
+    for (size_t i = 0; i < n; ++i) {
+        pmt_rider_entry &e = entries[i];
+        if (e.kind != 2) continue;
+        const pmt::SmallNode &nd = plan->nodes[(size_t)plan->node_of[i]];
+        const int64_t lda = nd.d[0], vmax = nd.in[3] ? max_index(static_cast<const int64_t *>(nd.in[1]), e.cols, false) : 0;
+        if (vmax < 0) { e.kind = 0; continue; }
+        set_range(e.reads[0], nd.in[0], sizeof(double) * (size_t)((e.cols - 1) * lda + e.rows));
+        set_range(e.reads[1], nd.in[1], sizeof(int64_t) * (size_t)e.cols);
+        set_range(e.reads[2], nd.in[2], sizeof(double) * (size_t)e.rows);
+        set_range(e.reads[3], nd.in[3], sizeof(int64_t) * (size_t)vmax);
+        set_range(e.writes[0], nd.out[0], sizeof(pmt::VAT) * (size_t)(e.rows * e.cols));
+        set_range(e.writes[1], nd.out[1], sizeof(double) * (size_t)e.rows);
+    }
+    std::vector<int> rides(n);
+    for (size_t i = 0; i < n; ++i) {
+        auto it = plan->mid_notes.find(i);
+        if (it == plan->mid_notes.end()) continue;
+        const pmt::MidNote &m = it->second;
+        const int64_t vmax = m.varmap ? max_index(m.xvar, m.cols, true) : 0;
+        if (vmax < 0) continue;
+        pmt_rider_entry &e = entries[i];
+        const size_t nq = (size_t)(m.cols * (m.cols + 1) / 2);
+        e.kind = 1; e.rows = m.rows; e.cols = m.cols;
+        set_range(e.reads[0], m.A, sizeof(double) * (size_t)((m.cols - 1) * m.lda + m.rows));
+        set_range(e.reads[1], m.b, sizeof(double) * (size_t)m.rows);
+        set_range(e.reads[2], m.xvar, sizeof(int64_t) * (size_t)m.cols);
+        set_range(e.reads[3], m.varmap, sizeof(int64_t) * (size_t)vmax);
+        set_range(e.writes[0], m.out_quad, sizeof(pmt::QT) * nq);
+        set_range(e.writes[1], m.out_csc, sizeof(double) * nq);
+        set_range(e.writes[2], m.out_lin, sizeof(pmt::LT) * (size_t)m.cols);
+        set_range(e.writes[3], m.out_const, sizeof(double));
+        set_range(e.writes[4], m.workspace, m.workspace_bytes);
+        if (pmt_plan_rider_check(entries.data(), (int64_t)n, (int64_t)i, rides.data(), nullptr, nullptr)) continue;
+        for (size_t k = 0; k < n; ++k)
+            if (rides[k]) { host[k] = (int64_t)i; entries[k].kind = 0; }
+        e.kind = 0;
+    }
+    return host;
+}
+
 static int build_exec_into(pmt_plan *plan, std::vector<pmt::Launch> &out_exec, std::vector<char> &out_lanes, std::vector<std::pair<void *, size_t>> &tables) {
     plan->fused_groups = 0; plan->fused_nodes = 0; plan->fused_phases = 0; plan->fused_workgroups = 0;
+    plan->riders = 0; plan->rider_tiles = 0; plan->lane1_riders = false;
     const int wg_limit = multi_workgroup_limit(plan);
     const size_t n = plan->tape.size();
+    const std::vector<int64_t> host = choose_riders(plan);
     auto small = [&](size_t i) {
-        return plan->fusion && plan->node_of[i] >= 0 && plan->lanes[i] == 0 && plan->nodes[(size_t)plan->node_of[i]].work <= pmt::SMALL_NODE_WORK_MAX;
+        return host[i] < 0 && plan->fusion && plan->node_of[i] >= 0 && plan->lanes[i] == 0 && plan->nodes[(size_t)plan->node_of[i]].work <= pmt::SMALL_NODE_WORK_MAX;
     };
     for (size_t i = 0; i < n;) {
         size_t j = i;
@@ -604,7 +753,37 @@
             ++j;
         }
         if (j - i < 2) {
-            out_exec.push_back(plan->tape[i]);
+            if (host[i] >= 0) { ++i; continue; }
+            pmt::Launch entry = plan->tape[i];
+            std::vector<pmt::AffineRider> riders;
+            for (size_t k = 0; k < n; ++k) {
+                pmt::AffineRider r;
+                if (host[k] != (int64_t)i || !pmt::affine_rider(plan->nodes[(size_t)plan->node_of[k]], &r)) continue;
+                r.first_tile = riders.empty() ? 0 : riders.back().first_tile + (int)pmt::affine_rider_tiles(riders.back().rows, riders.back().cols);
+                riders.push_back(r);
+                plan->lane1_riders |= plan->lanes[k] == 1;
+            }
+            if (!riders.empty()) {
+                const int count = (int)riders.size();
+                const int ntiles = riders.back().first_tile + (int)pmt::affine_rider_tiles(riders.back().rows, riders.back().cols);
+                const size_t table_bytes = sizeof(pmt::AffineRider) * riders.size();
+                void *table = nullptr;
+                hipError_t e = hipMalloc(&table, table_bytes);
+                if (e != hipSuccess) { (void)hipGetLastError(); return fail(PMT_OUT_OF_MEMORY, std::string("hipMalloc: ") + hipGetErrorString(e)); }
+                tables.emplace_back(table, table_bytes);
+                PMT_HIP_CHECK(hipMemcpy(table, riders.data(), table_bytes, hipMemcpyHostToDevice));
+                pmt::Launch node = entry;
+                entry = [=](hipStream_t s) {
+                    pmt::SideStream *ss = pmt::side_stream(s);
+                    if (ss) { ss->mid_riders = table; ss->mid_nriders = count; ss->mid_rider_tiles = ntiles; }
+                    const int rc = node(s);
+                    if (ss) { ss->mid_riders = nullptr; ss->mid_nriders = 0; ss->mid_rider_tiles = 0; }
+                    return rc;
+                };
+                plan->riders += count;
+                plan->rider_tiles += ntiles;
+            }
+            out_exec.push_back(std::move(entry));
             out_lanes.push_back(plan->lanes[i]);
             ++i;
             continue;
@@ -799,7 +978,7 @@
     hipStream_t s = lane == 0 ? plan->stream : pmt::side_stream_of(plan->stream);
     PMT_REQUIRE(s || lane == 0, PMT_STATE_ERROR, "plan_lane_stream: the plan's stream has no side stream");
     *out_stream = s;
-    return PMT_OK;
+    return lane ? side_stream_goes_external(plan) : PMT_OK;
 }
 
 extern "C" int pmt_plan_update(pmt_plan *plan) {
diff --git a/parametron.jl_amd/csrc/streams.h b/parametron.jl_amd/csrc/streams.h
--- a/parametron.jl_amd/csrc/streams.h
+++ b/parametron.jl_amd/csrc/streams.h
@@ -17,6 +17,7 @@
     bool in_replay = false;
     bool side_work = false;
     std::vector<std::function<int()>> deferred;
+    const void *mid_riders = nullptr; int mid_nriders = 0, mid_rider_tiles = 0;
 };
 constexpr int ERR_COURIER = 1, ERR_PAIR_FOLD = 2;
 constexpr size_t PROGRESS_OFFSET = 0;
```

New measurement: 929.4 re-evaluations/s (median of 6 runs). +1.4%, better.
